# xd009642/xd-tts

Hardware: AMD Instinct MI355X
Metric: mel-frames/s per GPU, 120-phoneme utterance (Tacotron2 decoder+postnet + 60-iter Griffin-Lim), end-to-end (higher is better)
Workload: dtype f32

## Files before the change

### include/xdtts.h

```cpp
#ifndef XDTTS_H
#define XDTTS_H

#include <stddef.h>
#include <stdint.h>

#ifdef __cplusplus
extern "C" {
#endif

typedef int32_t xdtts_status;
enum {
  XDTTS_OK = 0,
  XDTTS_ERR_BAD_ARG = 1,
  XDTTS_ERR_IO = 2,
  XDTTS_ERR_HIP = 3,
  XDTTS_ERR_OOM = 4,
  XDTTS_ERR_TOO_LONG = 5,
  XDTTS_ERR_NO_DEVICE = 6
};

typedef struct xdtts_tacotron2 xdtts_tacotron2;
typedef struct xdtts_griffinlim xdtts_griffinlim;

typedef struct {
  float gate_threshold;
  int32_t max_steps;
  int32_t fixed_steps;
  int32_t dropout_mode;
  uint32_t dropout_seed;
  int32_t max_chunk;
  uint32_t item_base;
  float fixed_frames_per_id;
  const uint8_t *dropout_masks;
  int32_t dropout_mask_steps;
} xdtts_infer_opts;

void xdtts_infer_opts_default(xdtts_infer_opts *opts);


xdtts_status xdtts_tacotron2_load(const char *dir, int32_t device_id, xdtts_tacotron2 **out);

#define XDTTS_DEVICE_DEFAULT (-1)
int32_t xdtts_default_device(void);

xdtts_status xdtts_model_dir_read(const char *dir, float *blob, size_t n_floats);

xdtts_status xdtts_model_dir_describe(const char *dir, char *buf, size_t cap, size_t *needed);

xdtts_status xdtts_tacotron2_load_synthetic(uint32_t seed, float rec_scale, int32_t device_id,
                                            xdtts_tacotron2 **out);

xdtts_status xdtts_tacotron2_load_blob(const float *blob, size_t n_floats, int32_t device_id,
                                       xdtts_tacotron2 **out);

xdtts_status xdtts_tacotron2_save(const xdtts_tacotron2 *h, const char *dir);

int32_t xdtts_tensor_count(void);
const char *xdtts_tensor_name(int32_t i);
int32_t xdtts_tensor_ndim(int32_t i);
int32_t xdtts_tensor_dim(int32_t i, int32_t d);
size_t xdtts_tensor_offset(int32_t i);
size_t xdtts_tensor_total(void);
xdtts_status xdtts_tacotron2_get_tensor(const xdtts_tacotron2 *h, int32_t i, float *out);

xdtts_status xdtts_tacotron2_infer_ids(xdtts_tacotron2 *h, const int64_t *ids, size_t n,
                                       const size_t *splits, size_t n_splits,
                                       const xdtts_infer_opts *opts, float **mel,
                                       size_t *n_frames);

xdtts_status xdtts_tacotron2_infer_batch(xdtts_tacotron2 *h, const int64_t *ids,
                                         const int32_t *lens, int32_t B, int32_t t_stride,
                                         const xdtts_infer_opts *opts,
                                         const int32_t *fixed_steps_per_item, float **mels,
                                         size_t *n_frames);

xdtts_status xdtts_tacotron2_encoder(xdtts_tacotron2 *h, const int64_t *ids, int32_t T,
                                     float *memory, float *processed_memory);
xdtts_status xdtts_tacotron2_decoder(xdtts_tacotron2 *h, const float *memory,
                                     const float *processed_memory, int32_t T, int32_t n_valid,
                                     const xdtts_infer_opts *opts, float *frames, float *gates,
                                     size_t *n_frames);
xdtts_status xdtts_tacotron2_decoder_step(xdtts_tacotron2 *h, const float *memory, const float *processed_memory,
                                          int32_t T, int32_t n_valid, const xdtts_infer_opts *opts, uint32_t step,
                                          const float *decoder_input, float *attention_hidden,
                                          float *attention_cell, float *decoder_hidden, float *decoder_cell,
                                          float *attention_weights, float *attention_weights_cum,
                                          float *attention_context, float *decoder_output,
                                          float *gate_prediction);

xdtts_status xdtts_tacotron2_decoder_steps(xdtts_tacotron2 *h, int32_t engine, int32_t B, const float *memory,
                                           const float *processed_memory, int32_t T, const int32_t *n_valid,
                                           const xdtts_infer_opts *opts, uint32_t step0, int32_t n_steps,
                                           const float *decoder_input, float *attention_hidden, float *attention_cell,
                                           float *decoder_hidden, float *decoder_cell, float *attention_weights,
                                           float *attention_weights_cum, float *attention_context, float *decoder_output,
                                           float *gate_prediction);

xdtts_status xdtts_tacotron2_engine_state(const xdtts_tacotron2 *h, int32_t *decoder_persistent,
                                          int32_t *encoder_cooperative, int32_t *batched_attention);
xdtts_status xdtts_tacotron2_engine_reset(xdtts_tacotron2 *h);
xdtts_status xdtts_tacotron2_small_batch_engine_state(const xdtts_tacotron2 *h, int32_t *state);

const char *xdtts_build_info(void);

xdtts_status xdtts_edge_floor_us(int32_t device_id, int32_t steps, int32_t T, int32_t tuned, double *us_per_step);

xdtts_status xdtts_tacotron2_postnet(xdtts_tacotron2 *h, const float *frames, int32_t F,
                                     float *mel_out);

xdtts_status xdtts_tacotron2_last_timings(const xdtts_tacotron2 *h, float ms[4], int32_t *steps);

void xdtts_tacotron2_free(xdtts_tacotron2 *h);


xdtts_status xdtts_mel_filter_bank(float sample_rate, size_t n_fft, size_t n_mels, float fmin,
                                   float fmax_or_nan, float *out);

xdtts_status xdtts_griffinlim_new(const float *mel_basis, size_t n_mels, size_t n_bins,
                                  size_t noverlap, float power, size_t iters, float momentum,
                                  int32_t device_id, xdtts_griffinlim **out);

typedef struct {
  int32_t nnls_iters;
  int32_t power_mode;
  int32_t mel_decompress;
  int32_t output_normalise;
  int32_t batch_shape;
  float rms_target;
} xdtts_griffinlim_opts;
void xdtts_griffinlim_opts_default(xdtts_griffinlim_opts *opts);
xdtts_status xdtts_griffinlim_set_opts(xdtts_griffinlim *g, const xdtts_griffinlim_opts *opts);
xdtts_status xdtts_griffinlim_get_opts(const xdtts_griffinlim *g, xdtts_griffinlim_opts *opts);

xdtts_status xdtts_griffinlim_set_seed(xdtts_griffinlim *g, uint32_t seed);

xdtts_status xdtts_griffinlim_infer(xdtts_griffinlim *g, const float *mel, size_t n_mels,
                                    size_t n_frames, float **audio, size_t *n_samples);

xdtts_status xdtts_griffinlim_infer_batch(xdtts_griffinlim *g, const float *const *mels, size_t n_mels,
                                          const size_t *n_frames, int32_t n_utt, float **audios,
                                          size_t *n_samples);

xdtts_status xdtts_griffinlim_infer_linear(xdtts_griffinlim *g, const float *S,
                                           const float *phase0, size_t n_frames, size_t iters,
                                           float **audio, size_t *n_samples);

xdtts_status xdtts_griffinlim_mel_to_linear(xdtts_griffinlim *g, const float *mel,
                                            size_t n_mels, size_t n_frames, float *S_out);

xdtts_status xdtts_griffinlim_step(xdtts_griffinlim *g, const float *S, float *angles,
                                   float *rebuilt, size_t n_frames, size_t n_iter);

xdtts_status xdtts_griffinlim_last_timings(const xdtts_griffinlim *g, float ms[3]);

size_t       xdtts_griffinlim_analysis_frames(const xdtts_griffinlim *g, size_t n_samples);
xdtts_status xdtts_griffinlim_analyze(xdtts_griffinlim *g, const float *audio, size_t n_samples, float mel_floor,
                                      float *S_out, float *mel_out, size_t *n_frames);
xdtts_status xdtts_griffinlim_analyze_batch(xdtts_griffinlim *g, const float *const *audios, const size_t *n_samples,
                                            int32_t n_utt, float mel_floor, float **S_outs, float **mel_outs,
                                            size_t *n_frames);
xdtts_status xdtts_griffinlim_spectral_convergence(xdtts_griffinlim *g, const float *audio, size_t n_samples,
                                                   const float *S, size_t n_frames, int32_t fit_gain, float out[2]);
xdtts_status xdtts_griffinlim_analysis_timings(const xdtts_griffinlim *g, float ms[3]);

void xdtts_griffinlim_free(xdtts_griffinlim *g);

xdtts_status xdtts_synthesize_ids(xdtts_tacotron2 *h, xdtts_griffinlim *g, const int64_t *ids,
                                  size_t n, const size_t *splits, size_t n_splits,
                                  const xdtts_infer_opts *opts, float **mel, size_t *n_frames,
                                  float **audio, size_t *n_samples);

xdtts_status xdtts_synthesize_batch(xdtts_tacotron2 *h, xdtts_griffinlim *g, const int64_t *ids,
                                    const int32_t *lens, int32_t B, int32_t t_stride,
                                    const int32_t *utt_chunks, int32_t n_utt,
                                    const xdtts_infer_opts *opts,
                                    const int32_t *fixed_steps_per_item, float **mels,
                                    size_t *n_frames, float **audios, size_t *n_samples);

xdtts_status xdtts_synthesize_sequence(xdtts_tacotron2 *h, xdtts_griffinlim *g, const int64_t *const *ids,
                                       const size_t *n_ids, const size_t *const *splits, const size_t *n_splits,
                                       int32_t n_utt, const xdtts_infer_opts *opts, float **mels,
                                       size_t *n_frames, float **audios, size_t *n_samples);

int32_t xdtts_symbol_count(void);
const char *xdtts_symbol_token(int32_t id);
int64_t xdtts_unit_id(const char *token, int32_t as_character);
int32_t xdtts_split_score(int64_t id);
xdtts_status xdtts_find_splits(const int64_t *ids, size_t n, size_t max_size, size_t *out,
                               size_t cap, size_t *n_out);

#define XDTTS_SAMPLE_RATE 22050
xdtts_status xdtts_audio_to_i16(const float *audio, size_t n, int16_t *pcm);
size_t xdtts_silence_samples(double seconds, uint32_t sample_rate);
size_t xdtts_silence_samples_duration(uint64_t secs, uint32_t nanos, uint32_t sample_rate);
xdtts_status xdtts_wav_write(const char *path, const int16_t *pcm, size_t n, uint32_t sample_rate);
xdtts_status xdtts_npy_write_f32(const char *path, const float *data, size_t rows, size_t cols);
double xdtts_real_time_factor(double compute_seconds, size_t n_samples);

void xdtts_free(void *p);
const char *xdtts_last_error(void);
int32_t xdtts_device_count(void);
xdtts_status xdtts_tacotron2_sync(xdtts_tacotron2 *h);

#ifdef __cplusplus
}
#endif
#endif
```

### xd-tts_amd/__init__.py

```python
import ctypes as C
import os

import numpy as np

_HERE = os.path.dirname(os.path.abspath(__file__))
LIB_PATH = os.environ.get("XDTTS_LIB") or os.path.join(_HERE, "libxdtts_hip.so")

N_MEL = 80
EMB = 512
ATT_DIM = 128

STATUS = {0: "OK", 1: "BAD_ARG", 2: "IO", 3: "HIP", 4: "OOM", 5: "TOO_LONG", 6: "NO_DEVICE"}
XDTTS_ERR_BAD_ARG, XDTTS_ERR_IO, XDTTS_ERR_HIP, XDTTS_ERR_OOM, XDTTS_ERR_TOO_LONG, XDTTS_ERR_NO_DEVICE = 1, 2, 3, 4, 5, 6


class XdttsError(RuntimeError):

    def __init__(self, status, message):
        super().__init__("xdtts status %d (%s): %s" % (status, STATUS.get(status, "?"), message))
        self.status = status


class GriffinLimOpts(C.Structure):

    _fields_ = [("nnls_iters", C.c_int32), ("power_mode", C.c_int32), ("mel_decompress", C.c_int32), ("output_normalise", C.c_int32), ("batch_shape", C.c_int32), ("rms_target", C.c_float)]


class InferOpts(C.Structure):
    _fields_ = [
        ("gate_threshold", C.c_float),
        ("max_steps", C.c_int32),
        ("fixed_steps", C.c_int32),
        ("dropout_mode", C.c_int32),
        ("dropout_seed", C.c_uint32),
        ("max_chunk", C.c_int32),
        ("item_base", C.c_uint32),
        ("fixed_frames_per_id", C.c_float),
        ("dropout_masks", C.c_void_p),
        ("dropout_mask_steps", C.c_int32),
    ]


_VP, _I32, _U32, _SZ, _F = C.c_void_p, C.c_int32, C.c_uint32, C.c_size_t, C.c_float
_PF = C.POINTER(C.c_float)
SYMBOLS = {
    "xdtts_infer_opts_default": (None, [C.POINTER(InferOpts)]),
    "xdtts_tacotron2_load": (_I32, [C.c_char_p, _I32, C.POINTER(_VP)]),
    "xdtts_model_dir_read": (_I32, [C.c_char_p, _VP, _SZ]),
    "xdtts_model_dir_describe": (_I32, [C.c_char_p, C.c_char_p, _SZ, C.POINTER(_SZ)]),
    "xdtts_tacotron2_load_synthetic": (_I32, [_U32, _F, _I32, C.POINTER(_VP)]),
    "xdtts_tacotron2_load_blob": (_I32, [_VP, _SZ, _I32, C.POINTER(_VP)]),
    "xdtts_tacotron2_save": (_I32, [_VP, C.c_char_p]),
    "xdtts_tensor_count": (_I32, []),
    "xdtts_tensor_name": (C.c_char_p, [_I32]),
    "xdtts_tensor_ndim": (_I32, [_I32]),
    "xdtts_tensor_dim": (_I32, [_I32, _I32]),
    "xdtts_tensor_offset": (_SZ, [_I32]),
    "xdtts_tensor_total": (_SZ, []),
    "xdtts_tacotron2_get_tensor": (_I32, [_VP, _I32, _VP]),
    "xdtts_tacotron2_infer_ids": (_I32, [_VP, _VP, _SZ, _VP, _SZ, C.POINTER(InferOpts), C.POINTER(_PF), C.POINTER(_SZ)]),
    "xdtts_tacotron2_infer_batch": (_I32, [_VP, _VP, _VP, _I32, _I32, C.POINTER(InferOpts), _VP, C.POINTER(_PF), C.POINTER(_SZ)]),
    "xdtts_tacotron2_encoder": (_I32, [_VP, _VP, _I32, _VP, _VP]),
    "xdtts_tacotron2_decoder": (_I32, [_VP, _VP, _VP, _I32, _I32, C.POINTER(InferOpts), _VP, _VP, C.POINTER(_SZ)]),
    "xdtts_tacotron2_decoder_step": (_I32, [_VP, _VP, _VP, _I32, _I32, C.POINTER(InferOpts), _U32] + [_VP] * 10),
    "xdtts_tacotron2_decoder_steps": (_I32, [_VP, _I32, _I32, _VP, _VP, _I32, _VP, C.POINTER(InferOpts), _U32, _I32] + [_VP] * 10),
    "xdtts_tacotron2_engine_state": (_I32, [_VP, C.POINTER(_I32), C.POINTER(_I32), C.POINTER(_I32)]),
    "xdtts_tacotron2_small_batch_engine_state": (_I32, [_VP, C.POINTER(_I32)]),
    "xdtts_tacotron2_engine_reset": (_I32, [_VP]),
    "xdtts_tacotron2_postnet": (_I32, [_VP, _VP, _I32, _VP]),
    "xdtts_tacotron2_last_timings": (_I32, [_VP, C.POINTER(C.c_float * 4), C.POINTER(_I32)]),
    "xdtts_tacotron2_free": (None, [_VP]),
    "xdtts_tacotron2_sync": (_I32, [_VP]),
    "xdtts_mel_filter_bank": (_I32, [_F, _SZ, _SZ, _F, _F, _VP]),
    "xdtts_griffinlim_new": (_I32, [_VP, _SZ, _SZ, _SZ, _F, _SZ, _F, _I32, C.POINTER(_VP)]),
    "xdtts_griffinlim_opts_default": (None, [_VP]),
    "xdtts_griffinlim_set_opts": (_I32, [_VP, _VP]),
    "xdtts_griffinlim_get_opts": (_I32, [_VP, _VP]),
    "xdtts_griffinlim_set_seed": (_I32, [_VP, _U32]),
    "xdtts_griffinlim_infer": (_I32, [_VP, _VP, _SZ, _SZ, C.POINTER(_PF), C.POINTER(_SZ)]),
    "xdtts_griffinlim_infer_batch": (_I32, [_VP, _VP, _SZ, _VP, _I32, _VP, _VP]),
    "xdtts_griffinlim_infer_linear": (_I32, [_VP, _VP, _VP, _SZ, _SZ, C.POINTER(_PF), C.POINTER(_SZ)]),
    "xdtts_griffinlim_mel_to_linear": (_I32, [_VP, _VP, _SZ, _SZ, _VP]),
    "xdtts_griffinlim_step": (_I32, [_VP, _VP, _VP, _VP, _SZ, _SZ]),
    "xdtts_griffinlim_last_timings": (_I32, [_VP, C.POINTER(C.c_float * 3)]),
    "xdtts_griffinlim_analysis_frames": (_SZ, [_VP, _SZ]),
    "xdtts_griffinlim_analyze": (_I32, [_VP, _VP, _SZ, _F, _VP, _VP, C.POINTER(_SZ)]),
    "xdtts_griffinlim_analyze_batch": (_I32, [_VP, _VP, _VP, _I32, _F, _VP, _VP, _VP]),
    "xdtts_griffinlim_spectral_convergence": (_I32, [_VP, _VP, _SZ, _VP, _SZ, _I32, C.POINTER(C.c_float * 2)]),
    "xdtts_griffinlim_analysis_timings": (_I32, [_VP, C.POINTER(C.c_float * 3)]),
    "xdtts_griffinlim_free": (None, [_VP]),
    "xdtts_synthesize_ids": (_I32, [_VP, _VP, _VP, _SZ, _VP, _SZ, C.POINTER(InferOpts), C.POINTER(_PF), C.POINTER(_SZ), C.POINTER(_PF), C.POINTER(_SZ)]),
    "xdtts_synthesize_batch": (_I32, [_VP, _VP, _VP, _VP, _I32, _I32, _VP, _I32, C.POINTER(InferOpts), _VP, _VP, _VP, _VP, _VP]),
    "xdtts_synthesize_sequence": (_I32, [_VP, _VP, _VP, _VP, _VP, _VP, _I32, C.POINTER(InferOpts), _VP, _VP, _VP, _VP]),
    "xdtts_symbol_count": (_I32, []),
    "xdtts_symbol_token": (C.c_char_p, [_I32]),
    "xdtts_unit_id": (C.c_int64, [C.c_char_p, _I32]),
    "xdtts_split_score": (_I32, [C.c_int64]),
    "xdtts_find_splits": (_I32, [_VP, _SZ, _SZ, _VP, _SZ, C.POINTER(_SZ)]),
    "xdtts_audio_to_i16": (_I32, [_VP, _SZ, _VP]),
    "xdtts_build_info": (C.c_char_p, []),
    "xdtts_edge_floor_us": (_I32, [C.c_int32, C.c_int32, C.c_int32, C.c_int32, C.POINTER(C.c_double)]),
    "xdtts_default_device": (C.c_int32, []),
    "xdtts_silence_samples": (_SZ, [C.c_double, _U32]),
    "xdtts_silence_samples_duration": (_SZ, [C.c_uint64, _U32, _U32]),
    "xdtts_wav_write": (_I32, [C.c_char_p, _VP, _SZ, _U32]),
    "xdtts_npy_write_f32": (_I32, [C.c_char_p, _VP, _SZ, _SZ]),
    "xdtts_real_time_factor": (C.c_double, [C.c_double, _SZ]),
    "xdtts_free": (None, [_VP]),
    "xdtts_last_error": (C.c_char_p, []),
    "xdtts_device_count": (_I32, []),
}


def _share_torch_hip_runtime():
    import importlib.util
    import sys

    if "torch" in sys.modules:
        return
    try:
        spec = importlib.util.find_spec("torch")
    except (ImportError, ValueError):
        spec = None
    if not spec or not spec.origin:
        return
    lib = os.path.join(os.path.dirname(spec.origin), "lib", "libamdhip64.so")
    if os.path.exists(lib):
        try:
            C.CDLL(lib, mode=C.RTLD_GLOBAL)
        except OSError:
            pass


def _load():
    _share_torch_hip_runtime()
    if not os.path.exists(LIB_PATH):
        raise ImportError(
            "%s not found: build it with `make -C %s` (or __graft_entry__.build()); there is no CPU fallback" % (LIB_PATH, _HERE)
        )
    lib = C.CDLL(LIB_PATH)
    for name, (res, args) in SYMBOLS.items():
        fn = getattr(lib, name)
        fn.restype = res
        fn.argtypes = args
    return lib


lib = _load()


def _check(status):
    if status != 0:
        raise XdttsError(status, lib.xdtts_last_error().decode("utf-8", "replace"))


def _ptr(a):
    return a.ctypes.data_as(C.c_void_p)


def default_opts(**kw):
    o = InferOpts()
    lib.xdtts_infer_opts_default(C.byref(o))
    masks = kw.pop("dropout_masks", None)
    for k, v in kw.items():
        setattr(o, k, v)
    if masks is not None:
        m = np.ascontiguousarray(masks, dtype=np.uint8)
        if m.ndim != 4 or m.shape[2:] != (2, 256):
            raise ValueError("dropout_masks must be (chunks, steps, 2, 256)")
        o._masks_keepalive = m
        o.dropout_masks = m.ctypes.data
        o.dropout_mask_steps = m.shape[1]
        o.dropout_mode = 2
    return o


def device_count():
    return lib.xdtts_device_count()


def tensor_table():
    out = []
    for i in range(lib.xdtts_tensor_count()):
        shape = tuple(lib.xdtts_tensor_dim(i, d) for d in range(lib.xdtts_tensor_ndim(i)))
        out.append((lib.xdtts_tensor_name(i).decode(), shape, lib.xdtts_tensor_offset(i)))
    return out


def read_model_dir(path):
    blob = np.empty(lib.xdtts_tensor_total(), dtype=np.float32)
    _check(lib.xdtts_model_dir_read(os.fsencode(path), _ptr(blob), blob.size))
    return {n: blob[off : off + int(np.prod(shape))].reshape(shape) for n, shape, off in tensor_table()}


def describe_model_dir(path):
    need = C.c_size_t()
    _check(lib.xdtts_model_dir_describe(os.fsencode(path), None, 0, C.byref(need)))
    buf = C.create_string_buffer(need.value)
    _check(lib.xdtts_model_dir_describe(os.fsencode(path), buf, need.value, None))
    out = {}
    for line in buf.value.decode().splitlines():
        f, rest = line.split(": inputs ", 1)
        i, o = rest.split(" ; outputs ", 1)
        out[f] = ([x for x in i.split(",") if x], [x for x in o.split(",") if x])
    return out


class _Pinned:

    def __init__(self, addr):
        self.addr = addr

    def __del__(self):
        if self.addr and lib is not None:
            lib.xdtts_free(C.cast(self.addr, _PF))
            self.addr = None


def _take(ptr, n, shape):
    addr = C.cast(ptr, C.c_void_p).value
# ... 71 lines not shown
def silence_samples_duration(secs, nanos, sample_rate=SAMPLE_RATE):
    return int(lib.xdtts_silence_samples_duration(int(secs), int(nanos), int(sample_rate)))


def write_wav(path, audio, sample_rate=SAMPLE_RATE):
    pcm = np.ascontiguousarray(audio) if np.asarray(audio).dtype == np.int16 else audio_to_i16(audio)
    _check(lib.xdtts_wav_write(os.fsencode(path), _ptr(pcm), pcm.size, int(sample_rate)))


def write_mel_npy(path, mel):
    m = np.ascontiguousarray(mel, dtype=np.float32)
    _check(lib.xdtts_npy_write_f32(os.fsencode(path), _ptr(m), m.shape[0], m.shape[1]))


def real_time_factor(compute_seconds, n_samples):
    return float(lib.xdtts_real_time_factor(float(compute_seconds), int(n_samples)))


def find_splits(ids, max_size=100):
    ids = np.ascontiguousarray(ids, dtype=np.int64)
    out = np.empty(max(ids.size, 1) + 2, dtype=np.uintp)
    n = C.c_size_t()
    _check(lib.xdtts_find_splits(_ptr(ids), ids.size, max_size, _ptr(out), out.size, C.byref(n)))
    return out[: n.value].astype(np.int64)


class Tacotron2:

    def __init__(self, handle):
        self._h = handle

    @classmethod
    def load(cls, path, device_id=0):
        h = C.c_void_p()
        _check(lib.xdtts_tacotron2_load(os.fsencode(path), device_id, C.byref(h)))
        return cls(h)

    @classmethod
    def synthetic(cls, seed=20240327, rec_scale=1.0, device_id=0):
        h = C.c_void_p()
        _check(lib.xdtts_tacotron2_load_synthetic(seed, rec_scale, device_id, C.byref(h)))
        return cls(h)

    @classmethod
    def from_blob(cls, blob, device_id=0):
        blob = np.ascontiguousarray(blob, dtype=np.float32)
        h = C.c_void_p()
        _check(lib.xdtts_tacotron2_load_blob(_ptr(blob), blob.size, device_id, C.byref(h)))
        return cls(h)

    def close(self):
        if self._h:
            lib.xdtts_tacotron2_free(self._h)
            self._h = None

    def __del__(self):
        try:
            self.close()
        except Exception:
            pass

    def save(self, path):
        _check(lib.xdtts_tacotron2_save(self._h, os.fsencode(path)))

    def blob(self):
        out = np.zeros(lib.xdtts_tensor_total(), dtype=np.float32)
        for i, (_n, shape, off) in enumerate(tensor_table()):
            t = np.empty(shape, dtype=np.float32)
            _check(lib.xdtts_tacotron2_get_tensor(self._h, i, _ptr(t)))
            out[off : off + t.size] = t.ravel()
        return out

    def get_tensor(self, name):
        for i, (n, shape, _off) in enumerate(tensor_table()):
            if n == name:
                out = np.empty(shape, dtype=np.float32)
                _check(lib.xdtts_tacotron2_get_tensor(self._h, i, _ptr(out)))
                return out
        raise KeyError(name)

    def infer(self, ids, splits=None, opts=None):
        ids = np.ascontiguousarray(ids, dtype=np.int64)
        sp = None if splits is None else np.ascontiguousarray(splits, dtype=np.uintp)
        mel, nf = _PF(), C.c_size_t()
        _check(
            lib.xdtts_tacotron2_infer_ids(
                self._h, _ptr(ids), ids.size, None if sp is None else _ptr(sp), 0 if sp is None else sp.size, C.byref(opts) if opts else None, C.byref(mel), C.byref(nf)
            )
        )
        return _take(mel, N_MEL * nf.value, (N_MEL, nf.value))

    def infer_units(self, tokens, opts=None, as_character=False):
        ids = units_to_ids(tokens, as_character)
        window = opts.max_chunk if opts else 100
        return self.infer(ids, splits=find_splits(ids, window), opts=opts)

    def infer_batch(self, ids_list, opts=None, fixed_steps=None):
        B = len(ids_list)
        lens = np.array([len(x) for x in ids_list], dtype=np.int32)
        stride = int(lens.max()) if B else 1
        ids = np.zeros((B, stride), dtype=np.int64)
        for b, x in enumerate(ids_list):
            ids[b, : len(x)] = x
        fs = None if fixed_steps is None else np.ascontiguousarray(fixed_steps, dtype=np.int32)
        mels = (_PF * B)()
        nf = (C.c_size_t * B)()
        _check(lib.xdtts_tacotron2_infer_batch(self._h, _ptr(ids), _ptr(lens), B, stride, C.byref(opts) if opts else None, None if fs is None else _ptr(fs), mels, nf))
        return [_take(mels[b], N_MEL * nf[b], (N_MEL, nf[b])) for b in range(B)]

    def encoder(self, ids):
        ids = np.ascontiguousarray(ids, dtype=np.int64)
        T = ids.size
        memory = np.empty((T, EMB), dtype=np.float32)
        pmem = np.empty((T, ATT_DIM), dtype=np.float32)
        _check(lib.xdtts_tacotron2_encoder(self._h, _ptr(ids), T, _ptr(memory), _ptr(pmem)))
        return memory, pmem

    def decoder(self, memory, pmem, n_valid, opts=None):
        memory = np.ascontiguousarray(memory, dtype=np.float32)
        pmem = np.ascontiguousarray(pmem, dtype=np.float32)
        o = opts if opts else default_opts()
        frames = np.empty((o.max_steps, N_MEL), dtype=np.float32)
        gates = np.empty(o.max_steps, dtype=np.float32)
        nf = C.c_size_t()
        _check(lib.xdtts_tacotron2_decoder(self._h, _ptr(memory), _ptr(pmem), memory.shape[0], n_valid, C.byref(o), _ptr(frames), _ptr(gates), C.byref(nf)))
        return frames[: nf.value].copy(), gates[: nf.value].copy()

    def decoder_step(self, memory, pmem, n_valid, state, decoder_input, step, opts=None):
        memory = np.ascontiguousarray(memory, dtype=np.float32)
        pmem = np.ascontiguousarray(pmem, dtype=np.float32)
        names = ("attention_hidden", "attention_cell", "decoder_hidden", "decoder_cell", "attention_weights", "attention_weights_cum", "attention_context")
        st = {k: np.array(state[k], dtype=np.float32, order="C") for k in names}
        din = np.ascontiguousarray(decoder_input, dtype=np.float32)
        out, gate = np.empty(N_MEL, dtype=np.float32), np.empty(1, dtype=np.float32)
        _check(lib.xdtts_tacotron2_decoder_step(self._h, _ptr(memory), _ptr(pmem), memory.shape[0], n_valid, C.byref(opts) if opts else None, step,
                                                _ptr(din), *[_ptr(st[k]) for k in names], _ptr(out), _ptr(gate)))
        return out, float(gate[0]), st

    ENGINES = {"launch": 0, "persistent": 1, "batched": 2, "persistent8": 3}

    def decoder_steps(self, engine, memory, pmem, n_valid, states, decoder_input, step0, n_steps=1, opts=None):
        memory = np.ascontiguousarray(memory, dtype=np.float32)
        pmem = np.ascontiguousarray(pmem, dtype=np.float32)
        B, T = memory.shape[0], memory.shape[1]
        nv = np.ascontiguousarray(n_valid, dtype=np.int32)
        names = ("attention_hidden", "attention_cell", "decoder_hidden", "decoder_cell", "attention_weights", "attention_weights_cum", "attention_context")
        st = {k: np.array(states[k], dtype=np.float32, order="C") for k in names}
        din = np.ascontiguousarray(decoder_input, dtype=np.float32)
        out, gate = np.empty((B, n_steps, N_MEL), dtype=np.float32), np.empty((B, n_steps), dtype=np.float32)
        _check(lib.xdtts_tacotron2_decoder_steps(self._h, self.ENGINES[engine], B, _ptr(memory), _ptr(pmem), T, _ptr(nv), C.byref(opts) if opts else None,
                                                 step0, n_steps, _ptr(din), *[_ptr(st[k]) for k in names], _ptr(out), _ptr(gate)))
        return out, gate, st

    def engine_state(self):
        a, b, c = C.c_int32(), C.c_int32(), C.c_int32()
        _check(lib.xdtts_tacotron2_engine_state(self._h, C.byref(a), C.byref(b), C.byref(c)))
        e = C.c_int32()
        _check(lib.xdtts_tacotron2_small_batch_engine_state(self._h, C.byref(e)))
        return {"decoder_persistent": a.value, "encoder_cooperative": b.value, "batched_attention": c.value, "decoder_persistent8": e.value}

    def engine_reset(self):
        _check(lib.xdtts_tacotron2_engine_reset(self._h))

    def postnet(self, frames):
        frames = np.ascontiguousarray(frames, dtype=np.float32)
        F = frames.shape[0]
        out = np.empty((N_MEL, F), dtype=np.float32)
        _check(lib.xdtts_tacotron2_postnet(self._h, _ptr(frames), F, _ptr(out)))
        return out

    def last_timings(self):
        ms = (C.c_float * 4)()
        steps = C.c_int32()
        _check(lib.xdtts_tacotron2_last_timings(self._h, C.byref(ms), C.byref(steps)))
        return {"encoder_ms": ms[0], "decoder_ms": ms[1], "postnet_ms": ms[2], "total_ms": ms[3], "steps": steps.value}


def create_mel_filter_bank(sample_rate, n_fft, n_mels, fmin, fmax=None):
    out = np.empty((n_mels, n_fft // 2 + 1), dtype=np.float32)
    _check(lib.xdtts_mel_filter_bank(sample_rate, n_fft, n_mels, fmin, float("nan") if fmax is None else fmax, _ptr(out)))
    return out


class GriffinLim:

    def __init__(self, mel_basis, noverlap, power, iters, momentum, device_id=0, seed=0):
        basis = np.ascontiguousarray(mel_basis, dtype=np.float32)
        self._h = C.c_void_p()
        _check(lib.xdtts_griffinlim_new(_ptr(basis), basis.shape[0], basis.shape[1], noverlap, power, iters, momentum, device_id, C.byref(self._h)))
        self.n_mels, self.n_bins = basis.shape
        self.set_seed(seed)

    def set_seed(self, seed):
        _check(lib.xdtts_griffinlim_set_seed(self._h, seed))

    def set_opts(self, **kw):
        o = self.get_opts()
        for k, v in kw.items():
            setattr(o, k, v)
        _check(lib.xdtts_griffinlim_set_opts(self._h, C.byref(o)))

    def get_opts(self):
        o = GriffinLimOpts()
        _check(lib.xdtts_griffinlim_get_opts(self._h, C.byref(o)))
        return o

    def close(self):
        if self._h:
            lib.xdtts_griffinlim_free(self._h)
            self._h = None

    def __del__(self):
        try:
            self.close()
        except Exception:
            pass

    def infer(self, mel):
        mel = np.ascontiguousarray(mel, dtype=np.float32)
        audio, n = _PF(), C.c_size_t()
        _check(lib.xdtts_griffinlim_infer(self._h, _ptr(mel), mel.shape[0], mel.shape[1], C.byref(audio), C.byref(n)))
        return _take(audio, n.value, (n.value,))

    def infer_batch(self, mels):
        ms = [np.ascontiguousarray(m, dtype=np.float32) for m in mels]
        n = len(ms)
        ptrs = (C.c_void_p * n)(*[m.ctypes.data for m in ms])
        nf = (C.c_size_t * n)(*[m.shape[1] for m in ms])
        audios = (_PF * n)()
        ns = (C.c_size_t * n)()
        _check(lib.xdtts_griffinlim_infer_batch(self._h, ptrs, ms[0].shape[0], nf, n, audios, ns))
        return [_take(audios[u], ns[u], (ns[u],)) for u in range(n)]

    def infer_linear(self, S, phase0=None, iters=0):
        S = np.ascontiguousarray(S, dtype=np.float32)
        p0 = None if phase0 is None else np.ascontiguousarray(phase0, dtype=np.float32)
        audio, n = _PF(), C.c_size_t()
        _check(lib.xdtts_griffinlim_infer_linear(self._h, _ptr(S), None if p0 is None else _ptr(p0), S.shape[1], iters, C.byref(audio), C.byref(n)))
        return _take(audio, n.value, (n.value,))

    def step(self, S, angles, rebuilt, n_iter=1):
        S = np.ascontiguousarray(S, dtype=np.float32)
        a = np.array(angles, dtype=np.float32, order="C")
        r = np.array(rebuilt, dtype=np.float32, order="C")
        _check(lib.xdtts_griffinlim_step(self._h, _ptr(S), _ptr(a), _ptr(r), S.shape[1], n_iter))
        return a, r

    def mel_to_linear(self, mel):
        mel = np.ascontiguousarray(mel, dtype=np.float32)
        S = np.empty((self.n_bins, mel.shape[1]), dtype=np.float32)
        _check(lib.xdtts_griffinlim_mel_to_linear(self._h, _ptr(mel), mel.shape[0], mel.shape[1], _ptr(S)))
        return S

    def last_timings(self):
        ms = (C.c_float * 3)()
        _check(lib.xdtts_griffinlim_last_timings(self._h, C.byref(ms)))
        return {"mel_to_linear_ms": ms[0], "iterations_ms": ms[1], "total_ms": ms[2]}

    def analysis_frames(self, n_samples):
        return int(lib.xdtts_griffinlim_analysis_frames(self._h, int(n_samples)))

    def analyze(self, audio, mel_floor=1e-5, want_S=True, want_mel=True):
        S, mel = self.analyze_batch([audio], mel_floor, want_S, want_mel)
        return (S[0] if want_S else None), (mel[0] if want_mel else None)

    def analyze_batch(self, audios, mel_floor=1e-5, want_S=True, want_mel=True):
        ys = [np.ascontiguousarray(a, dtype=np.float32).ravel() for a in audios]
        n = len(ys)
        Fs = [self.analysis_frames(max(y.size, 1)) for y in ys]
        S = [np.empty((self.n_bins, F), dtype=np.float32) for F in Fs] if want_S else None
        mel = [np.empty((self.n_mels, F), dtype=np.float32) for F in Fs] if want_mel else None
        ptrs = (C.c_void_p * n)(*[y.ctypes.data for y in ys])
        ns = (C.c_size_t * n)(*[y.size for y in ys])
        Sp = (C.c_void_p * n)(*[a.ctypes.data for a in S]) if want_S else None
        Mp = (C.c_void_p * n)(*[a.ctypes.data for a in mel]) if want_mel else None
        nf = (C.c_size_t * n)()
        _check(lib.xdtts_griffinlim_analyze_batch(self._h, ptrs, ns, n, mel_floor, Sp, Mp, nf))
        assert list(nf) == Fs
        return S, mel

    def spectral_convergence(self, audio, S, fit_gain=False):
        y = np.ascontiguousarray(audio, dtype=np.float32).ravel()
        S = np.ascontiguousarray(S, dtype=np.float32)
        out = (C.c_float * 2)()
        _check(lib.xdtts_griffinlim_spectral_convergence(self._h, _ptr(y), y.size, _ptr(S), S.shape[1], 1 if fit_gain else 0, C.byref(out)))
        return float(out[0]), float(out[1])

    def analysis_timings(self):
        ms = (C.c_float * 3)()
        _check(lib.xdtts_griffinlim_analysis_timings(self._h, C.byref(ms)))
        return {"magnitude_ms": ms[0], "projection_ms": ms[1], "total_ms": ms[2]}


def create_griffin_lim(device_id=0, iters=30, seed=0):
    mel_basis = create_mel_filter_bank(22050.0, 1024, 80, 0.0, 8000.0)
    return GriffinLim(mel_basis, 1024 - 256, 1.7, iters, 0.99, device_id=device_id, seed=seed)


def synthesize(tacotron2, vocoder, ids, splits=None, opts=None):
    ids = np.ascontiguousarray(ids, dtype=np.int64)
    sp = None if splits is None else np.ascontiguousarray(splits, dtype=np.uintp)
    mel, nf, audio, ns = _PF(), C.c_size_t(), _PF(), C.c_size_t()
    _check(
        lib.xdtts_synthesize_ids(
            tacotron2._h, vocoder._h, _ptr(ids), ids.size, None if sp is None else _ptr(sp), 0 if sp is None else sp.size, C.byref(opts) if opts else None, C.byref(mel), C.byref(nf), C.byref(audio), C.byref(ns)
        )
# ... 41 lines not shown
```

### xd-tts_amd/csrc/api_tacotron2.cpp

```cpp
#include <algorithm>
#include <cmath>
#include <memory>

#include "tacotron2_handle.h"

#include "edge_floor.hip"

using namespace xdtts;

extern "C" {

void xdtts_infer_opts_default(xdtts_infer_opts *o) {
  if (!o) return;
  o->gate_threshold = 0.6f;
  o->max_steps = 1000;
  o->fixed_steps = 0;
  o->dropout_mode = 1;
  o->dropout_seed = 0;
  o->max_chunk = 100;
  o->item_base = 0;
  o->fixed_frames_per_id = 0.f;
  o->dropout_masks = nullptr;
  o->dropout_mask_steps = 0;
}
// ... 251 lines not shown
          if (std::fabs(c - attention_context[(size_t)b * EMB + j]) > 1e-4 + 1e-4 * std::fabs(c))
            fail(XDTTS_ERR_BAD_ARG, "engine 1 needs attention_context = attention_weights . memory (chunk %d, column %d: %g vs %g)", b, j,
                 (double)attention_context[(size_t)b * EMB + j], c);
        }
    }
    std::lock_guard<std::mutex> lk(h->mu);
    HIP_CHECK(hipSetDevice(h->device));
    xdtts_infer_opts o = resolve_opts(opts);
    const int end = (int)step0 + n_steps;
    o.max_steps = end + 1;
    hipStream_t st = h->stream;
    h->memory.upload(memory, (size_t)B * T * EMB, st);
    h->pmem.upload(processed_memory, (size_t)B * T * ATT_DIM, st);
    h->n_valid.upload(n_valid, B, st);
    std::vector<int> lim((size_t)B, end);
    h->upload_dropout_masks(o, B, lim.data());
    if (engine == 2) h->w.ensure_batched_layout(h->blob, st);
    DecoderBufs d = h->decoder_bufs(B, T, h->memory.p, h->pmem.p, o, engine == 2 ? 1 : 0);
    d.use_gate = 0;
    h->limits.upload(lim.data(), lim.size(), st);
    h->lim_on_dev = lim;
    launch_decoder_init(d, h->limits.p, st);
    h->dec_in_dev.upload(decoder_input, (size_t)B * N_MEL, st);
    const size_t nh = (size_t)B * ATT_RNN, nt = (size_t)B * T, nc = (size_t)B * EMB;
    h->state_stage.alloc(4 * nh + 2 * nt + nc);
    float *s_ah = h->state_stage.p, *s_ac = s_ah + nh, *s_dh = s_ac + nh, *s_dc = s_dh + nh, *s_aw = s_dc + nh, *s_awc = s_aw + nt, *s_ctx = s_awc + nt;
    auto up = [&](float *dst, const float *src, size_t n) { HIP_CHECK(hipMemcpyAsync(dst, src, n * sizeof(float), hipMemcpyHostToDevice, st)); };
    auto dd = [&](float *dst, const float *src, size_t n) { HIP_CHECK(hipMemcpyAsync(dst, src, n * sizeof(float), hipMemcpyDeviceToDevice, st)); };
    up(s_ah, attention_hidden, nh);
    up(s_ac, attention_cell, nh);
    up(s_dh, decoder_hidden, nh);
    up(s_dc, decoder_cell, nh);
    up(s_aw, attention_weights, nt);
    up(s_awc, attention_weights_cum, nt);
    up(s_ctx, attention_context, nc);
    const int s0 = (int)step0;
    HIP_CHECK(hipMemcpyAsync(d.ctl, &s0, sizeof(int), hipMemcpyHostToDevice, st));
    HIP_CHECK(hipStreamSynchronize(st));
    dd(d.aw, s_aw, nt);
    dd(d.awc, s_awc, nt);
    dd(d.ctx, s_ctx, nc);
    if (engine == 2) {
      launch_frag_convert(s_ah, d.att_hf[0], B, d.Bpad, ATT_RNN, 0, st);
      launch_frag_convert(s_dh, d.dec_hf[0], B, d.Bpad, DEC_RNN, 0, st);
      launch_frag_convert(s_ac, d.att_c, B, d.Bpad, ATT_RNN, 0, st);
      launch_frag_convert(s_dc, d.dec_c, B, d.Bpad, DEC_RNN, 0, st);
      launch_frag_convert(s_ctx, d.ctxf, B, d.Bpad, EMB, 0, st);
    } else {
      dd(d.att_h[0], s_ah, nh);
      dd(d.att_c, s_ac, nh);
      dd(d.dec_h[0], s_dh, nh);
      dd(d.dec_c, s_dc, nh);
    }
    d.dec_in = h->dec_in_dev.p;
    int fin = 0;
    if (engine == 1) {
      if (!decoder_persistent_supported(h->device, PERSIST_B_MAX, PERSIST_T_MAX))
        fail(XDTTS_ERR_HIP, "persistent engine not available on this device (its 256-workgroup grid cannot be co-resident)");
      std::lock_guard<ChipLock> chip(chip_mutex(h->device));
      launch_decoder_prenet(d, h->w, st);
      d.dec_in = nullptr;
      h->dec_exchange.alloc(persist_granule_words(B));
      PersistBufs g = persist_bufs(h->dec_exchange.p, h->dec_err.p, B);
      launch_persist_seed_at(d, g, h->limits.p, s0, st);
      try {
        launch_decoder_persistent(d, h->w, g, n_steps, st);
      } catch (const CoopRefused &) {
        (void)hipStreamSynchronize(st);
        fail(XDTTS_ERR_HIP, "persistent engine not available on this device (cooperative launch refused)");
      }
      if (fetch_and_clear_error_word(h->dec_err.p, st)) fail(XDTTS_ERR_HIP, "persistent decoder exchange timed out (grid not co-resident)");
    } else if (engine == 3) {
      if (!decoder_p8_supported(h->device, B, PERSIST_T_MAX))
        fail(XDTTS_ERR_HIP, "persistent MFMA engine not available on this device (its 256-workgroup grid cannot be co-resident)");
      std::lock_guard<ChipLock> chip(chip_mutex(h->device));
      launch_decoder_prenet(d, h->w, st);
      d.dec_in = nullptr;
      h->dec_exchange.alloc(p8_exchange_words(B, n_steps));
      P8Bufs g = p8_bufs(h->dec_exchange.p, h->dec_err.p, B, n_steps);
      launch_p8_seed_at(d, g, h->limits.p, s0, st);
      try {
        launch_decoder_p8(d, h->w, g, n_steps, st);
      } catch (const CoopRefused &) {
        (void)hipStreamSynchronize(st);
        fail(XDTTS_ERR_HIP, "persistent MFMA engine not available on this device (cooperative launch refused)");
      }
      if (fetch_and_clear_error_word(h->dec_err.p, st)) fail(XDTTS_ERR_HIP, "persistent MFMA decoder exchange timed out (grid not co-resident)");
    } else {
      std::unique_lock<ChipLock> chip;
      if (d.hg) chip = std::unique_lock<ChipLock>(chip_mutex(h->device));
      if (engine == 0) launch_decoder_location(d, h->w, st);
      launch_decoder_early(d, h->w, 0, st);
      launch_decoder_prologue(d, h->w, st);
      for (int i = 0; i < n_steps; ++i) {
        launch_decoder_step_at(d, h->w, i, st);
        d.dec_in = nullptr;
      }
      launch_decoder_advance(d, n_steps, st);
      launch_decoder_flush(d, h->w, st);
      fin = n_steps & 1;
      if (d.ep_g && fetch_and_clear_error_word(h->dec_err.p, st)) fail(XDTTS_ERR_HIP, "batched attention exchange timed out (grid not co-resident)");
    }
    if (engine == 2) {
      launch_frag_convert(s_ah, d.att_hf[fin], B, d.Bpad, ATT_RNN, 1, st);
      launch_frag_convert(s_dh, d.dec_hf[fin], B, d.Bpad, DEC_RNN, 1, st);
      launch_frag_convert(s_ac, d.att_c, B, d.Bpad, ATT_RNN, 1, st);
      launch_frag_convert(s_dc, d.dec_c, B, d.Bpad, DEC_RNN, 1, st);
    }
    auto down = [&](float *dst, const float *src, size_t n) { HIP_CHECK(hipMemcpyAsync(dst, src, n * sizeof(float), hipMemcpyDeviceToHost, st)); };
    down(attention_hidden, engine == 2 ? s_ah : d.att_h[fin], nh);
    down(attention_cell, engine == 2 ? s_ac : d.att_c, nh);
    down(decoder_hidden, engine == 2 ? s_dh : d.dec_h[fin], nh);
    down(decoder_cell, engine == 2 ? s_dc : d.dec_c, nh);
    down(attention_weights, d.aw, nt);
    down(attention_weights_cum, engine == 2 && (n_steps & 1) ? d.awc2 : d.awc, nt);
    down(attention_context, d.ctx, nc);
    for (int b = 0; b < B; ++b) {
      down(decoder_output + (size_t)b * n_steps * N_MEL, d.frames + ((size_t)b * d.max_steps + step0) * N_MEL, (size_t)n_steps * N_MEL);
      down(gate_prediction + (size_t)b * n_steps, d.gates + (size_t)b * d.max_steps + step0, (size_t)n_steps);
    }
    HIP_CHECK(hipStreamSynchronize(st));
  });
}

xdtts_status xdtts_tacotron2_decoder_step(xdtts_tacotron2 *h, const float *memory, const float *processed_memory, int32_t T,
                                          int32_t n_valid, const xdtts_infer_opts *opts, uint32_t step, const float *decoder_input,
                                          float *attention_hidden, float *attention_cell, float *decoder_hidden, float *decoder_cell,
                                          float *attention_weights, float *attention_weights_cum, float *attention_context,
                                          float *decoder_output, float *gate_prediction) {
  return xdtts_tacotron2_decoder_steps(h, 0, 1, memory, processed_memory, T, &n_valid, opts, step, 1, decoder_input, attention_hidden,
                                       attention_cell, decoder_hidden, decoder_cell, attention_weights, attention_weights_cum,
                                       attention_context, decoder_output, gate_prediction);
}

xdtts_status xdtts_tacotron2_engine_state(const xdtts_tacotron2 *h, int32_t *decoder_persistent, int32_t *encoder_cooperative,
                                          int32_t *batched_attention) {
  return guard([&] {
    if (!h) fail(XDTTS_ERR_BAD_ARG, "null handle");
    std::lock_guard<std::mutex> lk(h->mu);
    if (decoder_persistent) *decoder_persistent = h->pair_gate.abi_state();
    if (encoder_cooperative) *encoder_cooperative = h->enc_gate.state != EngineGate::OFF ? 1 : 0;
    if (batched_attention) *batched_attention = h->att_fused();
  });
}

xdtts_status xdtts_tacotron2_small_batch_engine_state(const xdtts_tacotron2 *h, int32_t *state) {
  return guard([&] {
    if (!h || !state) fail(XDTTS_ERR_BAD_ARG, "null argument");
    std::lock_guard<std::mutex> lk(h->mu);
    *state = h->p8_gate.abi_state();
  });
}

xdtts_status xdtts_tacotron2_engine_reset(xdtts_tacotron2 *h) {
  return guard([&] {
    if (!h) fail(XDTTS_ERR_BAD_ARG, "null handle");
    std::lock_guard<std::mutex> lk(h->mu);
    h->pair_gate.reset();
    h->p8_gate.reset();
    h->enc_gate.reset();
    h->att_gate.reset();
    h->att_form = env::int_or(env::ATT_FUSED, 2);
  });
}

xdtts_status xdtts_edge_floor_us(int32_t device_id, int32_t steps, int32_t T, int32_t tuned, double *us_per_step) {
  return guard([&] {
    if (!us_per_step || steps < 1 || steps > 1000000 || T < 1 || T > 128) fail(XDTTS_ERR_BAD_ARG, "bad argument");
    device_id = select_device(device_id);
    std::lock_guard<ChipLock> chip(chip_mutex(device_id));
    const double us = xdtts_edge_floor::measure(device_id, steps, T, xdtts_edge_floor::kernel_delays(tuned ? 1 : 0), 5, false);
    if (us < 0) fail(XDTTS_ERR_HIP, "edge-floor skeleton: grid not co-resident on this device, or an exchange failed");
    *us_per_step = us;
  });
}

xdtts_status xdtts_tacotron2_postnet(xdtts_tacotron2 *h, const float *frames, int32_t F, float *mel_out) {
  return guard([&] {
    if (!h || !frames || !mel_out || F <= 0) fail(XDTTS_ERR_BAD_ARG, "bad argument");
    std::lock_guard<std::mutex> lk(h->mu);
    HIP_CHECK(hipSetDevice(h->device));
    h->frames.upload(frames, (size_t)F * N_MEL, h->stream);
    HIP_CHECK(hipStreamSynchronize(h->stream));
    h->mel_dev.alloc((size_t)N_MEL * F);
    const long zero = 0;
    h->run_postnet(h->frames.p, 0, &F, &zero, 1, h->mel_dev.p, F);
    HIP_CHECK(hipMemcpyAsync(mel_out, h->mel_dev.p, (size_t)N_MEL * F * sizeof(float), hipMemcpyDeviceToHost, h->stream));
    HIP_CHECK(hipStreamSynchronize(h->stream));
  });
}

xdtts_status xdtts_tacotron2_last_timings(const xdtts_tacotron2 *h, float ms[4], int32_t *steps) {
  return guard([&] {
    if (!h || !ms) fail(XDTTS_ERR_BAD_ARG, "null argument");
    for (int i = 0; i < 4; ++i) ms[i] = h->last_ms[i];
    if (steps) *steps = h->last_steps;
  });
}

}
```

### xd-tts_amd/csrc/decoder_persistent.hip

```cpp
#include <type_traits>

#include "device_utils.h"
#include "kernels.h"

namespace xdtts {

namespace {

typedef unsigned long long u64;

constexpr int PT = 512;
constexpr int NW = PT / 64;
constexpr int P_NCU = ATT_RNN / 4;
constexpr int TP = PERSIST_T_MAX;
constexpr int ATTN_CU = 8, PRE_CU = 16;
constexpr int EP_LD = TP, MEL_GL = 96;
#ifndef XDTTS_MEL_ST
#define XDTTS_MEL_ST 1
#endif
constexpr int MEL_ST = XDTTS_MEL_ST;
constexpr int GS = PERSIST_B_MAX;
constexpr unsigned P_SPIN_LIMIT = 1u << 21;
constexpr unsigned ACT_BIT = 0x80000000u;
constexpr int PERSIST_LAZY_DEFAULT = 9;
// ... 28 lines not shown
  for (int i = 0; i < N; ++i) {
    done[i] = !need[i];
    out[i] = 0.f;
    tag[i] = 0u;
  }
  if (PRE) {
    bool all = true;
#pragma unroll
    for (int i = 0; i < N; ++i)
      if (!done[i]) {
        const unsigned t = (unsigned)(pre[i] >> 32);
        if ((t & ~ACT_BIT) == want) {
          out[i] = __uint_as_float((unsigned)pre[i]);
          tag[i] = t;
          done[i] = true;
        } else {
          all = false;
        }
      }
    if (all) return 0u;
  }
  unsigned spins = 0;
  for (;;) {
    u64 v[N];
#pragma unroll
    for (int i = 0; i < N; ++i)
      if (!done[i]) v[i] = peek(base + (idx + (unsigned)i * stride));
    bool all = true;
#pragma unroll
    for (int i = 0; i < N; ++i)
      if (!done[i]) {
        const unsigned t = (unsigned)(v[i] >> 32);
        if ((t & ~ACT_BIT) == want) {
          out[i] = __uint_as_float((unsigned)v[i]);
          tag[i] = t;
          done[i] = true;
        } else {
          all = false;
        }
      }
    if (all || give_up(spins, err)) return spins;
  }
}

__device__ __forceinline__ void lazy_wait(int n) {
  for (int i = 0; i < n; ++i) __builtin_amdgcn_s_sleep(4);
}
__device__ __forceinline__ void straggle(bool me, int s, int at) {
  if (me && s % 6 == at)
    for (int i = 0; i < 2; ++i) __builtin_amdgcn_s_sleep(127);
}
__device__ __forceinline__ float4 lds4(const float *p) { return *reinterpret_cast<const float4 *>(p); }
__device__ __forceinline__ void chunk_fence() { asm volatile("" ::: "memory"); }
__device__ __forceinline__ unsigned opaque(unsigned v) {
  asm volatile("" : "+v"(v));
  return v;
}

constexpr int persist_lds_floats(int pb) {
  const int common = pb * (PRENET + TP + ATT_RNN + DEC_RNN + 16) + 8 + 32 + 16 * pb;
  const int attn = 2 * TP * 16 + 2 * TP + 16 + NW * 64 + 2 * WPAD + 62 * 16 + 64 + 16 + 8 * PT * 4;
  const int pre = N_MEL * PRENET + MEL_GL + 2 * PRENET + 8 + 6 * PT * 4;
  return common + (attn > pre ? attn : pre);
}

#ifdef XDTTS_PERSIST_PROFILE
#define PROF_MARK(i)                                       \
  do {                                                     \
    if (tid == 0) {                                        \
      const u64 now_ = wall_clock64();                     \
      s_prof[i] += now_ - prof_last;                       \
      prof_last = now_;                                    \
    }                                                      \
  } while (0)
#define PROF_POLLS(e, n)                                                   \
  do {                                                                     \
    const float m_ = wave_max((float)(n));                                 \
    if ((tid & 63) == 0) atomicAdd(&s_prof[16 + (e)], (u64)m_);            \
  } while (0)
#define PROF_WHEN(e)                                       \
  do {                                                     \
    if (tid == 0) s_prof[20 + (e)] += wall_clock64();      \
  } while (0)
#else
#define PROF_MARK(i) do { } while (0)
#define PROF_POLLS(e, n) do { (void)(n); } while (0)
#define PROF_WHEN(e) do { } while (0)
#endif

struct PersistWeights {
  const float4 *att_w, *dec_w, *q_w, *proj_w;
  const float *att_b, *dec_b, *v_w, *loc_fused, *proj_b, *pre0T, *pre1T;
};

template <int PB, bool SKEW = false, bool GATE = false>
__global__ __launch_bounds__(PT) void k_decoder_persistent(DecoderBufs d, PersistBufs g, PersistWeights w, int nsteps) {
  __shared__ __attribute__((aligned(16))) float smem[persist_lds_floats(PB)];
  const int c = blockIdx.x, tid = threadIdx.x, lane = tid & 63, wave = tid >> 6;
  const int T = d.T;
  const PollCtl pc{g.err, g.spins > 0 ? (unsigned)g.spins : P_SPIN_LIMIT};
  if (g.fault && c == g.fault - 1) return;
  const unsigned L4 = opaque(4u * (unsigned)lane);
  float *s_x = smem;
  float *s_e = s_x + PB * PRENET;
  float *s_hatt = s_e + PB * TP;
  float *s_hdec = s_hatt + PB * ATT_RNN;
  float *s_g = s_hdec + PB * DEC_RNN;
  int *s_act = reinterpret_cast<int *>(s_g + PB * 16);
  float *s_bias = s_g + PB * 16 + 8;
  float *s_cell = s_bias + 32;
  float *role = s_cell + 16 * PB;
  float *s_pm = role;
  float *s_loc = s_pm + TP * 16;
  float *s_aw = s_loc + TP * 16;
  float *s_awc = s_aw + TP;
  float *s_q = s_awc + TP;
  float *s_part = s_q + 16;
  float *s_wpad = s_part + NW * 64;
  float *s_G = s_wpad + 2 * WPAD;
  float *s_cown = s_G + 62 * 16;
  float *s_vv = s_cown + 64;
  float *s_qw = s_vv + 16;
  float *s_W0 = role;
  float *s_mel = s_W0 + N_MEL * PRENET;
  float *s_l1 = s_mel + MEL_GL;
  float *s_pb = s_l1 + 2 * PRENET;
  float *s_pw = s_pb + 8;

  float4 wa[2][ATT_COLS / 256], wd[2][DEC_COLS / 256];
#pragma unroll
  for (int r = 0; r < 2; ++r) {
    const int row = 16 * c + wave + NW * r;
#pragma unroll
    for (int k = 0; k < ATT_COLS / 256; ++k) wa[r][k] = ld_stream(w.att_w + (size_t)row * (ATT_COLS / 4) + lane + 64 * k);
#pragma unroll
    for (int k = 0; k < DEC_COLS / 256; ++k) wd[r][k] = ld_stream(w.dec_w + (size_t)row * (DEC_COLS / 4) + lane + 64 * k);
    if (lane == 0) {
      s_bias[wave + NW * r] = w.att_b[row];
      s_bias[16 + wave + NW * r] = w.dec_b[row];
    }
  }
  const bool attn = c < ATTN_CU * PB, pre = !attn && c < (ATTN_CU + PRE_CU) * PB;
  const int rb = attn ? c / ATTN_CU : (pre ? (c - ATTN_CU * PB) / PRE_CU : 0);
  const int rk = attn ? c % ATTN_CU : (c - ATTN_CU * PB) % PRE_CU;
  const int prow = rk + 16 * wave;
  const bool prow_ok = pre && wave < 6 && prow <= N_MEL;

  const int step0 = d.ctl[0];
  if (GATE && PB == 1 && !(step0 < d.nframes[0])) return;
  if (tid < PB) {
    s_act[tid] = 0;
    s_act[2 + tid] = step0 < d.nframes[tid];
  }
#pragma unroll
  for (int b = 0; b < PB; ++b) {
#pragma unroll
    for (int h = 0; h < 2; ++h) {
      s_hatt[b * ATT_RNN + tid + PT * h] = d.att_h[0][b * ATT_RNN + tid + PT * h];
      s_hdec[b * DEC_RNN + tid + PT * h] = d.dec_h[0][b * DEC_RNN + tid + PT * h];
    }
  }
  float wreg[PB][2];
  int nv[PB];
#pragma unroll
  for (int b = 0; b < PB; ++b) {
    wreg[b][0] = lane < T ? d.aw[b * T + lane] : 0.f;
    wreg[b][1] = lane + 64 < T ? d.aw[b * T + lane + 64] : 0.f;
    nv[b] = d.n_valid[b];
  }
  const int cb = tid >> 2, cu = tid & 3;
  const bool cell = tid < 4 * PB;
  if (cell) {
    s_cell[tid] = d.att_c[cb * ATT_RNN + 4 * c + cu];
    s_cell[4 * PB + tid] = d.dec_c[cb * DEC_RNN + 4 * c + cu];
    s_cell[8 * PB + tid] = d.att_h[0][cb * ATT_RNN + 4 * c + cu];
    s_cell[12 * PB + tid] = d.dec_h[0][cb * DEC_RNN + 4 * c + cu];
  }
  int nf_r = 0;
  if (attn) {
    for (int i = tid; i < TP * 16; i += PT) {
      const int t = i >> 4, dd = i & 15;
      s_pm[i] = t < T ? d.pmem[((size_t)rb * T + t) * ATT_DIM + 16 * rk + dd] : 0.f;
    }
    if (tid < TP) {
      s_aw[tid] = tid < T ? d.aw[rb * T + tid] : 0.f;
      s_awc[tid] = tid < T ? d.awc[rb * T + tid] : 0.f;
    }
    for (int i = tid; i < 62 * 16; i += PT) s_G[i] = w.loc_fused[(size_t)(i >> 4) * ATT_DIM + 16 * rk + (i & 15)];
    if (tid < 16) s_vv[tid] = w.v_w[16 * rk + tid];
#pragma unroll
    for (int r = 0; r < 2; ++r)
#pragma unroll
      for (int j = 0; j < 4; ++j)
        *reinterpret_cast<float4 *>(s_qw + 4 * ((4 * r + j) * PT + tid)) = w.q_w[(unsigned)((16 * rk + wave + NW * r) * (ATT_RNN / 4) + lane + 64 * j)];
  }
  if (pre) {
    for (int i = tid; i < N_MEL * PRENET; i += PT) s_W0[(((i / PRENET) >> 2) * PRENET + i % PRENET) * 4 + ((i / PRENET) & 3)] = w.pre0T[i];
    if (prow_ok) {
      if (lane == 0) s_pb[wave] = w.proj_b[prow];
#pragma unroll
      for (int j = 0; j < 6; ++j)
        *reinterpret_cast<float4 *>(s_pw + 4 * (j * PT + tid)) = w.proj_w[(unsigned)(prow * (PROJ_IN / 4) + lane + 64 * j)];
    }
    nf_r = d.nframes[rb];
  }
  constexpr bool ROLE_REGS = PB == 1;
  float rw[ROLE_REGS ? 40 : 1];
  if (ROLE_REGS) {
#pragma unroll
    for (int k = 0; k < 40; ++k) rw[ROLE_REGS ? k : 0] = 0.f;
    if (attn) {
#pragma unroll
      for (int r = 0; r < 2; ++r)
#pragma unroll
        for (int j = 0; j < 4; ++j) {
          const float4 q = w.q_w[(unsigned)((16 * rk + wave + NW * r) * (ATT_RNN / 4) + lane + 64 * j)];
          rw[ROLE_REGS ? 16 * r + 4 * j + 0 : 0] = q.x;
          rw[ROLE_REGS ? 16 * r + 4 * j + 1 : 0] = q.y;
          rw[ROLE_REGS ? 16 * r + 4 * j + 2 : 0] = q.z;
          rw[ROLE_REGS ? 16 * r + 4 * j + 3 : 0] = q.w;
        }
    } else if (pre) {
#pragma unroll
      for (int k = 0; k < N_MEL / 2; ++k) rw[ROLE_REGS ? k : 0] = w.pre0T[(unsigned)(((tid >> 8) * (N_MEL / 2) + k) * PRENET + (tid & 255))];
    }
  }
  float w1r[2][4];
#pragma unroll
  for (int r = 0; r < 2; ++r)
#pragma unroll
    for (int k = 0; k < 4; ++k) w1r[r][k] = pre ? w.pre1T[(unsigned)((lane + 64 * k) * PRENET + 16 * rk + wave + NW * r)] : 0.f;
  const uint32_t item = d.item_base + (uint32_t)rb;
  __syncthreads();

  float pma[PB][2][2], pmd[PB][2][2], pmp[2] = {0.f, 0.f};
  if (d.ctx_fold) {
#pragma unroll
    for (int b = 0; b < PB; ++b)
#pragma unroll
      for (int h = 0; h < 2; ++h) {
        const int t = lane + 64 * h;
        const float *F = d.ctx_fold + (size_t)b * CTXF_ROWS * CTXF_LD + t;
#pragma unroll
        for (int r = 0; r < 2; ++r) {
          const int row = 16 * c + wave + NW * r;
          pma[b][r][h] = t < T ? F[(size_t)row * CTXF_LD] : 0.f;
          pmd[b][r][h] = t < T ? F[(size_t)(4 * ATT_RNN + row) * CTXF_LD] : 0.f;
        }
        if (prow_ok && b == rb) pmp[h] = t < T ? F[(size_t)(4 * ATT_RNN + 4 * DEC_RNN + prow) * CTXF_LD] : 0.f;
      }
  } else {
    float4 pw4 = make_float4(0.f, 0.f, 0.f, 0.f), pw5 = pw4;
    if (prow_ok) {
      pw4 = lds4(s_pw + 4 * (4 * PT + tid));
      pw5 = lds4(s_pw + 4 * (5 * PT + tid));
    }
#pragma unroll
    for (int b = 0; b < PB; ++b) {
      const float4 *m4 = reinterpret_cast<const float4 *>(d.memory + (size_t)b * T * EMB);
#pragma unroll
      for (int h = 0; h < 2; ++h) {
        float ra[2] = {0.f, 0.f}, rd[2] = {0.f, 0.f}, rp = 0.f;
        for (int tt = 0; tt < 64 && tt + 64 * h < T; ++tt) {
          const int t = tt + 64 * h;
          const float4 m0 = m4[(size_t)t * (EMB / 4) + lane], m1 = m4[(size_t)t * (EMB / 4) + 64 + lane];
#pragma unroll
          for (int r = 0; r < 2; ++r) {
            const float va = wave_sum(dot4(wa[r][2], m1, dot4(wa[r][1], m0, 0.f)));
            const float vd = wave_sum(dot4(wd[r][5], m1, dot4(wd[r][4], m0, 0.f)));
            if (lane == tt) {
              ra[r] = va;
              rd[r] = vd;
            }
          }
          if (pre && b == rb) {
            const float vp = wave_sum(dot4(pw5, m1, dot4(pw4, m0, 0.f)));
            if (lane == tt) rp = vp;
          }
        }
#pragma unroll
        for (int r = 0; r < 2; ++r) {
          pma[b][r][h] = ra[r];
          pmd[b][r][h] = rd[r];
        }
        if (pre && b == rb) pmp[h] = rp;
      }
    }
  }

  float aacc[PB][2], dacc[PB][2];
  auto att_bulk = [&](unsigned L4, bool all) {
#pragma unroll
    for (int b = 0; b < PB; ++b) {
      if (!all && !s_act[b]) continue;
      const float w0 = wreg[b][0], w1 = wreg[b][1];
      float a0 = fmaf(pma[b][0][1], w1, pma[b][0][0] * w0), a1 = fmaf(pma[b][1][1], w1, pma[b][1][0] * w0);
#pragma unroll
      for (int k = 3; k < 7; ++k) {
        const float4 v = lds4(s_hatt + b * ATT_RNN + 256 * (k - 3) + L4);
        a0 = dot4(wa[0][k], v, a0);
        a1 = dot4(wa[1][k], v, a1);
      }
      aacc[b][0] = a0;
      aacc[b][1] = a1;
      chunk_fence();
    }
  };
  auto dec_bulk_h = [&](unsigned L4, bool all) {
#pragma unroll
    for (int b = 0; b < PB; ++b) {
      if (!all && !s_act[b]) continue;
      float a0 = 0.f, a1 = 0.f;
#pragma unroll
      for (int k = 6; k < 10; ++k) {
        const float4 v = lds4(s_hdec + b * DEC_RNN + 256 * (k - 6) + L4);
        a0 = dot4(wd[0][k], v, a0);
        a1 = dot4(wd[1][k], v, a1);
      }
      dacc[b][0] = a0;
      dacc[b][1] = a1;
      chunk_fence();
    }
  };
  auto location = [&](int tid) {
    typedef float f32x4 __attribute__((ext_vector_type(4)));
    for (int i = tid; i < 2 * WPAD; i += PT) {
      const int ch = i / WPAD, t = i % WPAD - (LOC_K - 1) / 2;
      s_wpad[i] = (t >= 0 && t < T) ? (ch ? s_awc[t] : s_aw[t]) : 0.f;
    }
    __syncthreads();
    {
      const unsigned l = (unsigned)tid & 63u, li = l & 15u, lg = l >> 4, t0 = 16u * ((unsigned)tid >> 6);
      float av[16], bv[16];
#pragma unroll
      for (int kk = 0; kk < 16; ++kk) {
        const unsigned q = 4u * kk + lg, qa = q < 2u * LOC_K ? q : 2u * LOC_K - 1u, ch = qa >= (unsigned)LOC_K ? 1u : 0u;
        av[kk] = s_wpad[ch * WPAD + t0 + li + (qa - ch * LOC_K)];
        bv[kk] = q < 2u * LOC_K ? s_G[qa * 16u + li] : 0.f;
      }
      f32x4 acc0 = (f32x4){0.f, 0.f, 0.f, 0.f}, acc1 = acc0;
#pragma unroll
      for (int kk = 0; kk < 16; kk += 2) {
        acc0 = __builtin_amdgcn_mfma_f32_16x16x4f32(av[kk], bv[kk], acc0, 0, 0, 0);
        acc1 = __builtin_amdgcn_mfma_f32_16x16x4f32(av[kk + 1], bv[kk + 1], acc1, 0, 0, 0);
      }
#pragma unroll
      for (int j = 0; j < 4; ++j) s_loc[(t0 + 4u * lg + j) * 16u + li] = acc0[j] + acc1[j];
    }
    __syncthreads();
  };
  att_bulk(L4, true);
  dec_bulk_h(L4, true);
  if (attn) location(tid);

#ifdef XDTTS_PERSIST_PROFILE
  __shared__ u64 s_prof[24];
  if (tid < 24) s_prof[tid] = 0;
  u64 prof_last = wall_clock64();
  __syncthreads();
#endif
  int s = step0;
  const int s_stop = step0 + nsteps;
  if constexpr (SKEW) {
    static_assert(PB == 2, "the skewed loop is the pair kernel");
    const int tid_k = tid;
    const bool lag = g.slow && c == g.slow - 1;
    unsigned drop1 = 0u, drop2 = 0u;
    u64 pf[2] = {0ull, 0ull};
    auto issue_x = [&](auto B, int s) {
      constexpr int b = decltype(B)::value;
      const int tid = tid_k + (int)opaque(0u);
      pf[0] = tid < 256 ? peek(g.x + (unsigned)(((s & 1) * GS + b) * PRENET + (tid & 255))) : 0ull;
      pf[1] = 0ull;
    };
    auto issue_h = [&](const u64 *base, auto B, int s) {
      constexpr int b = decltype(B)::value;
      const int tid = tid_k + (int)opaque(0u);
      pf[0] = peek(base + (unsigned)(((s & 1) * GS + b) * ATT_RNN + tid));
      pf[1] = peek(base + (unsigned)(((s & 1) * GS + b) * ATT_RNN + tid + PT));
    };
    auto issue_ep = [&](auto B, int s) {
      constexpr int b = decltype(B)::value;
      const int tid = tid_k + (int)opaque(0u), t = tid >> 2, j = tid & 3;
      pf[0] = t < T ? peek(g.ep + (unsigned)((((s & 1) * GS + b) * ATTN_CU + j) * EP_LD + t)) : 0ull;
      pf[1] = t < T ? peek(g.ep + (unsigned)((((s & 1) * GS + b) * ATTN_CU + j + 4) * EP_LD + t)) : 0ull;
    };
    auto issue_mel = [&](auto B, int s) {
      constexpr int b = decltype(B)::value;
      const int tid = tid_k + (int)opaque(0u);
      pf[0] = (pre && rb == b && tid < N_MEL + 1) ? peek(g.mel + (unsigned)((((s & 1) * GS + b) * MEL_GL + tid) * MEL_ST)) : 0ull;
      pf[1] = 0ull;
    };
    auto I0 = std::integral_constant<int, 0>{};
    auto I1 = std::integral_constant<int, 1>{};
    auto att_bulk1 = [&](auto B, unsigned L4) {
      constexpr int b = decltype(B)::value;
      const float w0 = wreg[b][0], w1 = wreg[b][1];
      float a0 = fmaf(pma[b][0][1], w1, pma[b][0][0] * w0), a1 = fmaf(pma[b][1][1], w1, pma[b][1][0] * w0);
#pragma unroll
      for (int k = 3; k < 7; ++k) {
        const float4 v = lds4(s_hatt + b * ATT_RNN + 256 * (k - 3) + L4);
        a0 = dot4(wa[0][k], v, a0);
        a1 = dot4(wa[1][k], v, a1);
      }
      aacc[b][0] = a0;
      aacc[b][1] = a1;
    };
    auto dec_bulk_h1 = [&](auto B, unsigned L4) {
      constexpr int b = decltype(B)::value;
      float a0 = 0.f, a1 = 0.f;
#pragma unroll
      for (int k = 6; k < 10; ++k) {
        const float4 v = lds4(s_hdec + b * DEC_RNN + 256 * (k - 6) + L4);
        a0 = dot4(wd[0][k], v, a0);
        a1 = dot4(wd[1][k], v, a1);
      }
      dacc[b][0] = a0;
      dacc[b][1] = a1;
    };
    auto ph1 = [&](auto B, int s, auto nxt) -> bool {
      constexpr int b = decltype(B)::value;
      const int tid = tid_k + (int)opaque(0u), lane = tid & 63, wave = tid >> 6;
      const unsigned L4 = 4u * (unsigned)lane;
      const int p = s & 1;
      const unsigned want = (unsigned)(s + 1);
      if (b == 0) straggle(lag, s, 0);
      {
        const int i = tid & 255;
        const bool need[1] = {tid < 256};
        float v[1];
        unsigned tg[1];
        gather<1, true>(g.x, (unsigned)((p * GS + b) * PRENET + i), 0u, want, need, v, tg, pc, pf);
        if (need[0]) {
          s_x[b * PRENET + i] = v[0];
          if (i == 0) s_act[b] = (tg[0] & ACT_BIT) ? 1 : 0;
        }
        if (tid == PT - 1) s_act[4] = __hip_atomic_load(g.err, __ATOMIC_RELAXED, __HIP_MEMORY_SCOPE_AGENT);
      }
      __syncthreads();
      const bool on = s_act[b] != 0 && s_act[4] == 0;
      if (!on) return false;
      {
        const float4 v = lds4(s_x + b * PRENET + L4);
        const float a0 = wave_sum(dot4(wa[0][0], v, aacc[b][0]));
        const float a1 = wave_sum(dot4(wa[1][0], v, aacc[b][1]));
        if (lane == 0) {
          s_g[b * 16 + wave] = a0 + s_bias[wave];
          s_g[b * 16 + wave + NW] = a1 + s_bias[wave + NW];
        }
      }
      __syncthreads();
      if (tid < 4 * PB && (tid >> 2) == b) {
        const int cu = tid & 3;
        const float *gp = s_g + b * 16 + 4 * cu;
        const float ig = fast_sigmoid(gp[0]), fg = fast_sigmoid(gp[1]), gg = fast_tanh(gp[2]), og = fast_sigmoid(gp[3]);
        const float cn = fmaf(fg, s_cell[tid], ig * gg), hn = og * fast_tanh(cn);
        publish(g.hatt + (unsigned)((p * GS + b) * ATT_RNN + 4 * c + cu), want, hn);
        s_cell[tid] = cn;
        s_cell[8 * PB + tid] = hn;
      }
      nxt();
      PROF_MARK(5 * b + 0);
      if (b == 0) straggle(lag, s, 1);
      __builtin_amdgcn_sched_barrier(0);
      return true;
    };
    auto ph2 = [&](auto B, int s, auto nxt) {
      constexpr int b = decltype(B)::value;
      const int tid = tid_k + (int)opaque(0u), lane = tid & 63, wave = tid >> 6;
      const unsigned L4 = 4u * (unsigned)lane, TID = (unsigned)tid;
      const int p = s & 1;
      const unsigned want = (unsigned)(s + 1);
      const bool mine = attn && rb == b;
      float4 lp4 = make_float4(0.f, 0.f, 0.f, 0.f), v4 = lp4;
      if (mine) {
        const float4 l4 = lds4(s_loc + 4 * TID), p4 = lds4(s_pm + 4 * TID);
        lp4 = make_float4(l4.x + p4.x, l4.y + p4.y, l4.z + p4.z, l4.w + p4.w);
        v4 = lds4(s_vv + 4 * (tid & 3));
      }
      {
        const bool need[2] = {true, true};
        float v[2];
        unsigned tg[2];
        gather<2, true>(g.hatt, (unsigned)((p * GS + b) * ATT_RNN + tid), PT, want, need, v, tg, pc, pf);
        s_hatt[b * ATT_RNN + TID] = v[0];
        s_hatt[b * ATT_RNN + TID + PT] = v[1];
      }
      __syncthreads();
      if (mine) {
        float q0 = 0.f, q1 = 0.f;
#pragma unroll
        for (int j = 0; j < 4; ++j) {
          const float4 v = lds4(s_hatt + b * ATT_RNN + 256 * j + L4);
          q0 = dot4(lds4(s_qw + 4 * (j * PT + TID)), v, q0);
          q1 = dot4(lds4(s_qw + 4 * ((4 + j) * PT + TID)), v, q1);
        }
        q0 = wave_sum(q0);
        q1 = wave_sum(q1);
        if (lane == 0) {
          s_q[wave] = q0;
          s_q[wave + NW] = q1;
        }
        __syncthreads();
        const int t = tid >> 2, dq = 4 * (tid & 3);
        const float4 q4 = lds4(s_q + dq);
        float e = v4.x * fast_tanh(q4.x + lp4.x);
        e = fmaf(v4.y, fast_tanh(q4.y + lp4.y), e);
        e = fmaf(v4.z, fast_tanh(q4.z + lp4.z), e);
        e = fmaf(v4.w, fast_tanh(q4.w + lp4.w), e);
        e += dpp_move<0xB1, 0xf>(0.f, e);
        e += dpp_move<0x4E, 0xf>(0.f, e);
        if ((tid & 3) == 0 && t < T) publish(g.ep + (unsigned)(((p * GS + b) * ATTN_CU + rk) * EP_LD + t), want, e);
      }
      {
        float a0 = dacc[b][0], a1 = dacc[b][1];
#pragma unroll
        for (int k = 0; k < 4; ++k) {
          const float4 v = lds4(s_hatt + b * ATT_RNN + 256 * k + L4);
          a0 = dot4(wd[0][k], v, a0);
          a1 = dot4(wd[1][k], v, a1);
        }
        dacc[b][0] = a0;
        dacc[b][1] = a1;
      }
      nxt();
      PROF_MARK(5 * b + 1);
      if (b == 0) straggle(lag, s, 2);
      __builtin_amdgcn_sched_barrier(0);
    };
    auto ph3 = [&](auto B, int s, auto nxt) {
      constexpr int b = decltype(B)::value;
      const int tid = tid_k + (int)opaque(0u), lane = tid & 63, wave = tid >> 6;
      const unsigned L4 = 4u * (unsigned)lane;
      const int p = s & 1;
      const unsigned want = (unsigned)(s + 1);
      const bool mine = attn && rb == b;
      {
        const int t = tid >> 2, j = tid & 3;
        const bool need[2] = {t < T, t < T};
        float v[2];
        unsigned tg[2];
        gather<2, true>(g.ep, (unsigned)(((p * GS + b) * ATTN_CU + j) * EP_LD + t), 4u * EP_LD, want, need, v, tg, pc, pf);
        float e = v[0] + v[1];
        e += dpp_move<0xB1, 0xf>(0.f, e);
        e += dpp_move<0x4E, 0xf>(0.f, e);
        if (j == 0) s_e[b * TP + t] = (t < T && t < nv[b]) ? e : -INFINITY;
      }
// ... 4 lines not shown
        const float x0 = fast_exp(e0 - m), x1 = fast_exp(e1 - m);
        const float rs = __builtin_amdgcn_rcpf(wave_sum(x0 + x1));
        wreg[b][0] = x0 * rs;
        wreg[b][1] = x1 * rs;
      }
      if (mine && wave == 0) {
        s_aw[lane] = wreg[b][0];
        s_awc[lane] += wreg[b][0];
        s_aw[lane + 64] = wreg[b][1];
        s_awc[lane + 64] += wreg[b][1];
      }
      if (b == 0) straggle(lag, s, 3);
      {
        const float w0 = wreg[b][0], w1 = wreg[b][1];
        float a0 = fmaf(pmd[b][0][1], w1, fmaf(pmd[b][0][0], w0, dacc[b][0]));
        float a1 = fmaf(pmd[b][1][1], w1, fmaf(pmd[b][1][0], w0, dacc[b][1]));
        a0 = wave_sum(a0);
        a1 = wave_sum(a1);
        if (lane == 0) {
          s_g[b * 16 + wave] = a0 + s_bias[16 + wave];
          s_g[b * 16 + wave + NW] = a1 + s_bias[16 + wave + NW];
        }
      }
      __syncthreads();
      if (tid < 4 * PB && (tid >> 2) == b) {
        const int cu = tid & 3;
        const float *gp = s_g + b * 16 + 4 * cu;
        const float ig = fast_sigmoid(gp[0]), fg = fast_sigmoid(gp[1]), gg = fast_tanh(gp[2]), og = fast_sigmoid(gp[3]);
        const float cn = fmaf(fg, s_cell[4 * PB + tid], ig * gg), hn = og * fast_tanh(cn);
        publish(g.hdec + (unsigned)((p * GS + b) * DEC_RNN + 4 * c + cu), want, hn);
        s_cell[4 * PB + tid] = cn;
        s_cell[12 * PB + tid] = hn;
      }
      att_bulk1(B, L4);
      nxt();
      PROF_MARK(5 * b + 2);
      if (b == 0) straggle(lag, s, 4);
      __builtin_amdgcn_sched_barrier(0);
    };
    auto ph4 = [&](auto B, int s, auto nxt) {
      constexpr int b = decltype(B)::value;
      const int tid = tid_k + (int)opaque(0u), lane = tid & 63, wave = tid >> 6;
      const unsigned L4 = 4u * (unsigned)lane, TID = (unsigned)tid;
      const int p = s & 1;
      const unsigned want = (unsigned)(s + 1);
      const bool mine = pre && rb == b;
      const int prow = rk + 16 * wave;
      const bool prow_ok = mine && wave < 6 && prow <= N_MEL;
      if (mine) {
        drop1 = 0u;
        drop2 = 0u;
        if (d.dropout_mode) {
#pragma unroll
          for (int k = 0; k < 4; ++k)
            drop1 |= (prenet_dropped(d.dropout_mode, d.dropout_seed, item, d.drop_masks, d.drop_steps, rb, s + 1, 0, lane + 64 * k) ? 1u : 0u) << k;
#pragma unroll
          for (int r = 0; r < 2; ++r)
            drop2 |= (prenet_dropped(d.dropout_mode, d.dropout_seed, item, d.drop_masks, d.drop_steps, rb, s + 1, 1, 16 * rk + wave + NW * r) ? 1u : 0u) << r;
        }
      }
      {
        const bool need[2] = {true, true};
        float v[2];
        unsigned tg[2];
        gather<2, true>(g.hdec, (unsigned)((p * GS + b) * DEC_RNN + tid), PT, want, need, v, tg, pc, pf);
        s_hdec[b * DEC_RNN + TID] = v[0];
        s_hdec[b * DEC_RNN + TID + PT] = v[1];
      }
      __syncthreads();
      if (prow_ok) {
        float a = 0.f;
#pragma unroll
        for (int j = 0; j < 4; ++j) a = dot4(lds4(s_pw + 4 * (j * PT + TID)), lds4(s_hdec + b * DEC_RNN + 256 * j + L4), a);
        a = fmaf(pmp[1], wreg[b][1], fmaf(pmp[0], wreg[b][0], a));
        a = wave_sum(a);
        if (lane == 0) publish(g.mel + (unsigned)(((p * GS + b) * MEL_GL + prow) * MEL_ST), want, a + s_pb[wave]);
      }
      dec_bulk_h1(B, L4);
      nxt();
      if (attn && rb == b) location(tid);
      PROF_MARK(5 * b + 3);
      if (b == 0) straggle(lag, s, 5);
      __builtin_amdgcn_sched_barrier(0);
    };
    auto ph5 = [&](auto B, int s, auto nxt) {
      constexpr int b = decltype(B)::value;
      if (!(pre && rb == b)) {
        nxt();
        return;
      }
      PROF_MARK(10 + 3 * b);
      const int tid = tid_k + (int)opaque(0u), lane = tid & 63, wave = tid >> 6;
      const unsigned L4 = 4u * (unsigned)lane, TID = (unsigned)tid;
      const int p = s & 1;
      const unsigned want = (unsigned)(s + 1);
      if (tid < N_MEL + 1) {
        const bool need[1] = {true};
        float v[1];
        unsigned tg[1];
        gather<1, true>(g.mel, (unsigned)(((p * GS + b) * MEL_GL + tid) * MEL_ST), 0, want, need, v, tg, pc, pf);
        s_mel[tid] = v[0];
      }
      __syncthreads();
      PROF_MARK(11 + 3 * b);
      const float gate = s_mel[N_MEL];
      const bool fired = GATE ? gate_fires(gate, d.gate_lo, d.gate_hi, d.gate_threshold) : (d.use_gate && gate_sigmoid(gate) > d.gate_threshold);
      if (rk == 0) {
        if (tid < N_MEL) d.frames[((size_t)b * d.max_steps + s) * N_MEL + tid] = s_mel[tid];
        if (tid == 0) {
          d.gates[(size_t)b * d.max_steps + s] = gate;
          if (fired) d.nframes[b] = s + 1;
        }
      }
      if (fired) nf_r = s + 1;
      const bool more = s + 1 < nf_r;
      float xo[2] = {0.f, 0.f};
      if (more) {
        const unsigned HM = (unsigned)((tid >> 8) * (N_MEL / 2));
        float acc = 0.f;
#pragma unroll
        for (int k = 0; k < N_MEL / 2; k += 4) {
          const float4 w4 = lds4(s_W0 + 4u * (((HM + k) >> 2) * PRENET + (TID & 255u))), m = lds4(s_mel + HM + k);
          acc = fmaf(w4.x, m.x, acc);
          acc = fmaf(w4.y, m.y, acc);
          acc = fmaf(w4.z, m.z, acc);
          acc = fmaf(w4.w, m.w, acc);
        }
        s_l1[TID] = acc;
        __syncthreads();
        float pk[4];
#pragma unroll
        for (int k = 0; k < 4; ++k) {
          const float v = fmaxf(s_l1[(L4 >> 2) + 64 * k] + s_l1[PRENET + (L4 >> 2) + 64 * k], 0.f);
          pk[k] = (drop1 >> k) & 1u ? 0.f : (d.dropout_mode ? 2.f * v : v);
        }
#pragma unroll
        for (int r = 0; r < 2; ++r) {
          float a = 0.f;
#pragma unroll
          for (int k = 0; k < 4; ++k) a = fmaf(w1r[r][k], pk[k], a);
          a = fmaxf(wave_sum(a), 0.f);
          xo[r] = (drop2 >> r) & 1u ? 0.f : (d.dropout_mode ? 2.f * a : a);
        }
      }
      if (lane < 2) s_mel[MEL_GL - 16 + wave + NW * lane] = lane ? xo[1] : xo[0];
      __syncthreads();
      if (tid < 16)
        publish(g.x + (unsigned)(((p ^ 1) * GS + b) * PRENET + 16 * rk + tid), (want + 1u) | (more ? ACT_BIT : 0u),
                s_mel[MEL_GL - 16 + tid]);
      nxt();
      PROF_MARK(5 * b + 4);
    };
    bool tail1 = false;
    if (s_act[2] != 0 && s_act[3] != 0) {
      issue_x(I0, s);
      for (;; ++s) {
        bool a0 = s < s_stop;
        if (a0) a0 = ph1(I0, s, [&] { if (tail1) issue_h(g.hdec, I1, s - 1); else issue_h(g.hatt, I0, s); });
        if (tail1) ph4(I1, s - 1, [&] { if (a0) issue_h(g.hatt, I0, s); });
        if (a0) ph2(I0, s, [&] { if (tail1) issue_mel(I1, s - 1); else issue_ep(I0, s); });
        if (tail1) {
          ph5(I1, s - 1, [&] { if (a0) issue_ep(I0, s); });
          tail1 = false;
        }
        if (!a0) break;
        ph3(I0, s, [&] { issue_x(I1, s); });
        const bool a1 = ph1(I1, s, [&] { issue_h(g.hdec, I0, s); });
        if (!a1) issue_h(g.hdec, I0, s);
        ph4(I0, s, [&] { if (a1) issue_h(g.hatt, I1, s); else issue_mel(I0, s); });
        if (a1) ph2(I1, s, [&] { issue_mel(I0, s); });
        ph5(I0, s, [&] { if (a1) issue_ep(I1, s); });
        if (!a1) {
          ++s;
          break;
        }
        ph3(I1, s, [&] { issue_x(I0, s + 1); });
        tail1 = true;
      }
    }
  } else
  for (; s < s_stop; ++s) {
    const int tid_it = tid + (int)opaque(0u);
    {
    const int tid = tid_it, lane = tid & 63, wave = tid >> 6;
    const unsigned L4 = 4u * (unsigned)lane, TID = (unsigned)tid;
    const int cb = tid >> 2, cu = tid & 3;
    const bool cell = tid < 4 * PB;
    const int prow = rk + 16 * wave;
    const bool prow_ok = pre && wave < 6 && prow <= N_MEL;
    const int p = s & 1;
    const unsigned want = (unsigned)(s + 1);
    const bool lag = g.slow && c == g.slow - 1;
    straggle(lag, s, 0);
    PROF_MARK(0);
    {
      const int b0 = tid >> 8, i = tid & 255;
      const bool need[2] = {b0 < PB && s_act[2 + (b0 < PB ? b0 : 0)] != 0, false};
      float v[2];
      unsigned tg[2];
      lazy_wait(pre ? g.xfirst : g.xlazy);
      const unsigned np_ = gather<2>(g.x, (unsigned)((p * GS + b0) * PRENET + i), 2u * PRENET, want, need, v, tg, pc);
      PROF_POLLS(0, np_);
#pragma unroll
      for (int j = 0; j < 2; ++j)
        if (need[j]) {
          s_x[(b0 + 2 * j) * PRENET + i] = v[j];
          if (i == 0) s_act[b0 + 2 * j] = (tg[j] & ACT_BIT) ? 1 : 0;
        }
      if (tid == PT - 1) s_act[4] = __hip_atomic_load(g.err, __ATOMIC_RELAXED, __HIP_MEMORY_SCOPE_AGENT);
    }
    __syncthreads();
    bool act[PB], any = false;
#pragma unroll
    for (int b = 0; b < PB; ++b) {
      act[b] = s_act[b] != 0;
      any = any || act[b];
    }
    if (tid < PB) s_act[2 + tid] = s_act[tid];
    PROF_MARK(1);
    PROF_WHEN(2);
    if (!any || s_act[4] != 0 || (PB == 2 && g.shrink && !(act[0] && act[1]))) break;
    const bool act_r = s_act[rb] != 0;
#pragma unroll
    for (int b = 0; b < PB; ++b)
      if (act[b]) {
        const float4 v = lds4(s_x + b * PRENET + L4);
        const float a0 = wave_sum(dot4(wa[0][0], v, aacc[b][0]));
        const float a1 = wave_sum(dot4(wa[1][0], v, aacc[b][1]));
        if (lane == 0) {
          s_g[b * 16 + wave] = a0 + s_bias[wave];
          s_g[b * 16 + wave + NW] = a1 + s_bias[wave + NW];
        }
      }
    __syncthreads();
    if (cell && s_act[cb]) {
      const float *gp = s_g + cb * 16 + 4 * cu;
      const float ig = fast_sigmoid(gp[0]), fg = fast_sigmoid(gp[1]), gg = fast_tanh(gp[2]), og = fast_sigmoid(gp[3]);
      const float cn = fmaf(fg, s_cell[tid], ig * gg), hn = og * fast_tanh(cn);
      publish(g.hatt + (unsigned)((p * GS + cb) * ATT_RNN + 4 * c + cu), want, hn);
      s_cell[tid] = cn;
      s_cell[8 * PB + tid] = hn;
    }
    PROF_MARK(2);
    PROF_WHEN(0);
    straggle(lag, s, 1);
    __builtin_amdgcn_sched_barrier(0);
    float4 lp4 = make_float4(0.f, 0.f, 0.f, 0.f), v4 = lp4;
    if (attn && act_r) {
      const float4 l4 = lds4(s_loc + 4 * TID), p4 = lds4(s_pm + 4 * TID);
      lp4 = make_float4(l4.x + p4.x, l4.y + p4.y, l4.z + p4.z, l4.w + p4.w);
      v4 = lds4(s_vv + 4 * (tid & 3));
    }
    {
      bool need[2 * PB];
#pragma unroll
      for (int i = 0; i < 2 * PB; ++i) need[i] = act[i >> 1];
      float v[2 * PB];
      unsigned tg[2 * PB];
      lazy_wait(attn ? g.first : g.lazy);
      const unsigned np_ = gather<2 * PB>(g.hatt, (unsigned)(p * GS * ATT_RNN + tid), PT, want, need, v, tg, pc);
      PROF_POLLS(1, np_);
#pragma unroll
      for (int i = 0; i < 2 * PB; ++i)
        if (need[i]) s_hatt[TID + PT * i] = v[i];
    }
    __syncthreads();
    PROF_MARK(3);
    if (attn && act_r) {
      float q0 = 0.f, q1 = 0.f;
#pragma unroll
      for (int j = 0; j < 4; ++j) {
        const float4 v = lds4(s_hatt + rb * ATT_RNN + 256 * j + L4);
        if (ROLE_REGS) {
          q0 = dot4(make_float4(rw[ROLE_REGS ? 4 * j : 0], rw[ROLE_REGS ? 4 * j + 1 : 0], rw[ROLE_REGS ? 4 * j + 2 : 0], rw[ROLE_REGS ? 4 * j + 3 : 0]), v, q0);
          q1 = dot4(make_float4(rw[ROLE_REGS ? 16 + 4 * j : 0], rw[ROLE_REGS ? 17 + 4 * j : 0], rw[ROLE_REGS ? 18 + 4 * j : 0], rw[ROLE_REGS ? 19 + 4 * j : 0]), v, q1);
        } else {
          q0 = dot4(lds4(s_qw + 4 * (j * PT + TID)), v, q0);
          q1 = dot4(lds4(s_qw + 4 * ((4 + j) * PT + TID)), v, q1);
        }
      }
      q0 = wave_sum(q0);
      q1 = wave_sum(q1);
      if (lane == 0) {
        s_q[wave] = q0;
        s_q[wave + NW] = q1;
      }
      __syncthreads();
      PROF_MARK(15);
      const int t = tid >> 2, dq = 4 * (tid & 3);
      const float4 q4 = lds4(s_q + dq);
      float e = v4.x * fast_tanh(q4.x + lp4.x);
      e = fmaf(v4.y, fast_tanh(q4.y + lp4.y), e);
      e = fmaf(v4.z, fast_tanh(q4.z + lp4.z), e);
      e = fmaf(v4.w, fast_tanh(q4.w + lp4.w), e);
      e += dpp_move<0xB1, 0xf>(0.f, e);
      e += dpp_move<0x4E, 0xf>(0.f, e);
      if ((tid & 3) == 0 && t < T) publish(g.ep + (unsigned)(((p * GS + rb) * ATTN_CU + rk) * EP_LD + t), want, e);
    }
#pragma unroll
    for (int b = 0; b < PB; ++b)
      if (act[b]) {
        float a0 = dacc[b][0], a1 = dacc[b][1];
#pragma unroll
        for (int k = 0; k < 4; ++k) {
          const float4 v = lds4(s_hatt + b * ATT_RNN + 256 * k + L4);
          a0 = dot4(wd[0][k], v, a0);
          a1 = dot4(wd[1][k], v, a1);
        }
        dacc[b][0] = a0;
        dacc[b][1] = a1;
        chunk_fence();
      }
    PROF_MARK(4);
    straggle(lag, s, 2);
    __builtin_amdgcn_sched_barrier(0);
    {
      const int t = tid >> 2, j = tid & 3;
      bool need[2 * PB];
#pragma unroll
      for (int i = 0; i < 2 * PB; ++i) need[i] = act[i >> 1] && t < T;
      float v[2 * PB];
      unsigned tg[2 * PB];
      lazy_wait(attn ? g.efirst : g.clazy);
      const unsigned np_ = gather<2 * PB>(g.ep, (unsigned)((p * GS * ATTN_CU + j) * EP_LD + t), 4u * EP_LD, want, need, v, tg, pc);
      PROF_POLLS(2, np_);
#pragma unroll
      for (int b = 0; b < PB; ++b) {
        float e = v[2 * b] + v[2 * b + 1];
        e += dpp_move<0xB1, 0xf>(0.f, e);
        e += dpp_move<0x4E, 0xf>(0.f, e);
        if (j == 0 && act[b]) s_e[b * TP + t] = (t < T && t < nv[b]) ? e : -INFINITY;
      }
    }
    __syncthreads();
    PROF_MARK(5);
    PROF_WHEN(3);
#pragma unroll
    for (int b = 0; b < PB; ++b)
      if (act[b]) {
        const float e0 = s_e[b * TP + lane], e1 = s_e[b * TP + lane + 64];
        const float m = wave_max(fmaxf(e0, e1));
        const float x0 = fast_exp(e0 - m), x1 = fast_exp(e1 - m);
        const float rs = __builtin_amdgcn_rcpf(wave_sum(x0 + x1));
        wreg[b][0] = x0 * rs;
        wreg[b][1] = x1 * rs;
      }
    if (attn && act_r && wave == 0) {
      s_aw[lane] = wreg[rb][0];
      s_awc[lane] += wreg[rb][0];
      s_aw[lane + 64] = wreg[rb][1];
      s_awc[lane + 64] += wreg[rb][1];
    }
    PROF_MARK(6);
    straggle(lag, s, 3);
    __builtin_amdgcn_sched_barrier(0);
#pragma unroll
    for (int b = 0; b < PB; ++b)
      if (act[b]) {
        const float w0 = wreg[b][0], w1 = wreg[b][1];
        float a0 = fmaf(pmd[b][0][1], w1, fmaf(pmd[b][0][0], w0, dacc[b][0]));
        float a1 = fmaf(pmd[b][1][1], w1, fmaf(pmd[b][1][0], w0, dacc[b][1]));
        a0 = wave_sum(a0);
        a1 = wave_sum(a1);
        if (lane == 0) {
          s_g[b * 16 + wave] = a0 + s_bias[16 + wave];
          s_g[b * 16 + wave + NW] = a1 + s_bias[16 + wave + NW];
        }
      }
    __syncthreads();
    if (cell && s_act[cb]) {
      const float *gp = s_g + cb * 16 + 4 * cu;
      const float ig = fast_sigmoid(gp[0]), fg = fast_sigmoid(gp[1]), gg = fast_tanh(gp[2]), og = fast_sigmoid(gp[3]);
      const float cn = fmaf(fg, s_cell[4 * PB + tid], ig * gg), hn = og * fast_tanh(cn);
      publish(g.hdec + (unsigned)((p * GS + cb) * DEC_RNN + 4 * c + cu), want, hn);
      s_cell[4 * PB + tid] = cn;
      s_cell[12 * PB + tid] = hn;
    }
    att_bulk(L4, false);
    PROF_MARK(7);
    PROF_WHEN(1);
    straggle(lag, s, 4);
    __builtin_amdgcn_sched_barrier(0);
    unsigned drop1 = 0u, drop2 = 0u;
    if (pre && act_r) {
      if (d.dropout_mode) {
#pragma unroll
        for (int k = 0; k < 4; ++k)
          drop1 |= (prenet_dropped(d.dropout_mode, d.dropout_seed, item, d.drop_masks, d.drop_steps, rb, s + 1, 0, lane + 64 * k) ? 1u : 0u) << k;
#pragma unroll
        for (int r = 0; r < 2; ++r)
          drop2 |= (prenet_dropped(d.dropout_mode, d.dropout_seed, item, d.drop_masks, d.drop_steps, rb, s + 1, 1, 16 * rk + wave + NW * r) ? 1u : 0u) << r;
      }
    }
    {
      bool need[2 * PB];
#pragma unroll
      for (int i = 0; i < 2 * PB; ++i) need[i] = act[i >> 1];
      float v[2 * PB];
      unsigned tg[2 * PB];
      lazy_wait(pre ? g.pfirst : g.lazy);
      const unsigned np_ = gather<2 * PB>(g.hdec, (unsigned)(p * GS * DEC_RNN + tid), PT, want, need, v, tg, pc);
      PROF_POLLS(3, np_);
#pragma unroll
      for (int i = 0; i < 2 * PB; ++i)
        if (need[i]) s_hdec[TID + PT * i] = v[i];
    }
    __syncthreads();
    PROF_MARK(8);
    if (prow_ok && act_r) {
      float a = 0.f;
#pragma unroll
      for (int j = 0; j < 4; ++j) a = dot4(lds4(s_pw + 4 * (j * PT + TID)), lds4(s_hdec + rb * DEC_RNN + 256 * j + L4), a);
      a = fmaf(pmp[1], wreg[rb][1], fmaf(pmp[0], wreg[rb][0], a));
      a = wave_sum(a);
      if (lane == 0) publish(g.mel + (unsigned)(((p * GS + rb) * MEL_GL + prow) * MEL_ST), want, a + s_pb[wave]);
    }
    dec_bulk_h(L4, false);
    if (attn && act_r) location(tid);
    PROF_MARK(9);
    straggle(lag, s, 5);
    __builtin_amdgcn_sched_barrier(0);
    if (pre && act_r) {
      bool nxt = false;
      if (act_r) {
        if (tid < N_MEL + 1) {
          const bool need[1] = {true};
          float v[1];
          unsigned tg[1];
          gather<1>(g.mel, (unsigned)(((p * GS + rb) * MEL_GL + tid) * MEL_ST), 0, want, need, v, tg, pc);
          s_mel[tid] = v[0];
        }
        __syncthreads();
        PROF_MARK(11);
        const float gate = s_mel[N_MEL];
        const bool fired = GATE ? gate_fires(gate, d.gate_lo, d.gate_hi, d.gate_threshold) : (d.use_gate && gate_sigmoid(gate) > d.gate_threshold);
        if (rk == 0) {
          if (tid < N_MEL) d.frames[((size_t)rb * d.max_steps + s) * N_MEL + tid] = s_mel[tid];
          if (tid == 0) {
            d.gates[(size_t)rb * d.max_steps + s] = gate;
            if (fired) d.nframes[rb] = s + 1;
          }
        }
        if (fired) nf_r = s + 1;
        nxt = s + 1 < nf_r;
      }
      float xo[2] = {0.f, 0.f};
      if (nxt) {
        const unsigned HM = (unsigned)((tid >> 8) * (N_MEL / 2));
        float acc = 0.f;
        if (ROLE_REGS) {
#pragma unroll
          for (int k = 0; k < N_MEL / 2; k += 4) {
            const float4 m = lds4(s_mel + HM + k);
            acc = fmaf(rw[ROLE_REGS ? k : 0], m.x, acc);
            acc = fmaf(rw[ROLE_REGS ? k + 1 : 0], m.y, acc);
            acc = fmaf(rw[ROLE_REGS ? k + 2 : 0], m.z, acc);
            acc = fmaf(rw[ROLE_REGS ? k + 3 : 0], m.w, acc);
          }
        } else {
#pragma unroll
          for (int k = 0; k < N_MEL / 2; k += 4) {
            const float4 w4 = lds4(s_W0 + 4u * (((HM + k) >> 2) * PRENET + (TID & 255u))), m = lds4(s_mel + HM + k);
            acc = fmaf(w4.x, m.x, acc);
            acc = fmaf(w4.y, m.y, acc);
            acc = fmaf(w4.z, m.z, acc);
            acc = fmaf(w4.w, m.w, acc);
          }
        }
        PROF_MARK(12);
        s_l1[TID] = acc;
        __syncthreads();
        PROF_MARK(13);
        float pk[4];
#pragma unroll
        for (int k = 0; k < 4; ++k) {
          const float v = fmaxf(s_l1[(L4 >> 2) + 64 * k] + s_l1[PRENET + (L4 >> 2) + 64 * k], 0.f);
          pk[k] = (drop1 >> k) & 1u ? 0.f : (d.dropout_mode ? 2.f * v : v);
        }
#pragma unroll
        for (int r = 0; r < 2; ++r) {
          float a = 0.f;
#pragma unroll
          for (int k = 0; k < 4; ++k) a = fmaf(w1r[r][k], pk[k], a);
          a = fmaxf(wave_sum(a), 0.f);
          xo[r] = (drop2 >> r) & 1u ? 0.f : (d.dropout_mode ? 2.f * a : a);
        }
      }
      PROF_MARK(14);
      if (lane < 2) s_mel[MEL_GL - 16 + wave + NW * lane] = lane ? xo[1] : xo[0];
      __syncthreads();
      if (tid < 16)
        publish(g.x + (unsigned)(((p ^ 1) * GS + rb) * PRENET + 16 * rk + tid), (want + 1u) | (nxt ? ACT_BIT : 0u),
                s_mel[MEL_GL - 16 + tid]);
    }
    PROF_MARK(10);
    }
  }
#ifdef XDTTS_PERSIST_PROFILE
  __syncthreads();
  if (g.prof && tid < 24) g.prof[c * 24 + tid] = s_prof[tid];
#endif

  if (cell) {
    d.att_c[cb * ATT_RNN + 4 * c + cu] = s_cell[tid];
    d.dec_c[cb * DEC_RNN + 4 * c + cu] = s_cell[4 * PB + tid];
    d.att_h[0][cb * ATT_RNN + 4 * c + cu] = s_cell[8 * PB + tid];
    d.dec_h[0][cb * DEC_RNN + 4 * c + cu] = s_cell[12 * PB + tid];
  }
  if (attn) {
    {
      const int col = tid & 63, q = tid >> 6;
      float acc = 0.f;
      for (int t = q; t < T; t += NW) acc = fmaf(s_aw[t], d.memory[((size_t)rb * T + t) * EMB + 64 * rk + col], acc);
      __syncthreads();
      s_part[tid] = acc;
      __syncthreads();
      if (tid < 64) {
        float v = 0.f;
#pragma unroll
        for (int u = 0; u < NW; ++u) v += s_part[u * 64 + tid];
        d.ctx[rb * EMB + 64 * rk + tid] = v;
      }
    }
    if (rk == 0 && tid < T) {
      d.aw[rb * T + tid] = s_aw[tid];
      d.awc[rb * T + tid] = s_awc[tid];
    }
  }
  if (c == 0 && tid == 0) d.ctl[0] = s;
}

__global__ void k_persist_seed(PersistBufs g, const int *limits, int B, unsigned words) {
  const int b = blockIdx.x, i = threadIdx.x;
  for (unsigned w = (unsigned)(b * PRENET + i); w < words; w += (unsigned)(B * PRENET)) g.x[w] = 0ull;
  publish(g.x + (size_t)b * PRENET + i, 1u | (limits[b] > 0 ? ACT_BIT : 0u), 0.f);
}

__global__ void k_persist_seed_at(PersistBufs g, const int *limits, const float *x, int step) {
  const int b = blockIdx.x, i = threadIdx.x;
  publish(g.x + (size_t)(((step & 1) * GS + b) * PRENET + i), (unsigned)(step + 1) | (limits[b] > step ? ACT_BIT : 0u), x[b * PRENET + i]);
}

__global__ void k_pack_ctx_rows(const float4 *__restrict__ att_w, const float4 *__restrict__ dec_w, const float4 *__restrict__ proj_w,
                                float4 *__restrict__ out) {
  const int n = blockIdx.x, q = threadIdx.x;
  float4 v = make_float4(0.f, 0.f, 0.f, 0.f);
  if (n < 4 * ATT_RNN) v = att_w[(size_t)n * (ATT_COLS / 4) + PRENET / 4 + q];
  else if (n < 4 * ATT_RNN + 4 * DEC_RNN) v = dec_w[(size_t)(n - 4 * ATT_RNN) * (DEC_COLS / 4) + ATT_RNN / 4 + q];
  else if (n <= 4 * ATT_RNN + 4 * DEC_RNN + N_MEL) v = proj_w[(size_t)(n - 4 * ATT_RNN - 4 * DEC_RNN) * (PROJ_IN / 4) + DEC_RNN / 4 + q];
  out[(size_t)n * (EMB / 4) + q] = v;
}

template <int PB, bool SKEW = false>
void launch_pb(const DecoderBufs &d, const PersistBufs &g, const PersistWeights &pw, int nsteps, hipStream_t s) {
  const void *fn = d.use_gate ? reinterpret_cast<const void *>(k_decoder_persistent<PB, SKEW, true>) : reinterpret_cast<const void *>(k_decoder_persistent<PB, SKEW, false>);
  COOP_CHECK(launch_coresident(true, fn, dim3(P_NCU), dim3(PT), 0, s, d, g, pw, nsteps));
}

}

void launch_pack_ctx_rows(const float *att_w, const float *dec_w, const float *proj_w, float *ctx_w, hipStream_t s) {
  static_assert(CTXF_ROWS >= 4 * ATT_RNN + 4 * DEC_RNN + N_MEL + 1 && CTXF_LD >= PERSIST_T_MAX, "context-fold table shape");
  hipLaunchKernelGGL(k_pack_ctx_rows, dim3(CTXF_ROWS), dim3(EMB / 4), 0, s, reinterpret_cast<const float4 *>(att_w),
                     reinterpret_cast<const float4 *>(dec_w), reinterpret_cast<const float4 *>(proj_w), reinterpret_cast<float4 *>(ctx_w));
  HIP_CHECK(hipGetLastError());
}

size_t persist_granule_words(int B) {
  (void)B;
  return (size_t)2 * GS * (PRENET + ATT_RNN + ATTN_CU * EP_LD + DEC_RNN + MEL_GL * MEL_ST);
}

PersistBufs persist_bufs(unsigned long long *base, int *err, int B) {
  PersistBufs g{};
  g.x = base;
  (void)B;
  g.hatt = g.x + (size_t)2 * GS * PRENET;
  g.ep = g.hatt + (size_t)2 * GS * ATT_RNN;
  g.hdec = g.ep + (size_t)2 * GS * ATTN_CU * EP_LD;
  g.mel = g.hdec + (size_t)2 * GS * DEC_RNN;
  g.err = err;
  g.lazy = PERSIST_LAZY_DEFAULT;
  g.xlazy = 0;
  g.clazy = 4;
  g.shrink = 0;
  g.spins = 0;
  g.fault = 0;
  g.slow = 0;
  g.pfirst = 0;
  g.xfirst = 4;
  g.efirst = 3;
  g.skew = 1;
  g.both_run = 0;
  g.first = 4;
  return g;
}

PersistBufs persist_view(const PersistBufs &g, int b0) {
  PersistBufs v = g;
  v.x += (size_t)b0 * PRENET;
  v.hatt += (size_t)b0 * ATT_RNN;
  v.ep += (size_t)b0 * ATTN_CU * EP_LD;
  v.hdec += (size_t)b0 * DEC_RNN;
  v.mel += (size_t)b0 * MEL_GL * MEL_ST;
  return v;
}

bool decoder_persistent_supported(int device, int B, int T) {
  if (B < 1 || B > PERSIST_B_MAX || T > PERSIST_T_MAX) return false;
  hipDeviceProp_t prop;
  if (hipGetDeviceProperties(&prop, device) != hipSuccess) return false;
  if (prop.multiProcessorCount < P_NCU) return false;
  int per_cu = 0;
  if (hipOccupancyMaxActiveBlocksPerMultiprocessor(&per_cu, k_decoder_persistent<PERSIST_B_MAX, false, true>, PT, 0) != hipSuccess)
    return false;
  return per_cu >= 1;
}

void launch_persist_seed(const DecoderBufs &d, const PersistBufs &g, const int *limits_dev, hipStream_t s) {
  hipLaunchKernelGGL(k_persist_seed, dim3(d.B), dim3(PRENET), 0, s, g, limits_dev, d.B, (unsigned)persist_granule_words(d.B));
  HIP_CHECK(hipGetLastError());
}

void launch_persist_seed_at(const DecoderBufs &d, const PersistBufs &g, const int *limits_dev, int step, hipStream_t s) {
  HIP_CHECK(hipMemsetAsync(g.x, 0, persist_granule_words(d.B) * sizeof(unsigned long long), s));
  hipLaunchKernelGGL(k_persist_seed_at, dim3(d.B), dim3(PRENET), 0, s, g, limits_dev, d.x, step);
  HIP_CHECK(hipGetLastError());
}

void launch_decoder_persistent(const DecoderBufs &d, const DeviceWeights &w, const PersistBufs &g, int nsteps,
                               hipStream_t s) {
  PersistWeights pw{};
  pw.att_w = reinterpret_cast<const float4 *>(w.att_w.p);
  pw.dec_w = reinterpret_cast<const float4 *>(w.dec_w.p);
  pw.q_w = reinterpret_cast<const float4 *>(w.q_w.p);
  pw.proj_w = reinterpret_cast<const float4 *>(w.proj_w.p);
  pw.att_b = w.att_b.p;
  pw.dec_b = w.dec_b.p;
  pw.v_w = w.v_w.p;
  pw.loc_fused = w.loc_fused.p;
  pw.proj_b = w.proj_b.p;
  pw.pre0T = w.pre0T.p;
  pw.pre1T = w.pre1T.p;
  switch (d.B) {
    case 1: launch_pb<1>(d, g, pw, nsteps, s); break;
    case 2:
      if (g.skew && (g.shrink || g.both_run)) launch_pb<2, true>(d, g, pw, nsteps, s);
      else launch_pb<2>(d, g, pw, nsteps, s);
      break;
    default: fail(XDTTS_ERR_BAD_ARG, "persistent decoder: %d chunks (max %d)", d.B, PERSIST_B_MAX);
  }
}

}
```

### xd-tts_amd/csrc/env.cpp

```cpp
#include "env.h"

#include <cstring>

namespace xdtts {
namespace env {

const Var table[N_VARS] = {
    {"XDTTS_DEVICE", Kind::product, When::handle},
    {"XDTTS_CHIP_LOCK_DIR", Kind::product, When::process},
    {"XDTTS_DECODER", Kind::product, When::request},
    {"XDTTS_GL", Kind::product, When::request},
    {"XDTTS_COOP", Kind::product, When::process},
    {"XDTTS_ATT_FUSED", Kind::form, When::handle},
    {"XDTTS_NO_EARLY", Kind::form, When::handle},
    {"XDTTS_NO_TAIL", Kind::form, When::handle},
    {"XDTTS_NO_CTXFOLD", Kind::form, When::handle},
    {"XDTTS_NO_SKEW", Kind::form, When::handle},
    {"XDTTS_P8", Kind::form, When::handle},
    {"XDTTS_GEMM_TILE", Kind::form, When::process},
    {"XDTTS_GEMM_SPLITK", Kind::form, When::process},
    {"XDTTS_GEMM_SPLIT_TILE", Kind::form, When::process},
    {"XDTTS_GL_BATCH_FORCE", Kind::form, When::request},
    {"XDTTS_ATT_SPINS", Kind::hook, When::request},
    {"XDTTS_ATT_FAULT", Kind::hook, When::request},
    {"XDTTS_ATT_SLOW", Kind::hook, When::request},
    {"XDTTS_TAIL_FAULT", Kind::hook, When::request},
    {"XDTTS_PERSIST_SPINS", Kind::hook, When::request},
    {"XDTTS_PERSIST_FAULT", Kind::hook, When::request},
    {"XDTTS_PERSIST_SLOW", Kind::hook, When::request},
    {"XDTTS_ENC_SPINS", Kind::hook, When::request},
    {"XDTTS_ENC_FAULT", Kind::hook, When::request},
    {"XDTTS_GL_SPINS", Kind::hook, When::request},
    {"XDTTS_GL_SLOW", Kind::hook, When::request},
    {"XDTTS_PERSIST_PROFILE", Kind::hook, When::request},
    {"XDTTS_GL_PROFILE", Kind::hook, When::request},
};

const char *raw(Id id) { return getenv(table[id].name); }
bool is_set(Id id) { return raw(id) != nullptr; }
bool equals(Id id, const char *v) {
  const char *e = raw(id);
  return e && std::strcmp(e, v) == 0;
}
int int_or(Id id, int unset) {
  const char *e = raw(id);
  return e ? atoi(e) : unset;
}
int coop_forced() {
  static const int forced = [] {
    const char *e = raw(COOP);
    return !e ? -1 : (e[0] == '0' ? 0 : 1);
  }();
  return forced;
}

}
}
```

### xd-tts_amd/csrc/env.h

```cpp
#pragma once
#include <cstdlib>

namespace xdtts {
namespace env {

enum Id {
  DEVICE, CHIP_LOCK_DIR, DECODER, GL, COOP,
  ATT_FUSED, NO_EARLY, NO_TAIL, NO_CTXFOLD, NO_SKEW, P8,
  GEMM_TILE, GEMM_SPLITK, GEMM_SPLIT_TILE, GL_BATCH_FORCE,
  ATT_SPINS, ATT_FAULT, ATT_SLOW, TAIL_FAULT,
  PERSIST_SPINS, PERSIST_FAULT, PERSIST_SLOW, ENC_SPINS, ENC_FAULT, GL_SPINS, GL_SLOW,
  PERSIST_PROFILE, GL_PROFILE,
  N_VARS
};
enum class Kind { product, form, hook };
enum class When { process, handle, request };
struct Var {
  const char *name;
  Kind kind;
  When when;
};
extern const Var table[N_VARS];

const char *raw(Id id);
bool is_set(Id id);
bool equals(Id id, const char *v);
int int_or(Id id, int unset);
template <class T>
void override_int(Id id, T *v) {
  if (const char *e = raw(id)) *v = (T)atoi(e);
}
int coop_forced();

}
}
```

### xd-tts_amd/csrc/kernels.h

```cpp
#pragma once
#include "common.h"
#include "weights.h"

namespace xdtts {

struct DecoderBufs {
  int B, T;
  const float *memory;
  const float *pmem;
  const int *n_valid;
  float *att_h[2];
  float *att_c;
  float *dec_h[2];
  float *dec_c;
  float *aw, *awc;
  float *ctx;
  float *x;
  float *loc;
  float *e_part;
  float *pmel;
  float *frames;
  float *gates;
  int *nframes;
  int *ctl;
  int max_steps;
  int use_gate;
  float gate_threshold;
  float gate_lo, gate_hi;
  int dropout_mode;
  uint32_t dropout_seed, item_base;
  const unsigned char *drop_masks;
  int drop_steps;
  float *xf, *ctxf, *att_hf[2], *dec_hf[2];
  int Bpad;
  float *awc2;
  const int *item_perm;
  const float *ctx_fold;
  const float *dec_in;
  const float *pmem_t;
  unsigned long long *ep_g;
  int *att_err;
  unsigned long long *hg;
  float *att_part;
  unsigned long long *hdg, *melg;
  float *dec_part;
  int att_spins, att_fault;
  int tail_fault;
  int att_slow;
};
constexpr int ATT_EXCHANGE_BLOCKS = 8;
void launch_dimgroup_transpose(const float *in, float *out, int B, int T, hipStream_t s);

void launch_decoder_steps(const DecoderBufs &d, const DeviceWeights &w, int nsteps, hipStream_t s);
void launch_decoder_step_at(const DecoderBufs &d, const DeviceWeights &w, int i, hipStream_t s);
void launch_decoder_advance(const DecoderBufs &d, int n, hipStream_t s);
void launch_decoder_early(const DecoderBufs &d, const DeviceWeights &w, int i, hipStream_t s);
bool decoder_two_launch(const DecoderBufs &d);
void launch_decoder_prologue(const DecoderBufs &d, const DeviceWeights &w, hipStream_t s);
void launch_decoder_location(const DecoderBufs &d, const DeviceWeights &w, hipStream_t s);
void launch_decoder_prenet(const DecoderBufs &d, const DeviceWeights &w, hipStream_t s);
void launch_frag_convert(float *rowmajor, float *frag, int B, int Bpad, int n, int dir, hipStream_t s);
void launch_decoder_flush(const DecoderBufs &d, const DeviceWeights &w, hipStream_t s);
size_t decoder_pmel_floats(int B);
void launch_decoder_init(const DecoderBufs &d, const int *limits_dev, hipStream_t s);

constexpr int CTXF_ROWS = 2 * 4096 + 128, CTXF_LD = 128;
void launch_pack_ctx_rows(const float *att_w, const float *dec_w, const float *proj_w, float *ctx_w, hipStream_t s);
constexpr int PERSIST_B_MAX = 2;
constexpr int PERSIST_T_MAX = 128;
struct PersistBufs {
  unsigned long long *x, *hatt, *ep, *hdec, *mel;
  int *err;
  int spins, fault;
  int slow;
  int skew;
  int both_run;
  int shrink;
  int first;
  int efirst;
  int xfirst;
  int pfirst;
  int xlazy, clazy;
  int lazy;
  unsigned long long *prof;
};
size_t persist_granule_words(int B);
PersistBufs persist_bufs(unsigned long long *base, int *err, int B);
PersistBufs persist_view(const PersistBufs &g, int b0);
bool decoder_persistent_supported(int device, int B, int T);
void launch_persist_seed(const DecoderBufs &d, const PersistBufs &g, const int *limits_dev, hipStream_t s);
void launch_persist_seed_at(const DecoderBufs &d, const PersistBufs &g, const int *limits_dev, int step, hipStream_t s);
void launch_decoder_persistent(const DecoderBufs &d, const DeviceWeights &w, const PersistBufs &g, int nsteps,
                               hipStream_t s);

constexpr int P8_B_MAX = 16;
constexpr int P8_STEPS_MAX = 16384;
struct P8Bufs {
  unsigned *rx, *rhatt, *rctx, *rhdec;
  unsigned long long *ep, *mel;
  int *err;
  int spins, fault;
  int delay[6];
  int ring_steps;
  unsigned long long *prof;
};
size_t p8_exchange_words(int B, int nsteps);
P8Bufs p8_bufs(unsigned long long *base, int *err, int B, int nsteps);
bool decoder_p8_supported(int device, int B, int T);
void launch_p8_seed(const DecoderBufs &d, const P8Bufs &g, const int *limits_dev, hipStream_t s);
void launch_p8_seed_at(const DecoderBufs &d, const P8Bufs &g, const int *limits_dev, int step, hipStream_t s);
void launch_decoder_p8(const DecoderBufs &d, const DeviceWeights &w, const P8Bufs &g, int nsteps, hipStream_t s);
struct P8Weights {
  const float4 *att_w, *dec_w, *q_w, *proj_w;
  const float *att_b, *dec_b, *v_w, *loc_fused, *proj_b, *pre0T, *pre1T;
};
bool decoder_p16_supported(int device, int T);
void launch_decoder_p16(const DecoderBufs &d, const P8Weights &w, const P8Bufs &g, int nsteps, hipStream_t s);

struct GemmArgs {
  const float *A;
  long lda, strideA;
  const float *W;
  const float *bias;
  float *C;
  long ldc, strideC;
  const float *R;
  long ldr, strideR;
  int M, N, K, batch;
  int ragged;
  int Mz[64];
  long Cz[64];
  int act;
  int transpose_out;
  int ldc_rows;
  float p;
  float alpha, beta;
  int r_before_act;
  int xcd_rows;
  int splitk;
  float *ws;
  unsigned *cnt;
  int tile;
};
int gemm_splitk_plan(const GemmArgs &g, size_t *ws_floats, size_t *tiles, int *tile);
constexpr int GEMM_RAGGED_MAX = 64;
void launch_gemm_nt(const GemmArgs &g, hipStream_t s);

void launch_embed(const int64_t *ids, const float *emb, float *xpad, int B, int T, int pad, hipStream_t s);
void launch_bilstm(const float *xproj, const float *whhT_fwd, const float *whhT_bwd, float *memory,
                   int B, int T, hipStream_t s);

size_t bilstm_coop_exchange_words(int B);
void launch_bilstm_coop(const float *xproj, const float *whhT_fwd, const float *whhT_bwd, float *memory,
                        unsigned long long *exchange, int *err, int B, int T, int group, hipStream_t s);

struct GlBufs {
  int F, n_fft, hop, nb;
  float *S;
  float2 *ang, *ang2;
  float2 *tprev;
  float *frames;
  float *wss_inv;
  const float2 *tw;
  const float *win;
};
constexpr int GLP_TF_MAX = 8;
struct GlSeg {
  int fbase;
  int F;
  int f0;
  int n_own;
  int first;
  int last;
  int abase;
  int pad;
};
struct GlPersist {
  const GlSeg *segs;
  unsigned long long *xch;
  int *err;
  unsigned epoch;
  int nblk, TF;
  int per_cu;
  int spins;
  int slow;
  int poll_delay;
  int gen_phase;
  unsigned seed;
  float2 *ang_out, *tprev_out;
  unsigned long long *prof;
};
bool gl_persistent_plan(int F, int n_cu, int *TF, int *nblk);
size_t gl_persistent_xch_words(int nblk);
bool gl_persistent_supported(int device, int *n_cu, int *per_cu4);
void launch_gl_persistent(const GlBufs &g, const GlPersist &p, const float2 *ang_in, const float2 *tprev_in, int n_iter,
                          float alpha, float *audio, hipStream_t s);
void launch_gl_exp_transpose(const float *mel_80xF, float *out_Fx80, int n_mels, int F, int mode, hipStream_t s);
void launch_gl_pow_rows(const float *in, int ld, float *out, int nb, int F, float p, hipStream_t s);
constexpr int GLN_PARTS = 64;
constexpr int GLN_SCRATCH = 2 * GLN_PARTS;
void launch_gl_output_normalise(float *y, const int2 *tab_dev, int n_utt, int first, int n_max, int mode, float target,
                                float *parts, hipStream_t s);
void launch_gl_phase_init(const GlBufs &g, uint32_t seed, const float *phase0_dev, hipStream_t s);
void launch_gl_phase_init_batch(const GlBufs &g, uint32_t seed, const int *frame_local, hipStream_t s);
void launch_gl_prepare(const GlBufs &g, hipStream_t s);
void launch_gl_iterations(const GlBufs &g, int n_iter, float alpha, float *audio, hipStream_t s);
const float2 *launch_gl_iterate(const GlBufs &g, int n_iter, float alpha, hipStream_t s);
void launch_gl_final(const GlBufs &g, const float2 *ang, float *audio, hipStream_t s);
void launch_gl_state_import(const GlBufs &g, const float *ang_in, const float *reb_in, hipStream_t s);
void launch_gl_state_export(const GlBufs &g, const float2 *ang, const float2 *tprev, float *ang_out, float *reb_out,
                            hipStream_t s);
void launch_transpose(const float *in, float *out, int rows, int cols, hipStream_t s);
void launch_copy_rows(const float *src, size_t src_stride, float *dst, size_t dst_stride, const int *rows, int n, int cols,
                      hipStream_t s);

struct AnSeg {
  long long abase;
  int n;
  int F;
  int f0;
  int row0;
};
void launch_stft_mag(const float *audio, const AnSeg *segs_dev, int nblk, const float2 *tw, const float *win, float *S, float *P,
                     int ldp, float e, hipStream_t s);
void launch_mel_compress(const float *melT, float *out_melsxF, int n_mels, int F, int mode, float floor, hipStream_t s);
constexpr int SPD_PARTS = 256;
void launch_spec_distance(const float *X, const float *St, size_t n, double *parts, double *sums, hipStream_t s);

}
```

### xd-tts_amd/csrc/tacotron2_decode.cpp

```cpp
#include <algorithm>

#include "tacotron2_handle.h"

using namespace xdtts;

struct xdtts_tacotron2::Decode {
  const DecoderBufs &d;
  const std::vector<int> &lim;
  int max_lim;
  const std::function<void()> *after;
  bool spec_ran;
  bool *after_ran;
};

int xdtts_tacotron2::run_decoder(const DecoderBufs &d, const std::vector<int> &lim, const std::function<void()> &after, bool *after_ran) {
  if (after_ran) *after_ran = false;
  if (lim_on_dev != lim || !limits.p) {
    limits.upload(lim.data(), lim.size(), stream);
    lim_on_dev = lim;
  }
  launch_decoder_init(d, limits.p, stream);
  launch_decoder_prologue(d, w, stream);
  Decode dc{d, lim, *std::max_element(lim.begin(), lim.end()), after && !d.use_gate ? &after : nullptr, false, after_ran};
  auto attempt = [&](int (xdtts_tacotron2::*engine)(Decode &), void (xdtts_tacotron2::*refused)()) {
// ... 28 lines not shown
  int steps = 0;
  bool as_planned = true;
  for (int b = 0; b < dc.d.B; ++b) {
    steps = std::max(steps, host_ctl[HOST_NF + b]);
    as_planned = as_planned && host_ctl[HOST_NF + b] == dc.lim[b];
  }
  if (dc.after_ran) *dc.after_ran = dc.spec_ran && as_planned;
  return steps;
}

int xdtts_tacotron2::decode_again(Decode &dc, bool refused) {
  dc.spec_ran = false;
  if (refused) HIP_CHECK(hipStreamSynchronize(stream));
  HIP_CHECK(hipMemsetAsync(dec_err.p, 0, sizeof(int), stream));
  launch_decoder_init(dc.d, limits.p, stream);
  return -1;
}

bool xdtts_tacotron2::small_batch_eligible(int B, int T, int max_steps) const {
  if (B < 3 || B > P8_B_MAX || T > PERSIST_T_MAX || max_steps > P8_STEPS_MAX) return false;
  return !env::equals(env::DECODER, "launch");
}
bool xdtts_tacotron2::small_batch_engine(int B, int T, int max_steps) {
  if (!small_batch_eligible(B, T, max_steps)) return false;
  p8_gate.ensure_probed([&] {
    return p8_wanted && decoder_p8_supported(device, 8, PERSIST_T_MAX) && decoder_p8_supported(device, P8_B_MAX, PERSIST_T_MAX);
  });
  return p8_gate.usable() && pair_gate.state != EngineGate::OFF;
}
void xdtts_tacotron2::small_batch_tick(int B, int T, int max_steps) {
  if (!small_batch_eligible(B, T, max_steps)) return;
  (void)small_batch_engine(B, T, max_steps);
  if (p8_gate.tick() && pair_gate.state == EngineGate::OFF && pair_gate.probe_ok) {
    pair_gate.state = EngineGate::ON;
    pair_gate.demoted_calls = 0;
  }
}

int xdtts_tacotron2::decode_small_batch(Decode &dc) {
  const DecoderBufs &d = dc.d;
  if (d.xf) return -1;
  small_batch_tick(d.B, d.T, dc.max_lim);
  if (!small_batch_engine(d.B, d.T, dc.max_lim)) return -1;
  try {
    dec_exchange.alloc(p8_exchange_words(d.B, dc.max_lim));
  } catch (const Error &e) {
    if (e.code != XDTTS_ERR_OOM) throw;
    (void)hipGetLastError();
    return -1;
  }
  std::lock_guard<ChipLock> lk(chip_mutex(device));
  P8Bufs g8 = p8_bufs(dec_exchange.p, dec_err.p, d.B, dc.max_lim);
  env::override_int(env::PERSIST_SPINS, &g8.spins);
  env::override_int(env::PERSIST_FAULT, &g8.fault);
  launch_p8_seed(d, g8, limits.p, stream);
  launch_decoder_p8(d, w, g8, dc.max_lim, stream);
  fetch(dc, true);
  if (!host_ctl[HOST_DEC_ERR]) return finish(dc);
  p8_gate.demote();
  pair_gate.ensure_probed([&] { return decoder_persistent_supported(device, PERSIST_B_MAX, PERSIST_T_MAX); });
  pair_gate.demote();
  std::fprintf(stderr, "libxdtts_hip: persistent MFMA decoder exchange timed out (grid not co-resident); this handle now "
                       "uses the launch-per-stage decoder (probed again after %d calls)\n", EngineGate::PROBE_AFTER);
  return decode_again(dc, false);
}
void xdtts_tacotron2::small_batch_refused() {
  p8_gate.refuse();
  std::fprintf(stderr, "libxdtts_hip: persistent MFMA decoder launch refused by the runtime; this handle decodes small batches "
                       "with its other engines\n");
}

bool xdtts_tacotron2::use_persistent(const DecoderBufs &d) {
  if (d.xf || d.B > 2 * PERSIST_B_MAX || d.T > PERSIST_T_MAX) return false;
  if (env::equals(env::DECODER, "launch")) return false;
  pair_gate.ensure_probed([&] { return decoder_persistent_supported(device, PERSIST_B_MAX, PERSIST_T_MAX); });
  pair_gate.tick();
  return pair_gate.usable();
}

int xdtts_tacotron2::decode_pairs(Decode &dc) {
  const DecoderBufs &d = dc.d;
  const std::vector<int> &lim = dc.lim;
  if (!use_persistent(d)) return -1;
  std::lock_guard<ChipLock> lk(chip_mutex(device));
  const float *fold = nullptr;
  if (ctx_fold_table && w.ctx_w.p) {
    ctx_fold.alloc((size_t)d.B * CTXF_ROWS * CTXF_LD);
    GemmArgs fg{};
    fg.A = d.memory;
    fg.lda = EMB;
    fg.strideA = (long)d.T * EMB;
    fg.W = w.ctx_w.p;
    fg.C = ctx_fold.p;
    fg.ldc = CTXF_LD;
    fg.strideC = (long)CTXF_ROWS * CTXF_LD;
    fg.M = d.T;
    fg.N = CTXF_ROWS;
    fg.K = EMB;
    fg.batch = d.B;
    fg.transpose_out = 1;
    launch_gemm_nt(fg, stream);
    fold = ctx_fold.p;
  }
  auto view = [&](int b0, int n) {
    DecoderBufs v = d;
    v.B = n;
    v.ctx_fold = fold ? fold + (size_t)b0 * CTXF_ROWS * CTXF_LD : nullptr;
    v.memory += (size_t)b0 * d.T * EMB;
    v.pmem += (size_t)b0 * d.T * ATT_DIM;
    v.n_valid += b0;
    for (int i = 0; i < 2; ++i) {
      v.att_h[i] = d.att_h[0] + (size_t)b0 * ATT_RNN;
      v.dec_h[i] = d.dec_h[0] + (size_t)b0 * DEC_RNN;
    }
    v.att_c += (size_t)b0 * ATT_RNN;
    v.dec_c += (size_t)b0 * DEC_RNN;
    v.aw += (size_t)b0 * d.T;
    v.awc += (size_t)b0 * d.T;
    v.ctx += (size_t)b0 * EMB;
    v.frames += (size_t)b0 * d.max_steps * N_MEL;
    v.gates += (size_t)b0 * d.max_steps;
    v.nframes += b0;
    v.item_base += (uint32_t)b0;
    if (v.drop_masks) v.drop_masks += (size_t)b0 * d.drop_steps * 2 * PRENET;
    return v;
  };
  for (int b0 = 0; b0 < d.B; b0 += PERSIST_B_MAX) {
    const int n = std::min(PERSIST_B_MAX, d.B - b0);
    const DecoderBufs v = view(b0, n);
    int sub_lim = 0;
    for (int b = 0; b < n; ++b) sub_lim = std::max(sub_lim, lim[b0 + b]);
    dec_exchange.alloc(persist_granule_words(n));
    PersistBufs g = persist_bufs(dec_exchange.p, dec_err.p, n);
    if (!pair_skew) g.skew = 0;
    env::override_int(env::PERSIST_SPINS, &g.spins);
    env::override_int(env::PERSIST_FAULT, &g.fault);
    env::override_int(env::PERSIST_SLOW, &g.slow);
    g.shrink = n == 2 ? 1 : 0;
    if (g.shrink && !d.use_gate && lim[b0] == lim[b0 + 1]) {
      g.shrink = 0;
      g.both_run = 1;
    }
#ifdef XDTTS_PERSIST_PROFILE
    static DevBuf<unsigned long long> prof;
    prof.alloc(256 * 24);
    g.prof = prof.p;
#endif
    if (b0 > 0) HIP_CHECK(hipMemsetAsync(d.ctl, 0, sizeof(int), stream));
    launch_persist_seed(v, g, limits.p + b0, stream);
    if (g.shrink && !d.use_gate && lim[b0] != lim[b0 + 1]) {
      const int first = std::min(lim[b0], lim[b0 + 1]), r = lim[b0] > lim[b0 + 1] ? 0 : 1;
      g.shrink = 0;
      g.both_run = 1;
      launch_decoder_persistent(v, w, g, first, stream);
      launch_decoder_persistent(view(b0 + r, 1), w, persist_view(g, r), lim[b0 + r] - first, stream);
    } else {
      launch_decoder_persistent(v, w, g, sub_lim, stream);
      if (g.shrink) {
        for (int r = 0; r < n; ++r) {
          PersistBufs g1 = persist_view(g, r);
          g1.shrink = 0;
          launch_decoder_persistent(view(b0 + r, 1), w, g1, lim[b0 + r], stream);
        }
      }
    }
#ifdef XDTTS_PERSIST_PROFILE
    if (const char *path = env::raw(env::PERSIST_PROFILE)) {
      std::vector<unsigned long long> hp(256 * 24);
      HIP_CHECK(hipMemcpyAsync(hp.data(), prof.p, hp.size() * 8, hipMemcpyDeviceToHost, stream));
      HIP_CHECK(hipStreamSynchronize(stream));
      if (FILE *f = fopen(path, "w")) {
        for (int c = 0; c < 256; ++c) {
          for (int i = 0; i < 24; ++i) fprintf(f, "%llu ", hp[c * 24 + i]);
          fprintf(f, "\n");
        }
        fclose(f);
      }
    }
#endif
  }
  fetch(dc, true);
  if (!host_ctl[HOST_DEC_ERR]) return finish(dc);
  pair_gate.demote();
  std::fprintf(stderr, "libxdtts_hip: persistent decoder exchange timed out (grid not co-resident); "
                       "this handle now uses the launch-per-stage decoder (probed again after %d calls)\n", EngineGate::PROBE_AFTER);
  return decode_again(dc, false);
}
void xdtts_tacotron2::pairs_refused() {
  pair_gate.refuse();
  std::fprintf(stderr, "libxdtts_hip: persistent decoder launch refused by the runtime; this handle uses the "
                       "launch-per-stage decoder\n");
}

void xdtts_tacotron2::replay_steps(const DecoderBufs &d) {
  graph.replay(&d, sizeof d, stream, [&] { launch_decoder_steps(d, w, GRAPH_STEPS, stream); });
}

int xdtts_tacotron2::decode_launches(Decode &dc) {
  const DecoderBufs &d = dc.d;
  const int max_lim = dc.max_lim;
  int launched = 0;
  std::unique_lock<ChipLock> chip;
  if (d.hg) chip = std::unique_lock<ChipLock>(chip_mutex(device));
  if (!d.use_gate) {
    while (launched + GRAPH_STEPS <= max_lim) {
      replay_steps(d);
      launched += GRAPH_STEPS;
    }
    if (launched < max_lim) {
      int r = max_lim - launched;
      r += r & 1;
      launch_decoder_steps(d, w, r, stream);
      launched += r;
    }
    launch_decoder_flush(d, w, stream);
    fetch(dc, true);
  } else {
    const int check_every = 3 * GRAPH_STEPS;
    for (;;) {
      for (int i = 0; i < check_every && launched < max_lim; i += GRAPH_STEPS) {
        replay_steps(d);
        launched += GRAPH_STEPS;
      }
      fetch(dc, false);
      int need = 0;
      for (int b = 0; b < d.B; ++b) need = std::max(need, host_ctl[HOST_NF + b]);
      if (host_ctl[0] >= need || launched >= max_lim) break;
    }
    launch_decoder_flush(d, w, stream);
    fetch(dc, true);
  }
  if (d.ep_g && host_ctl[HOST_DEC_ERR]) {
    HIP_CHECK(hipMemsetAsync(dec_err.p, 0, sizeof(int), stream));
    att_gate.demote();
    std::fprintf(stderr, "libxdtts_hip: batched attention exchange timed out; this handle now uses the "
                         "separate attention kernels (probed again after %d batches)\n", EngineGate::PROBE_AFTER);
    DecoderBufs d2 = d;
    d2.ep_g = nullptr;
    d2.hg = nullptr;
    d2.att_part = nullptr;
    d2.hdg = d2.melg = nullptr;
    d2.dec_part = nullptr;
    return run_decoder(d2, dc.lim);
  }
  return finish(dc);
}
```

### xd-tts_amd/csrc/tacotron2_handle.cpp

```cpp
#include "tacotron2_handle.h"

#include <algorithm>
#include <cmath>

using namespace xdtts;

xdtts_tacotron2::~xdtts_tacotron2() {
  if (fetched) (void)hipEventDestroy(fetched);
  if (host_ctl) (void)hipHostFree(host_ctl);
  if (in_host) (void)hipHostFree(in_host);
  if (stream) (void)hipStreamDestroy(stream);
}

void xdtts_tacotron2::init(int dev) {
  device = dev;
  select_device(dev);
  HIP_CHECK(hipStreamCreateWithFlags(&stream, hipStreamNonBlocking));
  ev.create();
  HIP_CHECK(hipEventCreateWithFlags(&fetched, hipEventDisableTiming));
  HIP_CHECK(hipHostMalloc((void **)&host_ctl, sizeof(int) * CTL_INTS, hipHostMallocDefault));
  int cus = 0;
  HIP_CHECK(hipDeviceGetAttribute(&cus, hipDeviceAttributeMultiprocessorCount, dev));
  coop_group = cus / 8 < 1 ? 1 : cus / 8;
  n_cu = cus;
  ctlblk.alloc(CTL_INTS);
  HIP_CHECK(hipMemsetAsync(ctlblk.p, 0, sizeof(int) * CTL_INTS, stream));
  ctl.p = ctlblk.p;
  enc_err.p = ctlblk.p + HOST_ENC_ERR;
  dec_err.p = ctlblk.p + HOST_DEC_ERR;
  nframes.p = ctlblk.p + HOST_NF;
  w.upload(blob, stream);
}

void xdtts_tacotron2::run_gemm(GemmArgs &g) {
  size_t wsf = 0, tiles = 0;
  int tile = 0;
  const int sk = gemm_splitk_plan(g, &wsf, &tiles, &tile);
  if (sk > 1) {
    if (tiles > gemm_cnt.n) {
      gemm_cnt.alloc(std::max<size_t>(tiles, 4096));
      HIP_CHECK(hipMemsetAsync(gemm_cnt.p, 0, gemm_cnt.n * sizeof(unsigned), stream));
    }
    gemm_ws.alloc(wsf);
    g.splitk = sk;
    g.tile = tile;
    g.ws = gemm_ws.p;
    g.cnt = gemm_cnt.p;
  }
  launch_gemm_nt(g, stream);
}

void xdtts_tacotron2::run_encoder(int B, int T) {
  const int pad = (ENC_K - 1) / 2, TP = T + 2 * pad;
  const size_t padded = (size_t)B * TP * EMB;
  xpadA.alloc(padded);
  xpadB.alloc(padded);
  xproj.alloc((size_t)2 * B * T * 4 * ENC_H);
  memory.alloc((size_t)B * T * EMB);
  pmem.alloc((size_t)B * T * ATT_DIM);
  if (xpad_zero[0] != xpadA.p || xpad_zero[1] != xpadB.p || xpad_B != B || xpad_T != T) {
    HIP_CHECK(hipMemsetAsync(xpadA.p, 0, padded * sizeof(float), stream));
    HIP_CHECK(hipMemsetAsync(xpadB.p, 0, padded * sizeof(float), stream));
    xpad_zero[0] = xpadA.p;
    xpad_zero[1] = xpadB.p;
    xpad_B = B;
    xpad_T = T;
  }
  launch_embed(ids.p, w.emb.p, xpadA.p, B, T, pad, stream);
  float *src = xpadA.p, *dst = xpadB.p;
  for (int i = 0; i < ENC_CONVS; ++i) {
    GemmArgs g{};
    g.A = src;
    g.lda = EMB;
    g.strideA = (long)TP * EMB;
    g.W = w.enc_conv[i].w.p;
    g.bias = w.enc_conv[i].b.p;
    g.C = dst + (size_t)pad * EMB;
    g.ldc = EMB;
    g.strideC = (long)TP * EMB;
    g.M = T;
    g.N = EMB;
    g.K = ENC_K * EMB;
    g.batch = B;
    g.act = 1;
    run_gemm(g);
    std::swap(src, dst);
  }
  for (int d = 0; d < 2; ++d) {
    GemmArgs g{};
    g.A = src + (size_t)pad * EMB;
    g.lda = EMB;
    g.strideA = (long)TP * EMB;
    g.W = w.enc_wih[d].p;
    g.bias = w.enc_bias[d].p;
    g.C = xproj.p + (size_t)d * B * T * 4 * ENC_H;
    g.ldc = 4 * ENC_H;
    g.strideC = (long)T * 4 * ENC_H;
    g.M = T;
    g.N = 4 * ENC_H;
    g.K = EMB;
    g.batch = B;
    run_gemm(g);
  }
  enc_gate.ensure_probed([] { return true; });
  enc_gate.tick();
  bool coop_ran = false;
  if (enc_gate.usable()) {
    const int slots = B > coop_group ? (B + 1) / 2 : B;
    const int launches = (slots + coop_group - 1) / coop_group, group = B > coop_group ? coop_group : (B + launches - 1) / launches;
    enc_exchange.alloc(bilstm_coop_exchange_words(2 * group));
    try {
      launch_bilstm_coop(xproj.p, w.enc_whhT[0].p, w.enc_whhT[1].p, memory.p, enc_exchange.p, enc_err.p, B, T, group,
                         stream);
      coop_ran = true;
    } catch (const CoopRefused &) {
      enc_gate.refuse();
      std::fprintf(stderr, "libxdtts_hip: cooperative encoder BiLSTM launch refused by the runtime; this handle uses the "
                           "single-workgroup recurrence\n");
    }
  }
  if (!coop_ran) launch_bilstm(xproj.p, w.enc_whhT[0].p, w.enc_whhT[1].p, memory.p, B, T, stream);
  GemmArgs g{};
  g.A = memory.p;
  g.lda = EMB;
  g.strideA = (long)T * EMB;
  g.W = w.mem_w.p;
  g.C = pmem.p;
  g.ldc = ATT_DIM;
  g.strideC = (long)T * ATT_DIM;
  g.M = T;
  g.N = ATT_DIM;
  g.K = EMB;
  g.batch = B;
  run_gemm(g);
}

void xdtts_tacotron2::upload_dropout_masks(const xdtts_infer_opts &o, int B, const int *lim) {
  if (o.dropout_mode < 0 || o.dropout_mode > 2) fail(XDTTS_ERR_BAD_ARG, "dropout_mode %d out of range (0 off, 1 seeded, 2 explicit)", o.dropout_mode);
  if (o.dropout_mode != 2) return;
  if (!o.dropout_masks || o.dropout_mask_steps <= 0) fail(XDTTS_ERR_BAD_ARG, "dropout_mode 2 needs dropout_masks and dropout_mask_steps");
  for (int b = 0; b < B; ++b)
    if (lim[b] > o.dropout_mask_steps)
      fail(XDTTS_ERR_BAD_ARG, "chunk %d may run %d steps, the dropout masks cover %d", b, lim[b], o.dropout_mask_steps);
  drop_dev.upload(o.dropout_masks, (size_t)B * o.dropout_mask_steps * 2 * PRENET, stream);
}

DecoderBufs xdtts_tacotron2::decoder_bufs(int B, int T, const float *mem, const float *pm, const xdtts_infer_opts &o, int force_batched) {
  const bool batched = force_batched < 0 ? B >= BATCH_MFMA_MIN : force_batched != 0;
  const int ms = o.max_steps;
  att_h.alloc((size_t)2 * B * ATT_RNN);
  att_c.alloc((size_t)((B + 15) / 16 * 16) * ATT_RNN);
  dec_h.alloc((size_t)2 * B * DEC_RNN);
  dec_c.alloc((size_t)((B + 15) / 16 * 16) * DEC_RNN);
  aw.alloc((size_t)B * T);
  awc.alloc((size_t)B * T);
  ctx.alloc((size_t)B * EMB);
  x.alloc((size_t)B * PRENET);
  loc.alloc((size_t)B * T * ATT_DIM);
  e_part.alloc((size_t)B * (ATT_DIM / 4) * T);
  pmel.alloc(decoder_pmel_floats(B));
  frames.alloc((size_t)B * ms * N_MEL);
  gates.alloc((size_t)B * ms);
  DecoderBufs d{};
  d.B = B;
  d.T = T;
  d.memory = mem;
  d.pmem = pm;
  d.n_valid = n_valid.p;
  d.att_h[0] = att_h.p;
  d.att_h[1] = att_h.p + (size_t)B * ATT_RNN;
  d.att_c = att_c.p;
  d.dec_h[0] = dec_h.p;
  d.dec_h[1] = dec_h.p + (size_t)B * DEC_RNN;
  d.dec_c = dec_c.p;
  d.aw = aw.p;
  d.awc = awc.p;
  d.ctx = ctx.p;
  d.x = x.p;
  d.loc = loc.p;
  d.e_part = e_part.p;
  d.pmel = pmel.p;
  d.frames = frames.p;
  d.gates = gates.p;
  d.nframes = nframes.p;
  d.ctl = ctl.p;
  d.max_steps = ms;
  d.use_gate = o.fixed_steps > 0 ? 0 : 1;
  d.gate_threshold = o.gate_threshold;
  {
    const double t = (double)o.gate_threshold;
    d.gate_lo = -INFINITY;
    d.gate_hi = INFINITY;
    if (t > 1e-3 && t < 1.0 - 1e-3) {
      const double L = std::log(t / (1.0 - t)), w = 1e-3 * (1.0 + std::fabs(L));
      d.gate_lo = (float)(L - w);
      d.gate_hi = (float)(L + w);
    }
  }
  d.dropout_mode = o.dropout_mode;
  d.dropout_seed = o.dropout_seed;
  d.item_base = o.item_base;
  if (o.dropout_mode == 2) {
    d.drop_masks = drop_dev.p;
    d.drop_steps = o.dropout_mask_steps;
  }
  if (batched) {
    const int Bpad = (B + 15) / 16 * 16;
    frag.alloc((size_t)Bpad * (PRENET + EMB + 2 * ATT_RNN + 2 * DEC_RNN) + (size_t)B * T);
    d.Bpad = Bpad;
    d.xf = frag.p;
    d.ctxf = d.xf + (size_t)Bpad * PRENET;
    d.att_hf[0] = d.ctxf + (size_t)Bpad * EMB;
    d.att_hf[1] = d.att_hf[0] + (size_t)Bpad * ATT_RNN;
    d.dec_hf[0] = d.att_hf[1] + (size_t)Bpad * ATT_RNN;
    d.dec_hf[1] = d.dec_hf[0] + (size_t)Bpad * DEC_RNN;
    d.awc2 = d.dec_hf[1] + (size_t)Bpad * DEC_RNN;
    pmem_t.alloc((size_t)B * T * ATT_DIM);
    launch_dimgroup_transpose(pm, pmem_t.p, B, T, stream);
    d.pmem_t = pmem_t.p;
    att_gate.ensure_probed([] { return true; });
    if (att_gate.tick()) att_form = env::int_or(env::ATT_FUSED, 2);
    if (att_fused() > 0 && T <= T_MAX) {
      const size_t ne = (size_t)B * ATT_EXCHANGE_BLOCKS * T;
      att_exchange.alloc(ne + (size_t)B * ATT_RNN);
      d.ep_g = att_exchange.p;
      d.att_err = dec_err.p;
      if (att_fused() > 1 && B <= 64 && n_cu >= ATT_RNN / 4) {
        d.hg = att_exchange.p + ne;
        if (early_partial) {
          att_part.alloc((size_t)(ATT_RNN / 4) * 4 * 64 * 4);
          d.att_part = att_part.p;
          if (two_launch && T <= PERSIST_T_MAX) {
            tail_exchange.alloc((size_t)B * (DEC_RNN + 96));
            d.hdg = tail_exchange.p;
            d.melg = d.hdg + (size_t)B * DEC_RNN;
            dec_part.alloc((size_t)(DEC_RNN / 4) * 4 * 64 * 4);
            d.dec_part = dec_part.p;
          }
        }
      }
      env::override_int(env::ATT_SPINS, &d.att_spins);
      env::override_int(env::ATT_FAULT, &d.att_fault);
      env::override_int(env::TAIL_FAULT, &d.tail_fault);
      env::override_int(env::ATT_SLOW, &d.att_slow);
    }
  }
  return d;
}

void xdtts_tacotron2::run_postnet(const float *frames_dev, size_t frame_stride, const int *F, const long *col_off, int n, float *out,
                                  long ldc, bool dense_items) {
  const int pad = (POST_K - 1) / 2;
  int Fmax = 0;
  for (int i = 0; i < n; ++i) Fmax = std::max(Fmax, F[i]);
  const size_t FP = (size_t)Fmax + 2 * pad, slot = FP * POST_CH, slot0 = FP * N_MEL;
  pp0.alloc(slot0 * n);
  ppA.alloc(slot * n);
  ppB.alloc(slot * n);
  {
    std::vector<long> sig{(long)n, (long)Fmax, (long)(size_t)pp0.p, (long)(size_t)ppA.p, (long)(size_t)ppB.p};
    for (int z = 0; z < n; ++z) sig.push_back(F[z]);
    if (sig != pp_sig) {
      HIP_CHECK(hipMemsetAsync(pp0.p, 0, slot0 * n * sizeof(float), stream));
      HIP_CHECK(hipMemsetAsync(ppA.p, 0, slot * n * sizeof(float), stream));
      HIP_CHECK(hipMemsetAsync(ppB.p, 0, slot * n * sizeof(float), stream));
      pp_sig = sig;
    }
  }
  launch_copy_rows(frames_dev, frame_stride, pp0.p + (size_t)pad * N_MEL, slot0, F, n, N_MEL, stream);
  float *src = pp0.p, *dst = ppA.p;
  for (int i = 0; i < POST_CONVS; ++i) {
    const ConvGemm &c = w.post_conv[i];
    const bool last = i == POST_CONVS - 1;
    GemmArgs g{};
    g.A = src;
    g.lda = c.ci;
    g.strideA = (long)(i == 0 ? slot0 : slot);
    g.W = c.w.p;
    g.bias = c.b.p;
    g.M = Fmax;
    g.N = c.co;
    g.K = c.k * c.ci;
    g.batch = n;
    g.ragged = 1;
    for (int z = 0; z < n; ++z) {
      g.Mz[z] = F[z];
      g.Cz[z] = last ? col_off[z] : 0;
    }
    if (!last) {
      g.C = dst + (size_t)pad * c.co;
      g.ldc = c.co;
      g.strideC = (long)slot;
      g.act = 2;
    } else {
      g.C = out;
      g.ldc = ldc;
      g.transpose_out = 1;
      g.ldc_rows = dense_items ? 1 : 0;
      g.R = frames_dev;
      g.ldr = N_MEL;
      g.strideR = (long)frame_stride;
    }
    run_gemm(g);
    if (i == 0) src = ppB.p;
    std::swap(src, dst);
  }
}

std::vector<int> xdtts_tacotron2::infer_batch_device(const int64_t *ids_host, const int *lens, int B, int T, const xdtts_infer_opts &o,
                                                     const int *fixed_per_item, int *F_total, bool per_chunk) {
  if (B <= 0 || B > 4096) fail(XDTTS_ERR_BAD_ARG, "batch %d out of range", B);
  if (T <= 0 || T > T_MAX) fail(XDTTS_ERR_BAD_ARG, "window %d out of range (1..%d)", T, T_MAX);
  if (o.max_steps <= 0 || o.max_steps > 100000) fail(XDTTS_ERR_BAD_ARG, "max_steps %d out of range", o.max_steps);
  for (int b = 0; b < B; ++b) {
    if (lens[b] <= 0) fail(XDTTS_ERR_BAD_ARG, "chunk %d is empty", b);
// ... 164 lines not shown
```

### xd-tts_amd/csrc/tacotron2_handle.h

```cpp
#pragma once
#include <functional>

#include "engine_gate.h"
#include "kernels.h"
#include "runtime.h"

struct xdtts_tacotron2 {
  using DecoderBufs = xdtts::DecoderBufs;
  using EngineGate = xdtts::EngineGate;
  template <class T>
  using DevBuf = xdtts::DevBuf<T>;
  int device = 0;
  hipStream_t stream = nullptr;
  mutable std::mutex mu;
  std::vector<float> blob;
  xdtts::DeviceWeights w;
  xdtts::Events ev;
  float last_ms[4] = {0, 0, 0, 0};
  int last_steps = 0;

  template <class T>
  struct DevSlot {
    T *p = nullptr;
    DevBuf<T> own;
    void upload(const T *src, size_t count, hipStream_t s) {
      own.upload(src, count, s);
      p = own.p;
    }
  };
  DevSlot<int64_t> ids;
  DevSlot<int> n_valid, limits;
  DevBuf<unsigned char> in_blk;
  unsigned char *in_host = nullptr;
  size_t in_host_bytes = 0;
  std::vector<int> lim_on_dev;
  struct IntRef {
    int *p = nullptr;
  };
  DevBuf<int> ctlblk;
  IntRef ctl, enc_err, dec_err, nframes;
  DevBuf<float> xpadA, xpadB, xproj, memory, pmem;
  const float *xpad_zero[2] = {nullptr, nullptr};
  int xpad_B = 0, xpad_T = 0;
  DevBuf<unsigned long long> enc_exchange;
  DevBuf<unsigned long long> dec_exchange;
  DevBuf<float> ctx_fold;
  DevBuf<unsigned long long> att_exchange;
  DevBuf<float> att_part;
  DevBuf<float> dec_part;
  DevBuf<unsigned long long> tail_exchange;
  int n_cu = 0;
  EngineGate pair_gate;
  EngineGate p8_gate;
  EngineGate enc_gate;
  EngineGate att_gate;
  int att_form = xdtts::env::int_or(xdtts::env::ATT_FUSED, 2);
  int att_fused() const { return att_gate.state == EngineGate::OFF ? 0 : att_form; }
  bool early_partial = !xdtts::env::is_set(xdtts::env::NO_EARLY);
  bool ctx_fold_table = !xdtts::env::is_set(xdtts::env::NO_CTXFOLD);
  bool pair_skew = !xdtts::env::is_set(xdtts::env::NO_SKEW);
  bool p8_wanted = [] { const char *p = xdtts::env::raw(xdtts::env::P8); return !(p && p[0] == '0'); }();
  bool two_launch = !xdtts::env::is_set(xdtts::env::NO_TAIL);
  int coop_group = 16;
  DevBuf<float> att_h, att_c, dec_h, dec_c, aw, awc, ctx, x, loc, e_part, pmel, frames, gates;
  DevBuf<float> frag;
  DevBuf<float> pmem_t;
  DevSlot<int> item_perm;
  DevBuf<float> dec_in_dev;
  DevBuf<unsigned char> drop_dev;
  DevBuf<float> state_stage;
  DevBuf<float> pp0, ppA, ppB, mel_dev;
  std::vector<long> pp_sig;
  std::function<void()> before_decoder;
  std::function<void()> while_decoding;
  int *host_ctl = nullptr;
  static constexpr int HOST_ENC_ERR = 2, HOST_DEC_ERR = 3, HOST_NF = 4, CTL_INTS = HOST_NF + 4096;


  static constexpr int GRAPH_STEPS = 20;
  xdtts::GraphCache graph;

  hipEvent_t fetched = nullptr;
  DevBuf<float> gemm_ws;
  DevBuf<unsigned> gemm_cnt;

  ~xdtts_tacotron2();
  void init(int dev);
  void run_gemm(xdtts::GemmArgs &g);
  void run_encoder(int B, int T);
  void upload_dropout_masks(const xdtts_infer_opts &o, int B, const int *lim);
  DecoderBufs decoder_bufs(int B, int T, const float *mem, const float *pm, const xdtts_infer_opts &o, int force_batched = -1);
  void run_postnet(const float *frames_dev, size_t frame_stride, const int *F, const long *col_off, int n, float *out, long ldc,
                   bool dense_items = false);
  std::vector<int> infer_batch_device(const int64_t *ids_host, const int *lens, int B, int T, const xdtts_infer_opts &o,
                                      const int *fixed_per_item, int *F_total, bool per_chunk = false);
  void check_encoder_exchange();
  void finish_timings();

  int run_decoder(const DecoderBufs &d, const std::vector<int> &lim, const std::function<void()> &after = {}, bool *after_ran = nullptr);
  bool small_batch_eligible(int B, int T, int max_steps) const;
  void small_batch_tick(int B, int T, int max_steps);
  bool small_batch_engine(int B, int T, int max_steps);
  bool use_persistent(const DecoderBufs &d);

 private:
  struct Decode;
  void replay_steps(const DecoderBufs &d);
  void fetch(Decode &dc, bool last);
  int finish(Decode &dc);
  int decode_again(Decode &dc, bool refused);
  int decode_small_batch(Decode &dc);
  int decode_pairs(Decode &dc);
  int decode_launches(Decode &dc);
  void small_batch_refused();
  void pairs_refused();
};

namespace xdtts {
void chunks_from_splits(const int64_t *ids, size_t n, const size_t *splits, size_t n_splits, int T, std::vector<int64_t> &padded,
                        std::vector<int> &lens);
std::vector<int64_t> pad_batch_ids(const int64_t *ids, const int32_t *lens, int B, int t_stride, int T);
xdtts_infer_opts resolve_opts(const xdtts_infer_opts *opts);
}
```

Before: 130,200.

## Continue surviving chunk inside persistent pair kernel instead of relaunching

```diff
diff --git a/include/xdtts.h b/include/xdtts.h
--- a/include/xdtts.h
+++ b/include/xdtts.h
@@ -100,6 +100,9 @@
                                           int32_t *encoder_cooperative, int32_t *batched_attention);
 xdtts_status xdtts_tacotron2_engine_reset(xdtts_tacotron2 *h);
 xdtts_status xdtts_tacotron2_small_batch_engine_state(const xdtts_tacotron2 *h, int32_t *state);
+xdtts_status xdtts_tacotron2_last_decoder_state(xdtts_tacotron2 *h, int32_t B, int32_t T, float *attention_hidden,
+                                                float *attention_cell, float *decoder_hidden, float *decoder_cell,
+                                                float *attention_weights, float *attention_weights_cum, float *attention_context);
 
 const char *xdtts_build_info(void);
 
diff --git a/xd-tts_amd/__init__.py b/xd-tts_amd/__init__.py
--- a/xd-tts_amd/__init__.py
+++ b/xd-tts_amd/__init__.py
@@ -66,6 +66,7 @@
     "xdtts_tacotron2_decoder_steps": (_I32, [_VP, _I32, _I32, _VP, _VP, _I32, _VP, C.POINTER(InferOpts), _U32, _I32] + [_VP] * 10),
     "xdtts_tacotron2_engine_state": (_I32, [_VP, C.POINTER(_I32), C.POINTER(_I32), C.POINTER(_I32)]),
     "xdtts_tacotron2_small_batch_engine_state": (_I32, [_VP, C.POINTER(_I32)]),
+    "xdtts_tacotron2_last_decoder_state": (_I32, [_VP, _I32, _I32] + [_VP] * 7),
     "xdtts_tacotron2_engine_reset": (_I32, [_VP]),
     "xdtts_tacotron2_postnet": (_I32, [_VP, _VP, _I32, _VP]),
     "xdtts_tacotron2_last_timings": (_I32, [_VP, C.POINTER(C.c_float * 4), C.POINTER(_I32)]),
@@ -443,6 +444,13 @@
                                                  step0, n_steps, _ptr(din), *[_ptr(st[k]) for k in names], _ptr(out), _ptr(gate)))
         return out, gate, st
 
+    def last_decoder_state(self, B, T):
+        shapes = {"attention_hidden": 1024, "attention_cell": 1024, "decoder_hidden": 1024, "decoder_cell": 1024,
+                  "attention_weights": T, "attention_weights_cum": T, "attention_context": 512}
+        st = {k: np.empty((B, n), dtype=np.float32) for k, n in shapes.items()}
+        _check(lib.xdtts_tacotron2_last_decoder_state(self._h, B, T, *[_ptr(st[k]) for k in shapes]))
+        return st
+
     def engine_state(self):
         a, b, c = C.c_int32(), C.c_int32(), C.c_int32()
         _check(lib.xdtts_tacotron2_engine_state(self._h, C.byref(a), C.byref(b), C.byref(c)))
diff --git a/xd-tts_amd/csrc/api_tacotron2.cpp b/xd-tts_amd/csrc/api_tacotron2.cpp
--- a/xd-tts_amd/csrc/api_tacotron2.cpp
+++ b/xd-tts_amd/csrc/api_tacotron2.cpp
@@ -427,6 +427,28 @@
   });
 }
 
+xdtts_status xdtts_tacotron2_last_decoder_state(xdtts_tacotron2 *h, int32_t B, int32_t T, float *attention_hidden, float *attention_cell,
+                                                float *decoder_hidden, float *decoder_cell, float *attention_weights,
+                                                float *attention_weights_cum, float *attention_context) {
+  return guard([&] {
+    if (!h || !attention_hidden || !attention_cell || !decoder_hidden || !decoder_cell || !attention_weights || !attention_weights_cum || !attention_context)
+      fail(XDTTS_ERR_BAD_ARG, "null argument");
+    std::lock_guard<std::mutex> lk(h->mu);
+    if (B <= 0 || T <= 0 || B != h->state_B || T != h->state_T) fail(XDTTS_ERR_BAD_ARG, "no decoder state of %d chunks x %d encoder steps on this handle", B, T);
+    HIP_CHECK(hipSetDevice(h->device));
+    hipStream_t st = h->stream;
+    auto down = [&](float *dst, const float *src, size_t n) { HIP_CHECK(hipMemcpyAsync(dst, src, n * sizeof(float), hipMemcpyDeviceToHost, st)); };
+    down(attention_hidden, h->att_h.p, (size_t)B * ATT_RNN);
+    down(attention_cell, h->att_c.p, (size_t)B * ATT_RNN);
+    down(decoder_hidden, h->dec_h.p, (size_t)B * DEC_RNN);
+    down(decoder_cell, h->dec_c.p, (size_t)B * DEC_RNN);
+    down(attention_weights, h->aw.p, (size_t)B * T);
+    down(attention_weights_cum, h->awc.p, (size_t)B * T);
+    down(attention_context, h->ctx.p, (size_t)B * EMB);
+    HIP_CHECK(hipStreamSynchronize(st));
+  });
+}
+
 xdtts_status xdtts_tacotron2_engine_reset(xdtts_tacotron2 *h) {
   return guard([&] {
     if (!h) fail(XDTTS_ERR_BAD_ARG, "null handle");
diff --git a/xd-tts_amd/csrc/decoder_persistent.hip b/xd-tts_amd/csrc/decoder_persistent.hip
--- a/xd-tts_amd/csrc/decoder_persistent.hip
+++ b/xd-tts_amd/csrc/decoder_persistent.hip
@@ -204,6 +204,7 @@
     s_act[tid] = 0;
     s_act[2 + tid] = step0 < d.nframes[tid];
   }
+  if (tid == PT - 1) s_act[4] = 0;
 #pragma unroll
   for (int b = 0; b < PB; ++b) {
 #pragma unroll
@@ -256,25 +257,21 @@
     }
     nf_r = d.nframes[rb];
   }
-  constexpr bool ROLE_REGS = PB == 1;
-  float rw[ROLE_REGS ? 40 : 1];
-  if (ROLE_REGS) {
-#pragma unroll
-    for (int k = 0; k < 40; ++k) rw[ROLE_REGS ? k : 0] = 0.f;
+  float4 rw[10];
+  if (PB == 1) {
+#pragma unroll
+    for (int k = 0; k < 10; ++k) rw[k] = make_float4(0.f, 0.f, 0.f, 0.f);
     if (attn) {
 #pragma unroll
       for (int r = 0; r < 2; ++r)
 #pragma unroll
-        for (int j = 0; j < 4; ++j) {
-          const float4 q = w.q_w[(unsigned)((16 * rk + wave + NW * r) * (ATT_RNN / 4) + lane + 64 * j)];
-          rw[ROLE_REGS ? 16 * r + 4 * j + 0 : 0] = q.x;
-          rw[ROLE_REGS ? 16 * r + 4 * j + 1 : 0] = q.y;
-          rw[ROLE_REGS ? 16 * r + 4 * j + 2 : 0] = q.z;
-          rw[ROLE_REGS ? 16 * r + 4 * j + 3 : 0] = q.w;
-        }
+        for (int j = 0; j < 4; ++j) rw[4 * r + j] = w.q_w[(unsigned)((16 * rk + wave + NW * r) * (ATT_RNN / 4) + lane + 64 * j)];
     } else if (pre) {
 #pragma unroll
-      for (int k = 0; k < N_MEL / 2; ++k) rw[ROLE_REGS ? k : 0] = w.pre0T[(unsigned)(((tid >> 8) * (N_MEL / 2) + k) * PRENET + (tid & 255))];
+      for (int k = 0; k < N_MEL / 8; ++k) {
+        const unsigned at = (unsigned)(((tid >> 8) * (N_MEL / 2) + 4 * k) * PRENET + (tid & 255));
+        rw[k] = make_float4(w.pre0T[at], w.pre0T[at + PRENET], w.pre0T[at + 2 * PRENET], w.pre0T[at + 3 * PRENET]);
+      }
     }
   }
   float w1r[2][4];
@@ -341,9 +338,10 @@
   }
 
   float aacc[PB][2], dacc[PB][2];
-  auto att_bulk = [&](unsigned L4, bool all) {
+  auto att_bulk = [&](unsigned L4, bool all, int lo, int hi) {
 #pragma unroll
     for (int b = 0; b < PB; ++b) {
+      if (b < lo || b >= hi) continue;
       if (!all && !s_act[b]) continue;
       const float w0 = wreg[b][0], w1 = wreg[b][1];
       float a0 = fmaf(pma[b][0][1], w1, pma[b][0][0] * w0), a1 = fmaf(pma[b][1][1], w1, pma[b][1][0] * w0);
@@ -358,9 +356,10 @@
       chunk_fence();
     }
   };
-  auto dec_bulk_h = [&](unsigned L4, bool all) {
+  auto dec_bulk_h = [&](unsigned L4, bool all, int lo, int hi) {
 #pragma unroll
     for (int b = 0; b < PB; ++b) {
+      if (b < lo || b >= hi) continue;
       if (!all && !s_act[b]) continue;
       float a0 = 0.f, a1 = 0.f;
 #pragma unroll
@@ -401,8 +400,8 @@
     }
     __syncthreads();
   };
-  att_bulk(L4, true);
-  dec_bulk_h(L4, true);
+  att_bulk(L4, true, 0, PB);
+  dec_bulk_h(L4, true, 0, PB);
   if (attn) location(tid);
 
 #ifdef XDTTS_PERSIST_PROFILE
@@ -413,10 +412,328 @@
 #endif
   int s = step0;
   const int s_stop = step0 + nsteps;
+  const int tid_k = tid;
+  const bool lag = g.slow && c == g.slow - 1;
+  const bool attn_w = attn, pre_w = pre;
+  int surv = -1;
+  auto step = [&](auto NBc, auto R0c, int s) __attribute__((always_inline)) -> bool {
+    constexpr int NB = decltype(NBc)::value, R0 = decltype(R0c)::value;
+    constexpr bool ROLE_REGS = NB == 1;
+    static_assert(NB >= 1 && R0 + NB <= PB, "chunk range of a step");
+    const int tid = tid_k + (int)opaque(0u), lane = tid & 63, wave = tid >> 6;
+    const unsigned L4 = 4u * (unsigned)lane, TID = (unsigned)tid;
+    const int cb = tid >> 2, cu = tid & 3;
+    const bool cell = tid < 4 * PB && cb >= R0 && cb < R0 + NB;
+    auto wr = [&](int h) { return NB == 1 ? wreg[R0][h] : (rb ? wreg[PB - 1][h] : wreg[0][h]); };
+    const bool attn = attn_w && rb >= R0 && rb < R0 + NB, pre = pre_w && rb >= R0 && rb < R0 + NB;
+    const int prow = rk + 16 * wave;
+    const bool prow_ok = pre && wave < 6 && prow <= N_MEL;
+    const int p = s & 1;
+    const unsigned want = (unsigned)(s + 1);
+    straggle(lag, s, 0);
+    PROF_MARK(0);
+    {
+      const int b0 = R0 + (tid >> 8), i = tid & 255;
+      const bool need[2] = {b0 < R0 + NB && s_act[2 + (b0 < R0 + NB ? b0 : R0)] != 0, false};
+      float v[2];
+      unsigned tg[2];
+      lazy_wait(pre ? g.xfirst : g.xlazy);
+      const unsigned np_ = gather<2>(g.x, (unsigned)((p * GS + b0) * PRENET + i), 2u * PRENET, want, need, v, tg, pc);
+      PROF_POLLS(0, np_);
+#pragma unroll
+      for (int j = 0; j < 2; ++j)
+        if (need[j]) {
+          s_x[(b0 + 2 * j) * PRENET + i] = v[j];
+          if (i == 0) s_act[b0 + 2 * j] = (tg[j] & ACT_BIT) ? 1 : 0;
+        }
+      if (tid == PT - 1) s_act[4] = __hip_atomic_load(g.err, __ATOMIC_RELAXED, __HIP_MEMORY_SCOPE_AGENT);
+    }
+    __syncthreads();
+    bool act[PB], any = false;
+#pragma unroll
+    for (int b = R0; b < R0 + NB; ++b) {
+      act[b] = s_act[b] != 0;
+      any = any || act[b];
+    }
+    if (tid >= R0 && tid < R0 + NB) s_act[2 + tid] = s_act[tid];
+    PROF_MARK(1);
+    PROF_WHEN(2);
+    if (!any || s_act[4] != 0) return false;
+    if constexpr (NB == 2)
+      if (g.shrink && !(act[0] && act[1])) return false;
+    const bool act_r = s_act[rb] != 0;
+#pragma unroll
+    for (int b = R0; b < R0 + NB; ++b)
+      if (act[b]) {
+        const float4 v = lds4(s_x + b * PRENET + L4);
+        const float a0 = wave_sum(dot4(wa[0][0], v, aacc[b][0]));
+        const float a1 = wave_sum(dot4(wa[1][0], v, aacc[b][1]));
+        if (lane == 0) {
+          s_g[b * 16 + wave] = a0 + s_bias[wave];
+          s_g[b * 16 + wave + NW] = a1 + s_bias[wave + NW];
+        }
+      }
+    __syncthreads();
+    if (cell && s_act[cb]) {
+      const float *gp = s_g + cb * 16 + 4 * cu;
+      const float ig = fast_sigmoid(gp[0]), fg = fast_sigmoid(gp[1]), gg = fast_tanh(gp[2]), og = fast_sigmoid(gp[3]);
+      const float cn = fmaf(fg, s_cell[tid], ig * gg), hn = og * fast_tanh(cn);
+      publish(g.hatt + (unsigned)((p * GS + cb) * ATT_RNN + 4 * c + cu), want, hn);
+      s_cell[tid] = cn;
+      s_cell[8 * PB + tid] = hn;
+    }
+    PROF_MARK(2);
+    PROF_WHEN(0);
+    straggle(lag, s, 1);
+    __builtin_amdgcn_sched_barrier(0);
+    float4 lp4 = make_float4(0.f, 0.f, 0.f, 0.f), v4 = lp4;
+    if (attn && act_r) {
+      const float4 l4 = lds4(s_loc + 4 * TID), p4 = lds4(s_pm + 4 * TID);
+      lp4 = make_float4(l4.x + p4.x, l4.y + p4.y, l4.z + p4.z, l4.w + p4.w);
+      v4 = lds4(s_vv + 4 * (tid & 3));
+    }
+    {
+      bool need[2 * NB];
+#pragma unroll
+      for (int i = 0; i < 2 * NB; ++i) need[i] = act[R0 + (i >> 1)];
+      float v[2 * NB];
+      unsigned tg[2 * NB];
+      lazy_wait(attn ? g.first : g.lazy);
+      const unsigned np_ = gather<2 * NB>(g.hatt, (unsigned)((p * GS + R0) * ATT_RNN + tid), PT, want, need, v, tg, pc);
+      PROF_POLLS(1, np_);
+#pragma unroll
+      for (int i = 0; i < 2 * NB; ++i)
+        if (need[i]) s_hatt[R0 * ATT_RNN + TID + PT * i] = v[i];
+    }
+    __syncthreads();
+    PROF_MARK(3);
+    if (attn && act_r) {
+      float q0 = 0.f, q1 = 0.f;
+#pragma unroll
+      for (int j = 0; j < 4; ++j) {
+        const float4 v = lds4(s_hatt + rb * ATT_RNN + 256 * j + L4);
+        if constexpr (ROLE_REGS) {
+          q0 = dot4(rw[j], v, q0);
+          q1 = dot4(rw[4 + j], v, q1);
+        } else {
+          q0 = dot4(lds4(s_qw + 4 * (j * PT + TID)), v, q0);
+          q1 = dot4(lds4(s_qw + 4 * ((4 + j) * PT + TID)), v, q1);
+        }
+      }
+      q0 = wave_sum(q0);
+      q1 = wave_sum(q1);
+      if (lane == 0) {
+        s_q[wave] = q0;
+        s_q[wave + NW] = q1;
+      }
+      __syncthreads();
+      PROF_MARK(15);
+      const int t = tid >> 2, dq = 4 * (tid & 3);
+      const float4 q4 = lds4(s_q + dq);
+      float e = v4.x * fast_tanh(q4.x + lp4.x);
+      e = fmaf(v4.y, fast_tanh(q4.y + lp4.y), e);
+      e = fmaf(v4.z, fast_tanh(q4.z + lp4.z), e);
+      e = fmaf(v4.w, fast_tanh(q4.w + lp4.w), e);
+      e += dpp_move<0xB1, 0xf>(0.f, e);
+      e += dpp_move<0x4E, 0xf>(0.f, e);
+      if ((tid & 3) == 0 && t < T) publish(g.ep + (unsigned)(((p * GS + rb) * ATTN_CU + rk) * EP_LD + t), want, e);
+    }
+#pragma unroll
+    for (int b = R0; b < R0 + NB; ++b)
+      if (act[b]) {
+        float a0 = dacc[b][0], a1 = dacc[b][1];
+#pragma unroll
+        for (int k = 0; k < 4; ++k) {
+          const float4 v = lds4(s_hatt + b * ATT_RNN + 256 * k + L4);
+          a0 = dot4(wd[0][k], v, a0);
+          a1 = dot4(wd[1][k], v, a1);
+        }
+        dacc[b][0] = a0;
+        dacc[b][1] = a1;
+        chunk_fence();
+      }
+    PROF_MARK(4);
+    straggle(lag, s, 2);
+    __builtin_amdgcn_sched_barrier(0);
+    {
+      const int t = tid >> 2, j = tid & 3;
+      bool need[2 * NB];
+#pragma unroll
+      for (int i = 0; i < 2 * NB; ++i) need[i] = act[R0 + (i >> 1)] && t < T;
+      float v[2 * NB];
+      unsigned tg[2 * NB];
+      lazy_wait(attn ? g.efirst : g.clazy);
+      const unsigned np_ = gather<2 * NB>(g.ep, (unsigned)(((p * GS + R0) * ATTN_CU + j) * EP_LD + t), 4u * EP_LD, want, need, v, tg, pc);
+      PROF_POLLS(2, np_);
+#pragma unroll
+      for (int b = R0; b < R0 + NB; ++b) {
+        float e = v[2 * (b - R0)] + v[2 * (b - R0) + 1];
+        e += dpp_move<0xB1, 0xf>(0.f, e);
+        e += dpp_move<0x4E, 0xf>(0.f, e);
+        if (j == 0 && act[b]) s_e[b * TP + t] = (t < T && t < nv[b]) ? e : -INFINITY;
+      }
+    }
+    __syncthreads();
+    PROF_MARK(5);
+    PROF_WHEN(3);
+#pragma unroll
+    for (int b = R0; b < R0 + NB; ++b)
+      if (act[b]) {
+        const float e0 = s_e[b * TP + lane], e1 = s_e[b * TP + lane + 64];
+        const float m = wave_max(fmaxf(e0, e1));
+        const float x0 = fast_exp(e0 - m), x1 = fast_exp(e1 - m);
+        const float rs = __builtin_amdgcn_rcpf(wave_sum(x0 + x1));
+        wreg[b][0] = x0 * rs;
+        wreg[b][1] = x1 * rs;
+      }
+    if (attn && act_r && wave == 0) {
+      s_aw[lane] = wr(0);
+      s_awc[lane] += wr(0);
+      s_aw[lane + 64] = wr(1);
+      s_awc[lane + 64] += wr(1);
+    }
+    PROF_MARK(6);
+    straggle(lag, s, 3);
+    __builtin_amdgcn_sched_barrier(0);
+#pragma unroll
+    for (int b = R0; b < R0 + NB; ++b)
+      if (act[b]) {
+        const float w0 = wreg[b][0], w1 = wreg[b][1];
+        float a0 = fmaf(pmd[b][0][1], w1, fmaf(pmd[b][0][0], w0, dacc[b][0]));
+        float a1 = fmaf(pmd[b][1][1], w1, fmaf(pmd[b][1][0], w0, dacc[b][1]));
+        a0 = wave_sum(a0);
+        a1 = wave_sum(a1);
+        if (lane == 0) {
+          s_g[b * 16 + wave] = a0 + s_bias[16 + wave];
+          s_g[b * 16 + wave + NW] = a1 + s_bias[16 + wave + NW];
+        }
+      }
+    __syncthreads();
+    if (cell && s_act[cb]) {
+      const float *gp = s_g + cb * 16 + 4 * cu;
+      const float ig = fast_sigmoid(gp[0]), fg = fast_sigmoid(gp[1]), gg = fast_tanh(gp[2]), og = fast_sigmoid(gp[3]);
+      const float cn = fmaf(fg, s_cell[4 * PB + tid], ig * gg), hn = og * fast_tanh(cn);
+      publish(g.hdec + (unsigned)((p * GS + cb) * DEC_RNN + 4 * c + cu), want, hn);
+      s_cell[4 * PB + tid] = cn;
+      s_cell[12 * PB + tid] = hn;
+    }
+    att_bulk(L4, false, R0, R0 + NB);
+    PROF_MARK(7);
+    PROF_WHEN(1);
+    straggle(lag, s, 4);
+    __builtin_amdgcn_sched_barrier(0);
+    unsigned drop1 = 0u, drop2 = 0u;
+    if (pre && act_r) {
+      if (d.dropout_mode) {
+#pragma unroll
+        for (int k = 0; k < 4; ++k)
+          drop1 |= (prenet_dropped(d.dropout_mode, d.dropout_seed, item, d.drop_masks, d.drop_steps, rb, s + 1, 0, lane + 64 * k) ? 1u : 0u) << k;
+#pragma unroll
+        for (int r = 0; r < 2; ++r)
+          drop2 |= (prenet_dropped(d.dropout_mode, d.dropout_seed, item, d.drop_masks, d.drop_steps, rb, s + 1, 1, 16 * rk + wave + NW * r) ? 1u : 0u) << r;
+      }
+    }
+    {
+      bool need[2 * NB];
+#pragma unroll
+      for (int i = 0; i < 2 * NB; ++i) need[i] = act[R0 + (i >> 1)];
+      float v[2 * NB];
+      unsigned tg[2 * NB];
+      lazy_wait(pre ? g.pfirst : g.lazy);
+      const unsigned np_ = gather<2 * NB>(g.hdec, (unsigned)((p * GS + R0) * DEC_RNN + tid), PT, want, need, v, tg, pc);
+      PROF_POLLS(3, np_);
+#pragma unroll
+      for (int i = 0; i < 2 * NB; ++i)
+        if (need[i]) s_hdec[R0 * DEC_RNN + TID + PT * i] = v[i];
+    }
+    __syncthreads();
+    PROF_MARK(8);
+    if (prow_ok && act_r) {
+      float a = 0.f;
+#pragma unroll
+      for (int j = 0; j < 4; ++j) a = dot4(lds4(s_pw + 4 * (j * PT + TID)), lds4(s_hdec + rb * DEC_RNN + 256 * j + L4), a);
+      a = fmaf(pmp[1], wr(1), fmaf(pmp[0], wr(0), a));
+      a = wave_sum(a);
+      if (lane == 0) publish(g.mel + (unsigned)(((p * GS + rb) * MEL_GL + prow) * MEL_ST), want, a + s_pb[wave]);
+    }
+    dec_bulk_h(L4, false, R0, R0 + NB);
+    if (attn && act_r) location(tid);
+    PROF_MARK(9);
+    straggle(lag, s, 5);
+    __builtin_amdgcn_sched_barrier(0);
+    if (pre && act_r) {
+      bool nxt = false;
+      if (act_r) {
+        if (tid < N_MEL + 1) {
+          const bool need[1] = {true};
+          float v[1];
+          unsigned tg[1];
+          gather<1>(g.mel, (unsigned)(((p * GS + rb) * MEL_GL + tid) * MEL_ST), 0, want, need, v, tg, pc);
+          s_mel[tid] = v[0];
+        }
+        __syncthreads();
+        PROF_MARK(11);
+        const float gate = s_mel[N_MEL];
+        const bool fired = GATE ? gate_fires(gate, d.gate_lo, d.gate_hi, d.gate_threshold) : (d.use_gate && gate_sigmoid(gate) > d.gate_threshold);
+        if (rk == 0) {
+          if (tid < N_MEL) d.frames[((size_t)rb * d.max_steps + s) * N_MEL + tid] = s_mel[tid];
+          if (tid == 0) {
+            d.gates[(size_t)rb * d.max_steps + s] = gate;
+            if (fired) d.nframes[rb] = s + 1;
+          }
+        }
+        if (fired) nf_r = s + 1;
+        nxt = s + 1 < nf_r;
+      }
+      float xo[2] = {0.f, 0.f};
+      if (nxt) {
+        const unsigned HM = (unsigned)((tid >> 8) * (N_MEL / 2));
+        float acc = 0.f;
+#pragma unroll
+        for (int k = 0; k < N_MEL / 2; k += 4) {
+          const float4 m = lds4(s_mel + HM + k);
+          float4 w4;
+          if constexpr (ROLE_REGS) w4 = rw[k >> 2];
+          else w4 = lds4(s_W0 + 4u * (((HM + k) >> 2) * PRENET + (TID & 255u)));
+          acc = fmaf(w4.x, m.x, acc);
+          acc = fmaf(w4.y, m.y, acc);
+          acc = fmaf(w4.z, m.z, acc);
+          acc = fmaf(w4.w, m.w, acc);
+        }
+        PROF_MARK(12);
+        s_l1[TID] = acc;
+        __syncthreads();
+        PROF_MARK(13);
+        float pk[4];
+#pragma unroll
+        for (int k = 0; k < 4; ++k) {
+          const float v = fmaxf(s_l1[(L4 >> 2) + 64 * k] + s_l1[PRENET + (L4 >> 2) + 64 * k], 0.f);
+          pk[k] = (drop1 >> k) & 1u ? 0.f : (d.dropout_mode ? 2.f * v : v);
+        }
+#pragma unroll
+        for (int r = 0; r < 2; ++r) {
+          float a = 0.f;
+#pragma unroll
+          for (int k = 0; k < 4; ++k) a = fmaf(w1r[r][k], pk[k], a);
+          a = fmaxf(wave_sum(a), 0.f);
+          xo[r] = (drop2 >> r) & 1u ? 0.f : (d.dropout_mode ? 2.f * a : a);
+        }
+      }
+      PROF_MARK(14);
+      if (lane < 2) s_mel[MEL_GL - 16 + wave + NW * lane] = lane ? xo[1] : xo[0];
+      __syncthreads();
+      if (tid < 16)
+        publish(g.x + (unsigned)(((p ^ 1) * GS + rb) * PRENET + 16 * rk + tid), (want + 1u) | (nxt ? ACT_BIT : 0u),
+                s_mel[MEL_GL - 16 + tid]);
+    }
+    PROF_MARK(10);
+    return true;
+  };
+  auto I0 = std::integral_constant<int, 0>{};
+  auto I1 = std::integral_constant<int, 1>{};
+  auto IPB = std::integral_constant<int, PB>{};
   if constexpr (SKEW) {
     static_assert(PB == 2, "the skewed loop is the pair kernel");
-    const int tid_k = tid;
-    const bool lag = g.slow && c == g.slow - 1;
     unsigned drop1 = 0u, drop2 = 0u;
     u64 pf[2] = {0ull, 0ull};
     auto issue_x = [&](auto B, int s) {
@@ -443,8 +760,6 @@
       pf[0] = (pre && rb == b && tid < N_MEL + 1) ? peek(g.mel + (unsigned)((((s & 1) * GS + b) * MEL_GL + tid) * MEL_ST)) : 0ull;
       pf[1] = 0ull;
     };
-    auto I0 = std::integral_constant<int, 0>{};
-    auto I1 = std::integral_constant<int, 1>{};
     auto att_bulk1 = [&](auto B, unsigned L4) {
       constexpr int b = decltype(B)::value;
       const float w0 = wreg[b][0], w1 = wreg[b][1];
@@ -755,6 +1070,7 @@
       PROF_MARK(5 * b + 4);
     };
     bool tail1 = false;
+    surv = s_act[2] != 0 ? 0 : (s_act[3] != 0 ? 1 : -1);
     if (s_act[2] != 0 && s_act[3] != 0) {
       issue_x(I0, s);
       for (;; ++s) {
@@ -766,7 +1082,10 @@
           ph5(I1, s - 1, [&] { if (a0) issue_ep(I0, s); });
           tail1 = false;
         }
-        if (!a0) break;
+        if (!a0) {
+          surv = 1;
+          break;
+        }
         ph3(I0, s, [&] { issue_x(I1, s); });
         const bool a1 = ph1(I1, s, [&] { issue_h(g.hdec, I0, s); });
         if (!a1) issue_h(g.hdec, I0, s);
@@ -775,328 +1094,45 @@
         ph5(I0, s, [&] { if (a1) issue_ep(I1, s); });
         if (!a1) {
           ++s;
+          surv = 0;
           break;
         }
         ph3(I1, s, [&] { issue_x(I0, s + 1); });
         tail1 = true;
       }
     }
-  } else
-  for (; s < s_stop; ++s) {
-    const int tid_it = tid + (int)opaque(0u);
-    {
-    const int tid = tid_it, lane = tid & 63, wave = tid >> 6;
-    const unsigned L4 = 4u * (unsigned)lane, TID = (unsigned)tid;
-    const int cb = tid >> 2, cu = tid & 3;
-    const bool cell = tid < 4 * PB;
-    const int prow = rk + 16 * wave;
-    const bool prow_ok = pre && wave < 6 && prow <= N_MEL;
-    const int p = s & 1;
-    const unsigned want = (unsigned)(s + 1);
-    const bool lag = g.slow && c == g.slow - 1;
-    straggle(lag, s, 0);
-    PROF_MARK(0);
-    {
-      const int b0 = tid >> 8, i = tid & 255;
-      const bool need[2] = {b0 < PB && s_act[2 + (b0 < PB ? b0 : 0)] != 0, false};
-      float v[2];
-      unsigned tg[2];
-      lazy_wait(pre ? g.xfirst : g.xlazy);
-      const unsigned np_ = gather<2>(g.x, (unsigned)((p * GS + b0) * PRENET + i), 2u * PRENET, want, need, v, tg, pc);
-      PROF_POLLS(0, np_);
-#pragma unroll
-      for (int j = 0; j < 2; ++j)
-        if (need[j]) {
-          s_x[(b0 + 2 * j) * PRENET + i] = v[j];
-          if (i == 0) s_act[b0 + 2 * j] = (tg[j] & ACT_BIT) ? 1 : 0;
-        }
-      if (tid == PT - 1) s_act[4] = __hip_atomic_load(g.err, __ATOMIC_RELAXED, __HIP_MEMORY_SCOPE_AGENT);
+  } else {
+    while (s < s_stop && step(IPB, I0, s)) ++s;
+    if constexpr (PB == 2) {
+      __syncthreads();
+      surv = s_act[0] != 0 ? 0 : (s_act[1] != 0 ? 1 : -1);
+    }
+  }
+  if constexpr (PB == 2) {
+    int r = -1, s_end = s_stop;
+    if (GATE) {
+      if (g.cont) r = surv;
+    } else if (g.tail > 0 && s == s_stop) {
+      r = g.tail_slot;
+      s_end = s_stop + g.tail;
     }
     __syncthreads();
-    bool act[PB], any = false;
-#pragma unroll
-    for (int b = 0; b < PB; ++b) {
-      act[b] = s_act[b] != 0;
-      any = any || act[b];
-    }
-    if (tid < PB) s_act[2 + tid] = s_act[tid];
-    PROF_MARK(1);
-    PROF_WHEN(2);
-    if (!any || s_act[4] != 0 || (PB == 2 && g.shrink && !(act[0] && act[1]))) break;
-    const bool act_r = s_act[rb] != 0;
-#pragma unroll
-    for (int b = 0; b < PB; ++b)
-      if (act[b]) {
-        const float4 v = lds4(s_x + b * PRENET + L4);
-        const float a0 = wave_sum(dot4(wa[0][0], v, aacc[b][0]));
-        const float a1 = wave_sum(dot4(wa[1][0], v, aacc[b][1]));
-        if (lane == 0) {
-          s_g[b * 16 + wave] = a0 + s_bias[wave];
-          s_g[b * 16 + wave + NW] = a1 + s_bias[wave + NW];
-        }
-      }
-    __syncthreads();
-    if (cell && s_act[cb]) {
-      const float *gp = s_g + cb * 16 + 4 * cu;
-      const float ig = fast_sigmoid(gp[0]), fg = fast_sigmoid(gp[1]), gg = fast_tanh(gp[2]), og = fast_sigmoid(gp[3]);
-      const float cn = fmaf(fg, s_cell[tid], ig * gg), hn = og * fast_tanh(cn);
-      publish(g.hatt + (unsigned)((p * GS + cb) * ATT_RNN + 4 * c + cu), want, hn);
-      s_cell[tid] = cn;
-      s_cell[8 * PB + tid] = hn;
-    }
-    PROF_MARK(2);
-    PROF_WHEN(0);
-    straggle(lag, s, 1);
-    __builtin_amdgcn_sched_barrier(0);
-    float4 lp4 = make_float4(0.f, 0.f, 0.f, 0.f), v4 = lp4;
-    if (attn && act_r) {
-      const float4 l4 = lds4(s_loc + 4 * TID), p4 = lds4(s_pm + 4 * TID);
-      lp4 = make_float4(l4.x + p4.x, l4.y + p4.y, l4.z + p4.z, l4.w + p4.w);
-      v4 = lds4(s_vv + 4 * (tid & 3));
-    }
-    {
-      bool need[2 * PB];
-#pragma unroll
-      for (int i = 0; i < 2 * PB; ++i) need[i] = act[i >> 1];
-      float v[2 * PB];
-      unsigned tg[2 * PB];
-      lazy_wait(attn ? g.first : g.lazy);
-      const unsigned np_ = gather<2 * PB>(g.hatt, (unsigned)(p * GS * ATT_RNN + tid), PT, want, need, v, tg, pc);
-      PROF_POLLS(1, np_);
-#pragma unroll
-      for (int i = 0; i < 2 * PB; ++i)
-        if (need[i]) s_hatt[TID + PT * i] = v[i];
-    }
-    __syncthreads();
-    PROF_MARK(3);
-    if (attn && act_r) {
-      float q0 = 0.f, q1 = 0.f;
-#pragma unroll
-      for (int j = 0; j < 4; ++j) {
-        const float4 v = lds4(s_hatt + rb * ATT_RNN + 256 * j + L4);
-        if (ROLE_REGS) {
-          q0 = dot4(make_float4(rw[ROLE_REGS ? 4 * j : 0], rw[ROLE_REGS ? 4 * j + 1 : 0], rw[ROLE_REGS ? 4 * j + 2 : 0], rw[ROLE_REGS ? 4 * j + 3 : 0]), v, q0);
-          q1 = dot4(make_float4(rw[ROLE_REGS ? 16 + 4 * j : 0], rw[ROLE_REGS ? 17 + 4 * j : 0], rw[ROLE_REGS ? 18 + 4 * j : 0], rw[ROLE_REGS ? 19 + 4 * j : 0]), v, q1);
-        } else {
-          q0 = dot4(lds4(s_qw + 4 * (j * PT + TID)), v, q0);
-          q1 = dot4(lds4(s_qw + 4 * ((4 + j) * PT + TID)), v, q1);
-        }
-      }
-      q0 = wave_sum(q0);
-      q1 = wave_sum(q1);
-      if (lane == 0) {
-        s_q[wave] = q0;
-        s_q[wave + NW] = q1;
-      }
-      __syncthreads();
-      PROF_MARK(15);
-      const int t = tid >> 2, dq = 4 * (tid & 3);
-      const float4 q4 = lds4(s_q + dq);
-      float e = v4.x * fast_tanh(q4.x + lp4.x);
-      e = fmaf(v4.y, fast_tanh(q4.y + lp4.y), e);
-      e = fmaf(v4.z, fast_tanh(q4.z + lp4.z), e);
-      e = fmaf(v4.w, fast_tanh(q4.w + lp4.w), e);
-      e += dpp_move<0xB1, 0xf>(0.f, e);
-      e += dpp_move<0x4E, 0xf>(0.f, e);
-      if ((tid & 3) == 0 && t < T) publish(g.ep + (unsigned)(((p * GS + rb) * ATTN_CU + rk) * EP_LD + t), want, e);
-    }
-#pragma unroll
-    for (int b = 0; b < PB; ++b)
-      if (act[b]) {
-        float a0 = dacc[b][0], a1 = dacc[b][1];
-#pragma unroll
-        for (int k = 0; k < 4; ++k) {
-          const float4 v = lds4(s_hatt + b * ATT_RNN + 256 * k + L4);
-          a0 = dot4(wd[0][k], v, a0);
-          a1 = dot4(wd[1][k], v, a1);
-        }
-        dacc[b][0] = a0;
-        dacc[b][1] = a1;
-        chunk_fence();
-      }
-    PROF_MARK(4);
-    straggle(lag, s, 2);
-    __builtin_amdgcn_sched_barrier(0);
-    {
-      const int t = tid >> 2, j = tid & 3;
-      bool need[2 * PB];
-#pragma unroll
-      for (int i = 0; i < 2 * PB; ++i) need[i] = act[i >> 1] && t < T;
-      float v[2 * PB];
-      unsigned tg[2 * PB];
-      lazy_wait(attn ? g.efirst : g.clazy);
-      const unsigned np_ = gather<2 * PB>(g.ep, (unsigned)((p * GS * ATTN_CU + j) * EP_LD + t), 4u * EP_LD, want, need, v, tg, pc);
-      PROF_POLLS(2, np_);
-#pragma unroll
-      for (int b = 0; b < PB; ++b) {
-        float e = v[2 * b] + v[2 * b + 1];
-        e += dpp_move<0xB1, 0xf>(0.f, e);
-        e += dpp_move<0x4E, 0xf>(0.f, e);
-        if (j == 0 && act[b]) s_e[b * TP + t] = (t < T && t < nv[b]) ? e : -INFINITY;
-      }
-    }
-    __syncthreads();
-    PROF_MARK(5);
-    PROF_WHEN(3);
-#pragma unroll
-    for (int b = 0; b < PB; ++b)
-      if (act[b]) {
-        const float e0 = s_e[b * TP + lane], e1 = s_e[b * TP + lane + 64];
-        const float m = wave_max(fmaxf(e0, e1));
-        const float x0 = fast_exp(e0 - m), x1 = fast_exp(e1 - m);
-        const float rs = __builtin_amdgcn_rcpf(wave_sum(x0 + x1));
-        wreg[b][0] = x0 * rs;
-        wreg[b][1] = x1 * rs;
-      }
-    if (attn && act_r && wave == 0) {
-      s_aw[lane] = wreg[rb][0];
-      s_awc[lane] += wreg[rb][0];
-      s_aw[lane + 64] = wreg[rb][1];
-      s_awc[lane + 64] += wreg[rb][1];
-    }
-    PROF_MARK(6);
-    straggle(lag, s, 3);
-    __builtin_amdgcn_sched_barrier(0);
-#pragma unroll
-    for (int b = 0; b < PB; ++b)
-      if (act[b]) {
-        const float w0 = wreg[b][0], w1 = wreg[b][1];
-        float a0 = fmaf(pmd[b][0][1], w1, fmaf(pmd[b][0][0], w0, dacc[b][0]));
-        float a1 = fmaf(pmd[b][1][1], w1, fmaf(pmd[b][1][0], w0, dacc[b][1]));
-        a0 = wave_sum(a0);
-        a1 = wave_sum(a1);
-        if (lane == 0) {
-          s_g[b * 16 + wave] = a0 + s_bias[16 + wave];
-          s_g[b * 16 + wave + NW] = a1 + s_bias[16 + wave + NW];
-        }
-      }
-    __syncthreads();
-    if (cell && s_act[cb]) {
-      const float *gp = s_g + cb * 16 + 4 * cu;
-      const float ig = fast_sigmoid(gp[0]), fg = fast_sigmoid(gp[1]), gg = fast_tanh(gp[2]), og = fast_sigmoid(gp[3]);
-      const float cn = fmaf(fg, s_cell[4 * PB + tid], ig * gg), hn = og * fast_tanh(cn);
-      publish(g.hdec + (unsigned)((p * GS + cb) * DEC_RNN + 4 * c + cu), want, hn);
-      s_cell[4 * PB + tid] = cn;
-      s_cell[12 * PB + tid] = hn;
-    }
-    att_bulk(L4, false);
-    PROF_MARK(7);
-    PROF_WHEN(1);
-    straggle(lag, s, 4);
-    __builtin_amdgcn_sched_barrier(0);
-    unsigned drop1 = 0u, drop2 = 0u;
-    if (pre && act_r) {
-      if (d.dropout_mode) {
-#pragma unroll
-        for (int k = 0; k < 4; ++k)
-          drop1 |= (prenet_dropped(d.dropout_mode, d.dropout_seed, item, d.drop_masks, d.drop_steps, rb, s + 1, 0, lane + 64 * k) ? 1u : 0u) << k;
-#pragma unroll
-        for (int r = 0; r < 2; ++r)
-          drop2 |= (prenet_dropped(d.dropout_mode, d.dropout_seed, item, d.drop_masks, d.drop_steps, rb, s + 1, 1, 16 * rk + wave + NW * r) ? 1u : 0u) << r;
-      }
-    }
-    {
-      bool need[2 * PB];
-#pragma unroll
-      for (int i = 0; i < 2 * PB; ++i) need[i] = act[i >> 1];
-      float v[2 * PB];
-      unsigned tg[2 * PB];
-      lazy_wait(pre ? g.pfirst : g.lazy);
-      const unsigned np_ = gather<2 * PB>(g.hdec, (unsigned)(p * GS * DEC_RNN + tid), PT, want, need, v, tg, pc);
-      PROF_POLLS(3, np_);
-#pragma unroll
-      for (int i = 0; i < 2 * PB; ++i)
-        if (need[i]) s_hdec[TID + PT * i] = v[i];
-    }
-    __syncthreads();
-    PROF_MARK(8);
-    if (prow_ok && act_r) {
-      float a = 0.f;
-#pragma unroll
-      for (int j = 0; j < 4; ++j) a = dot4(lds4(s_pw + 4 * (j * PT + TID)), lds4(s_hdec + rb * DEC_RNN + 256 * j + L4), a);
-      a = fmaf(pmp[1], wreg[rb][1], fmaf(pmp[0], wreg[rb][0], a));
-      a = wave_sum(a);
-      if (lane == 0) publish(g.mel + (unsigned)(((p * GS + rb) * MEL_GL + prow) * MEL_ST), want, a + s_pb[wave]);
-    }
-    dec_bulk_h(L4, false);
-    if (attn && act_r) location(tid);
-    PROF_MARK(9);
-    straggle(lag, s, 5);
-    __builtin_amdgcn_sched_barrier(0);
-    if (pre && act_r) {
-      bool nxt = false;
-      if (act_r) {
-        if (tid < N_MEL + 1) {
-          const bool need[1] = {true};
-          float v[1];
-          unsigned tg[1];
-          gather<1>(g.mel, (unsigned)(((p * GS + rb) * MEL_GL + tid) * MEL_ST), 0, want, need, v, tg, pc);
-          s_mel[tid] = v[0];
-        }
-        __syncthreads();
-        PROF_MARK(11);
-        const float gate = s_mel[N_MEL];
-        const bool fired = GATE ? gate_fires(gate, d.gate_lo, d.gate_hi, d.gate_threshold) : (d.use_gate && gate_sigmoid(gate) > d.gate_threshold);
-        if (rk == 0) {
-          if (tid < N_MEL) d.frames[((size_t)rb * d.max_steps + s) * N_MEL + tid] = s_mel[tid];
-          if (tid == 0) {
-            d.gates[(size_t)rb * d.max_steps + s] = gate;
-            if (fired) d.nframes[rb] = s + 1;
-          }
-        }
-        if (fired) nf_r = s + 1;
-        nxt = s + 1 < nf_r;
-      }
-      float xo[2] = {0.f, 0.f};
-      if (nxt) {
-        const unsigned HM = (unsigned)((tid >> 8) * (N_MEL / 2));
-        float acc = 0.f;
-        if (ROLE_REGS) {
-#pragma unroll
-          for (int k = 0; k < N_MEL / 2; k += 4) {
-            const float4 m = lds4(s_mel + HM + k);
-            acc = fmaf(rw[ROLE_REGS ? k : 0], m.x, acc);
-            acc = fmaf(rw[ROLE_REGS ? k + 1 : 0], m.y, acc);
-            acc = fmaf(rw[ROLE_REGS ? k + 2 : 0], m.z, acc);
-            acc = fmaf(rw[ROLE_REGS ? k + 3 : 0], m.w, acc);
-          }
-        } else {
-#pragma unroll
-          for (int k = 0; k < N_MEL / 2; k += 4) {
-            const float4 w4 = lds4(s_W0 + 4u * (((HM + k) >> 2) * PRENET + (TID & 255u))), m = lds4(s_mel + HM + k);
-            acc = fmaf(w4.x, m.x, acc);
-            acc = fmaf(w4.y, m.y, acc);
-            acc = fmaf(w4.z, m.z, acc);
-            acc = fmaf(w4.w, m.w, acc);
-          }
-        }
-        PROF_MARK(12);
-        s_l1[TID] = acc;
-        __syncthreads();
-        PROF_MARK(13);
-        float pk[4];
-#pragma unroll
-        for (int k = 0; k < 4; ++k) {
-          const float v = fmaxf(s_l1[(L4 >> 2) + 64 * k] + s_l1[PRENET + (L4 >> 2) + 64 * k], 0.f);
-          pk[k] = (drop1 >> k) & 1u ? 0.f : (d.dropout_mode ? 2.f * v : v);
-        }
-#pragma unroll
-        for (int r = 0; r < 2; ++r) {
-          float a = 0.f;
-#pragma unroll
-          for (int k = 0; k < 4; ++k) a = fmaf(w1r[r][k], pk[k], a);
-          a = fmaxf(wave_sum(a), 0.f);
-          xo[r] = (drop2 >> r) & 1u ? 0.f : (d.dropout_mode ? 2.f * a : a);
-        }
-      }
-      PROF_MARK(14);
-      if (lane < 2) s_mel[MEL_GL - 16 + wave + NW * lane] = lane ? xo[1] : xo[0];
-      __syncthreads();
-      if (tid < 16)
-        publish(g.x + (unsigned)(((p ^ 1) * GS + rb) * PRENET + 16 * rk + tid), (want + 1u) | (nxt ? ACT_BIT : 0u),
-                s_mel[MEL_GL - 16 + tid]);
-    }
-    PROF_MARK(10);
+    if (s_act[4] != 0) r = -1;
+    if (r >= 0) {
+      const unsigned TID = (unsigned)tid_k + opaque(0u), HM = (TID >> 8) * (N_MEL / 2);
+      const bool a_role = attn_w && rb == r, p_role = pre_w && rb == r;
+#pragma unroll
+      for (int k = 0; k < 10; ++k) {
+        float4 v = make_float4(0.f, 0.f, 0.f, 0.f);
+        if (a_role && k < 8) v = lds4(s_qw + 4u * (k * PT + TID));
+        if (p_role) v = lds4(s_W0 + 4u * (((HM + 4 * k) >> 2) * PRENET + (TID & 255u)));
+        rw[k] = v;
+      }
+    }
+    if (r == 0) {
+      while (s < s_end && step(I1, I0, s)) ++s;
+    } else if (r == 1) {
+      while (s < s_end && step(I1, I1, s)) ++s;
     }
   }
 #ifdef XDTTS_PERSIST_PROFILE
@@ -1187,6 +1223,9 @@
   g.xlazy = 0;
   g.clazy = 4;
   g.shrink = 0;
+  g.cont = 0;
+  g.tail = 0;
+  g.tail_slot = 0;
   g.spins = 0;
   g.fault = 0;
   g.slow = 0;
diff --git a/xd-tts_amd/csrc/env.cpp b/xd-tts_amd/csrc/env.cpp
--- a/xd-tts_amd/csrc/env.cpp
+++ b/xd-tts_amd/csrc/env.cpp
@@ -16,6 +16,7 @@
     {"XDTTS_NO_TAIL", Kind::form, When::handle},
     {"XDTTS_NO_CTXFOLD", Kind::form, When::handle},
     {"XDTTS_NO_SKEW", Kind::form, When::handle},
+    {"XDTTS_PAIR_RELAUNCH", Kind::form, When::handle},
     {"XDTTS_P8", Kind::form, When::handle},
     {"XDTTS_GEMM_TILE", Kind::form, When::process},
     {"XDTTS_GEMM_SPLITK", Kind::form, When::process},
diff --git a/xd-tts_amd/csrc/env.h b/xd-tts_amd/csrc/env.h
--- a/xd-tts_amd/csrc/env.h
+++ b/xd-tts_amd/csrc/env.h
@@ -6,7 +6,7 @@
 
 enum Id {
   DEVICE, CHIP_LOCK_DIR, DECODER, GL, COOP,
-  ATT_FUSED, NO_EARLY, NO_TAIL, NO_CTXFOLD, NO_SKEW, P8,
+  ATT_FUSED, NO_EARLY, NO_TAIL, NO_CTXFOLD, NO_SKEW, PAIR_RELAUNCH, P8,
   GEMM_TILE, GEMM_SPLITK, GEMM_SPLIT_TILE, GL_BATCH_FORCE,
   ATT_SPINS, ATT_FAULT, ATT_SLOW, TAIL_FAULT,
   PERSIST_SPINS, PERSIST_FAULT, PERSIST_SLOW, ENC_SPINS, ENC_FAULT, GL_SPINS, GL_SLOW,
diff --git a/xd-tts_amd/csrc/kernels.h b/xd-tts_amd/csrc/kernels.h
--- a/xd-tts_amd/csrc/kernels.h
+++ b/xd-tts_amd/csrc/kernels.h
@@ -76,6 +76,8 @@
   int skew;
   int both_run;
   int shrink;
+  int cont;
+  int tail, tail_slot;
   int first;
   int efirst;
   int xfirst;
diff --git a/xd-tts_amd/csrc/tacotron2_decode.cpp b/xd-tts_amd/csrc/tacotron2_decode.cpp
--- a/xd-tts_amd/csrc/tacotron2_decode.cpp
+++ b/xd-tts_amd/csrc/tacotron2_decode.cpp
@@ -204,11 +204,18 @@
       const int first = std::min(lim[b0], lim[b0 + 1]), r = lim[b0] > lim[b0 + 1] ? 0 : 1;
       g.shrink = 0;
       g.both_run = 1;
-      launch_decoder_persistent(v, w, g, first, stream);
-      launch_decoder_persistent(view(b0 + r, 1), w, persist_view(g, r), lim[b0 + r] - first, stream);
+      if (!pair_relaunch) {
+        g.tail = lim[b0 + r] - first;
+        g.tail_slot = r;
+        launch_decoder_persistent(v, w, g, first, stream);
+      } else {
+        launch_decoder_persistent(v, w, g, first, stream);
+        launch_decoder_persistent(view(b0 + r, 1), w, persist_view(g, r), lim[b0 + r] - first, stream);
+      }
     } else {
+      g.cont = g.shrink && !pair_relaunch ? 1 : 0;
       launch_decoder_persistent(v, w, g, sub_lim, stream);
-      if (g.shrink) {
+      if (g.shrink && pair_relaunch) {
         for (int r = 0; r < n; ++r) {
           PersistBufs g1 = persist_view(g, r);
           g1.shrink = 0;
diff --git a/xd-tts_amd/csrc/tacotron2_handle.cpp b/xd-tts_amd/csrc/tacotron2_handle.cpp
--- a/xd-tts_amd/csrc/tacotron2_handle.cpp
+++ b/xd-tts_amd/csrc/tacotron2_handle.cpp
@@ -161,6 +161,8 @@
   pmel.alloc(decoder_pmel_floats(B));
   frames.alloc((size_t)B * ms * N_MEL);
   gates.alloc((size_t)B * ms);
+  state_B = B;
+  state_T = T;
   DecoderBufs d{};
   d.B = B;
   d.T = T;
diff --git a/xd-tts_amd/csrc/tacotron2_handle.h b/xd-tts_amd/csrc/tacotron2_handle.h
--- a/xd-tts_amd/csrc/tacotron2_handle.h
+++ b/xd-tts_amd/csrc/tacotron2_handle.h
@@ -59,10 +59,12 @@
   bool early_partial = !xdtts::env::is_set(xdtts::env::NO_EARLY);
   bool ctx_fold_table = !xdtts::env::is_set(xdtts::env::NO_CTXFOLD);
   bool pair_skew = !xdtts::env::is_set(xdtts::env::NO_SKEW);
+  bool pair_relaunch = xdtts::env::is_set(xdtts::env::PAIR_RELAUNCH);
   bool p8_wanted = [] { const char *p = xdtts::env::raw(xdtts::env::P8); return !(p && p[0] == '0'); }();
   bool two_launch = !xdtts::env::is_set(xdtts::env::NO_TAIL);
   int coop_group = 16;
   DevBuf<float> att_h, att_c, dec_h, dec_c, aw, awc, ctx, x, loc, e_part, pmel, frames, gates;
+  int state_B = 0, state_T = 0;
   DevBuf<float> frag;
   DevBuf<float> pmem_t;
   DevSlot<int> item_perm;
```

Result: slower. 128,400 (-1.4%).
